# deprekate/PHANOTATE

Hardware: AMD Instinct MI355X
Metric: Mbp/s annotated (whole node) on 50 kb synthetic phage contigs (higher is better)
Workload: dtype u8 bases / fp64 scores / int64 edge weights / int128 distances; 1 GPU; batch of 1000 synthetic 50000 bp phage contigs on one GPU, resident in HBM (BASELINE config 4); contigs_total=1000, contigs_rank0=1000, contig_length=50000

## Files before the change

include/phx.h:

```cpp
#ifndef PHX_H
#define PHX_H

#include <stddef.h>
#include <stdint.h>

#ifdef __cplusplus
extern "C" {
#endif

#define PHX_VERSION 410
#define PHX_MAX_CODONS 16

#define PHX_OK 0
#define PHX_E_ARG (-1)
#define PHX_E_NODEVICE (-10)
#define PHX_E_HIP (-11)
#define PHX_E_NOMEM (-12)
#define PHX_E_STATE (-13)
#define PHX_E_PARAM (-14)
#define PHX_E_IO (-15)

#define PHX_S_OK 0
#define PHX_S_BADLETTER (-2)
#define PHX_S_TOOSHORT (-3)
#define PHX_S_BADTRNA (-4)
#define PHX_S_PARALLEL (-6)
#define PHX_S_OVERFLOW (-7)
#define PHX_S_LONGORF (-8)
#define PHX_S_NEGCYCLE (-9)
#define PHX_S_NOPATH 1

typedef struct phx_ctx phx_ctx;

typedef struct phx_params {
    int32_t minlen;
    int32_t n_start;
    char start[PHX_MAX_CODONS][4];
    double start_w[PHX_MAX_CODONS];
    int32_t n_stop;
    char stop[PHX_MAX_CODONS][4];
    char start_w_text[PHX_MAX_CODONS][32];
} phx_params;

typedef struct phx_gene {
    int32_t left;
    int32_t right;
    int32_t strand;
    int32_t frame;
    double score;
} phx_gene;

typedef struct phx_result {
    int32_t status;
    int32_t n_genes;
    phx_gene *genes;
} phx_result;

typedef struct phx_orf {
    int32_t start;
    int32_t stop;
    int32_t frame;
    int32_t length;
    int32_t rbs;
    int32_t startidx;
    int32_t group;
    int32_t hist[9];
    double pstop;
    double weight_rbs;
    double S;
    double weight;
} phx_orf;

typedef struct phx_node {
    int32_t pos;
    int8_t type;
    int8_t frame;
    int16_t pad;
    int32_t other;
    int32_t refidx;
    double o;
} phx_node;

typedef struct phx_edge {
    int32_t src, dst;
    double w;
    int32_t inexact;
    int32_t pad;
    double d1, d2, err;
} phx_edge;

typedef struct phx_globals {
    int64_t L;
    double pstop;
    double background_rbs[28];
    double training_rbs[28];
    double pos_max[4], pos_min[4];
    int32_t n_orf, n_group, n_node, n_edge, n_bridge;
    int32_t n_limbs;
    int32_t sssp_sweeps;
    int32_t sssp_iters;
    int32_t status;
    int32_t sssp_kernel;
    int32_t sssp_handed_back;
    int32_t tie;
    int32_t certified;
    uint32_t rbs_background_count[28], rbs_training_count[28];
    uint32_t gc_max_count[4], gc_min_count[4];
    int64_t gc_count;
} phx_globals;

int phx_version(void);
int phx_device_count(void);
const char *phx_strerror(int code);
const char *phx_last_error(const phx_ctx *ctx);

void phx_default_params(phx_params *p);
int phx_params_from_flags(const char *start_codons, const char *stop_codons, int32_t minlen, phx_params *p);

int phx_create(const phx_params *params, int device, void *stream, phx_ctx **out);
#define PHX_CREATE_USE_STREAM 1u
#define PHX_CREATE_NO_GRAPH 2u
#define PHX_CREATE_SIZE_EVERY_RUN 4u
#define PHX_CREATE_SOLVER_GLOBAL 8u
#define PHX_CREATE_SOLVER_NO_WAVE 16u
#define PHX_CREATE_NO_CERTIFY 32u
#define PHX_CREATE_CERT_TIGHT 64u
#define PHX_CREATE_POISON 256u
#define PHX_CREATE_ONE_STREAM 512u
#define PHX_CREATE_CERT_WIDE 128u
#define PHX_CREATE_NO_DUO 4096u
#define PHX_CREATE_NO_SEG 8192u
#define PHX_CREATE_NO_FUSE 2048u
#define PHX_CREATE_NO_EXACT 1024u
int phx_create_ex(const phx_params *params, int device, void *stream, uint32_t flags, phx_ctx **out);
void phx_destroy(phx_ctx *ctx);

int phx_annotate(phx_ctx *ctx, int32_t n, const char *const *seq, const int64_t *len, phx_result *out );
void phx_free_results(phx_result *res, int32_t n);

int phx_upload(phx_ctx *ctx, int32_t n, const char *const *seq, const int64_t *len);
int phx_attach(phx_ctx *ctx, int32_t n, const void *d_ascii, const int64_t *offsets);
int phx_set_trnas(phx_ctx *ctx, const int64_t *offsets , const int32_t *start, const int32_t *stop);
int phx_run(phx_ctx *ctx);
int phx_run_async(phx_ctx *ctx);
int phx_wait(phx_ctx *ctx);
int phx_download(phx_ctx *ctx, phx_result *out);
int phx_download_flat(phx_ctx *ctx, phx_gene *genes, int64_t cap, int64_t *offsets , int32_t *status , int64_t *total);

typedef struct phx_pool phx_pool;
int phx_pool_create(const phx_params *params, int32_t n_dev, const int32_t *devices, uint32_t flags, phx_pool **out);
void phx_pool_destroy(phx_pool *pool);
const char *phx_pool_last_error(const phx_pool *pool);
int phx_pool_annotate(phx_pool *pool, int32_t n, const char *const *seq, const int64_t *len, int64_t batch_bases,
                      const int64_t *trna_offsets, const int32_t *trna_start, const int32_t *trna_stop, phx_result *out );

int phx_certified(phx_ctx *ctx, int8_t *cert );
int phx_set_exact(phx_ctx *ctx, int on);

int phx_tap_globals(phx_ctx *ctx, int32_t contig, phx_globals *out);
int phx_tap_positions(phx_ctx *ctx, int32_t contig, uint8_t *cls, uint8_t *gcc, uint8_t *binF, uint8_t *binR);
int phx_tap_orfs(phx_ctx *ctx, int32_t contig, phx_orf *out );
int phx_tap_nodes(phx_ctx *ctx, int32_t contig, phx_node *out );
int phx_tap_edges(phx_ctx *ctx, int32_t contig, phx_edge *out );
int phx_tap_path(phx_ctx *ctx, int32_t contig, int32_t *path, int32_t cap, int32_t *n_path, uint64_t *dist_limbs, int32_t cap_limbs);
int phx_tap_dist(phx_ctx *ctx, int32_t contig, uint64_t *dist_limbs, int64_t cap_words);

typedef struct phx_orf_margin {
    int32_t left, right, strand, frame;
    double score;
    double margin;
    int32_t called;
    int32_t through;
} phx_orf_margin;
int phx_margins_flat(phx_ctx *ctx, phx_orf_margin *rec, int64_t cap, int64_t *offsets , int32_t *status , int64_t *total);
int phx_tap_dist_target(phx_ctx *ctx, int32_t contig, uint64_t *dist_limbs, int64_t cap_words);
int phx_margins_ms(phx_ctx *ctx, float *ms );

typedef struct phx_gene_drop {
    int32_t left, right, strand, frame;
    double score;
    double drop;
    int32_t called;
    int32_t bypass;
} phx_gene_drop;
int phx_drop_margins_flat(phx_ctx *ctx, phx_gene_drop *rec, int64_t cap, int64_t *offsets , int32_t *status , int64_t *total);
int phx_drop_ms(phx_ctx *ctx, float *ms );
int phx_drop_stats(phx_ctx *ctx, int64_t *out );

typedef struct phx_gene_repl {
    int32_t left, right, strand, frame;
    double drop;
    int32_t called, bypass;
    int32_t span_left, span_right;
    int32_t n_removed, n_added;
    int64_t gene_off;
} phx_gene_repl;
int phx_replacements_flat(phx_ctx *ctx, phx_gene_repl *rec, int64_t cap, phx_gene *genes, int64_t gene_cap, int64_t *offsets ,
                          int32_t *status , int64_t *total, int64_t *gene_total);
int phx_tap_replacement(phx_ctx *ctx, int32_t contig, int32_t k, int32_t *path, int32_t cap, int32_t *n_path);
int phx_replacements_ms(phx_ctx *ctx, float *ms );
int phx_replacement_stats(phx_ctx *ctx, int64_t *out );

int phx_reannotate_flat(phx_ctx *ctx, const uint8_t *forbid, const int64_t *orf_offsets , uint32_t flags, phx_gene *genes, int64_t cap,
                        int64_t *offsets , int32_t *status , double *delta , int64_t *total);
int phx_orf_offsets(phx_ctx *ctx, int64_t *orf_offsets );
int phx_tap_repath(phx_ctx *ctx, int32_t contig, int32_t *path, int32_t cap, int32_t *n_path, uint64_t *dist_limbs, int32_t cap_limbs);
int phx_reannotate_ms(phx_ctx *ctx, float *ms );

int phx_dump_text(phx_ctx *ctx, int32_t contig, char **text, int64_t *text_len);

int phx_solve(phx_ctx *ctx, int32_t V, int32_t E, const int32_t *src, const int32_t *dst, const uint64_t *w_limbs,
              int32_t n_limbs, int32_t source, int32_t target, int32_t *path_out, int32_t cap, int32_t *n_path,
              uint64_t *dist_limbs);

#define PHX_N_STAGES 14
int phx_set_profiling(phx_ctx *ctx, int on);
int phx_set_profiling_stages(phx_ctx *ctx, uint32_t stage_mask);
int phx_get_stage_ms(phx_ctx *ctx, float *ms , int32_t *launches , int reset);
const char *phx_stage_name(int k);
int64_t phx_plan_timeouts(phx_ctx *ctx);
int64_t phx_front_runs(phx_ctx *ctx);
int64_t phx_seg_runs(phx_ctx *ctx);
int64_t phx_seg_fallbacks(phx_ctx *ctx);
int phx_seg_stats(phx_ctx *ctx, int32_t i, int32_t *out, int32_t cap_records);
int phx_batch_sizes(phx_ctx *ctx, int64_t *L, int64_t *n_orf, int64_t *n_node, int64_t *n_edge);

int phx_synth_contig(uint64_t seed, int64_t L, char *out);
int phx_dec_eval(const char *op, const char *a, const char *b, int prec, char *out, int cap);
int phx_dd_eval(const char *op, double ah, double al, double bh, double bl, double *rh, double *rl);
int phx_dd_shortest(double x, uint64_t *digits, int32_t *exp10);

typedef struct phx_fasta phx_fasta;
int phx_fasta_read(const char *path, phx_fasta **out);
int32_t phx_fasta_count(const phx_fasta *f);
int phx_fasta_record(const phx_fasta *f, int32_t i, const char **name, const char **seq, int64_t *len);
int phx_fasta_arrays(const phx_fasta *f, const char **names, const char **seqs, int64_t *lens);
void phx_fasta_free(phx_fasta *f);
int phx_format_tabular(int32_t n, const char *const *names, const phx_gene *genes, const int64_t *offsets, const int32_t *status, char **text, int64_t *text_len);
int phx_format_margins(int32_t n, const char *const *names, const phx_orf_margin *rec, const int64_t *offsets, const int32_t *status, char **text, int64_t *text_len);
int phx_format_drops(int32_t n, const char *const *names, const phx_gene_drop *rec, const int64_t *offsets, const int32_t *status, char **text, int64_t *text_len);
int phx_format_replacements(int32_t n, const char *const *names, const phx_gene_repl *rec, const phx_gene *genes, const int64_t *offsets,
                            const int32_t *status, char **text, int64_t *text_len);
void phx_free_text(char *text);

#ifdef __cplusplus
}
#endif
#endif
```

phanotate_amd/_lib.py:

```python
import ctypes as C
import os

import numpy as np

HERE = os.path.dirname(os.path.abspath(__file__))
SO = os.path.join(HERE, "libphx.so")
MAXC = 16
N_STAGES = 14


class Params(C.Structure):
    _fields_ = [
        ("minlen", C.c_int32),
        ("n_start", C.c_int32),
        ("start", (C.c_char * 4) * MAXC),
        ("start_w", C.c_double * MAXC),
        ("n_stop", C.c_int32),
        ("stop", (C.c_char * 4) * MAXC),
        ("start_w_text", (C.c_char * 32) * MAXC),
    ]


class Gene(C.Structure):
    _fields_ = [("left", C.c_int32), ("right", C.c_int32), ("strand", C.c_int32), ("frame", C.c_int32), ("score", C.c_double)]


class Result(C.Structure):
    _fields_ = [("status", C.c_int32), ("n_genes", C.c_int32), ("genes", C.POINTER(Gene))]


class Globals(C.Structure):
    _fields_ = [
        ("L", C.c_int64), ("pstop", C.c_double),
        ("background_rbs", C.c_double * 28), ("training_rbs", C.c_double * 28),
        ("pos_max", C.c_double * 4), ("pos_min", C.c_double * 4),
        ("n_orf", C.c_int32), ("n_group", C.c_int32), ("n_node", C.c_int32), ("n_edge", C.c_int32), ("n_bridge", C.c_int32),
        ("n_limbs", C.c_int32), ("sssp_sweeps", C.c_int32), ("sssp_iters", C.c_int32), ("status", C.c_int32),
        ("sssp_kernel", C.c_int32), ("sssp_handed_back", C.c_int32), ("tie", C.c_int32), ("certified", C.c_int32),
        ("rbs_background_count", C.c_uint32 * 28), ("rbs_training_count", C.c_uint32 * 28), ("gc_max_count", C.c_uint32 * 4), ("gc_min_count", C.c_uint32 * 4),
        ("gc_count", C.c_int64),
    ]


GENE_DT = np.dtype([("left", "i4"), ("right", "i4"), ("strand", "i4"), ("frame", "i4"), ("score", "f8")], align=True)
ORF_DT = np.dtype([("start", "i4"), ("stop", "i4"), ("frame", "i4"), ("length", "i4"), ("rbs", "i4"), ("startidx", "i4"), ("group", "i4"),
                   ("hist", "i4", (9,)), ("pstop", "f8"), ("weight_rbs", "f8"), ("S", "f8"), ("weight", "f8")], align=True)
NODE_DT = np.dtype([("pos", "i4"), ("type", "i1"), ("frame", "i1"), ("pad", "i2"), ("other", "i4"), ("refidx", "i4"), ("o", "f8")], align=True)
MARGIN_DT = np.dtype([("left", "i4"), ("right", "i4"), ("strand", "i4"), ("frame", "i4"), ("score", "f8"), ("margin", "f8"), ("called", "i4"), ("through", "i4")], align=True)
DROP_DT = np.dtype([("left", "i4"), ("right", "i4"), ("strand", "i4"), ("frame", "i4"), ("score", "f8"), ("drop", "f8"), ("called", "i4"), ("bypass", "i4")], align=True)
REPL_DT = np.dtype([("left", "i4"), ("right", "i4"), ("strand", "i4"), ("frame", "i4"), ("drop", "f8"), ("called", "i4"), ("bypass", "i4"),
                    ("span_left", "i4"), ("span_right", "i4"), ("n_removed", "i4"), ("n_added", "i4"), ("gene_off", "i8")], align=True)
EDGE_DT = np.dtype([("src", "i4"), ("dst", "i4"), ("w", "f8"), ("inexact", "i4"), ("pad", "i4"), ("d1", "f8"), ("d2", "f8"), ("err", "f8")], align=True)

_lib = None


class PhxError(RuntimeError):
    def __init__(self, code, msg):
        super().__init__("libphx error %d: %s" % (code, msg))
        self.code = code


def _preload_hip_runtime():
    import importlib.util
    import sys

    if "torch" in sys.modules:
        return
    try:
        spec = importlib.util.find_spec("torch")
    except (ImportError, ValueError):
        spec = None
    if spec is None or not spec.submodule_search_locations:
        return
    cand = os.path.join(list(spec.submodule_search_locations)[0], "lib", "libamdhip64.so")
    if os.path.exists(cand):
        try:
            C.CDLL(cand, mode=C.RTLD_GLOBAL)
        except OSError:
            pass


def lib():
    global _lib
    if _lib is not None:
        return _lib
    if not os.path.exists(SO):
        raise ImportError("%s is missing: build it with `python -c 'import __graft_entry__ as g; g.build()'` "
                          "or `make -C phanotate_amd/csrc`; phanotate_amd has no CPU fallback" % SO)
    _preload_hip_runtime()
    L = C.CDLL(SO)
    vp, i32, i64 = C.c_void_p, C.c_int32, C.c_int64
    P = C.POINTER
    sig = {
        "phx_version": (C.c_int, []),
        "phx_device_count": (C.c_int, []),
        "phx_strerror": (C.c_char_p, [C.c_int]),
        "phx_last_error": (C.c_char_p, [vp]),
        "phx_default_params": (None, [P(Params)]),
        "phx_params_from_flags": (C.c_int, [C.c_char_p, C.c_char_p, i32, P(Params)]),
        "phx_set_exact": (C.c_int, [vp, C.c_int]),
        "phx_pool_create": (C.c_int, [P(Params), i32, P(i32), C.c_uint32, P(vp)]),
        "phx_pool_destroy": (None, [vp]),
        "phx_pool_last_error": (C.c_char_p, [vp]),
        "phx_pool_annotate": (C.c_int, [vp, i32, P(C.c_char_p), P(i64), i64, vp, vp, vp, P(Result)]),
        "phx_dump_text": (C.c_int, [vp, i32, P(vp), P(i64)]),
        "phx_dec_eval": (C.c_int, [C.c_char_p, C.c_char_p, C.c_char_p, C.c_int, C.c_char_p, C.c_int]),
        "phx_dd_eval": (C.c_int, [C.c_char_p, C.c_double, C.c_double, C.c_double, C.c_double, P(C.c_double), P(C.c_double)]),
        "phx_dd_shortest": (C.c_int, [C.c_double, P(C.c_uint64), P(i32)]),
        "phx_create": (C.c_int, [P(Params), C.c_int, vp, P(vp)]),
        "phx_create_ex": (C.c_int, [P(Params), C.c_int, vp, C.c_uint32, P(vp)]),
        "phx_destroy": (None, [vp]),
        "phx_annotate": (C.c_int, [vp, i32, P(C.c_char_p), P(i64), P(Result)]),
        "phx_free_results": (None, [P(Result), i32]),
        "phx_upload": (C.c_int, [vp, i32, P(C.c_char_p), P(i64)]),
        "phx_attach": (C.c_int, [vp, i32, vp, P(i64)]),
        "phx_set_trnas": (C.c_int, [vp, vp, vp, vp]),
        "phx_run": (C.c_int, [vp]),
        "phx_run_async": (C.c_int, [vp]),
        "phx_wait": (C.c_int, [vp]),
        "phx_download": (C.c_int, [vp, P(Result)]),
        "phx_download_flat": (C.c_int, [vp, vp, i64, vp, vp, P(i64)]),
        "phx_certified": (C.c_int, [vp, vp]),
        "phx_tap_globals": (C.c_int, [vp, i32, P(Globals)]),
        "phx_tap_positions": (C.c_int, [vp, i32, vp, vp, vp, vp]),
        "phx_tap_orfs": (C.c_int, [vp, i32, vp]),
        "phx_tap_nodes": (C.c_int, [vp, i32, vp]),
        "phx_tap_edges": (C.c_int, [vp, i32, vp]),
        "phx_tap_path": (C.c_int, [vp, i32, vp, i32, P(i32), vp, i32]),
        "phx_tap_dist": (C.c_int, [vp, i32, vp, i64]),
        "phx_tap_dist_target": (C.c_int, [vp, i32, vp, i64]),
        "phx_margins_flat": (C.c_int, [vp, vp, i64, vp, vp, P(i64)]),
        "phx_margins_ms": (C.c_int, [vp, P(C.c_float)]),
        "phx_format_margins": (C.c_int, [i32, vp, vp, vp, vp, P(vp), P(i64)]),
        "phx_drop_margins_flat": (C.c_int, [vp, vp, i64, vp, vp, P(i64)]),
        "phx_drop_ms": (C.c_int, [vp, P(C.c_float)]),
        "phx_drop_stats": (C.c_int, [vp, P(i64)]),
        "phx_format_drops": (C.c_int, [i32, vp, vp, vp, vp, P(vp), P(i64)]),
        "phx_replacements_flat": (C.c_int, [vp, vp, i64, vp, i64, vp, vp, P(i64), P(i64)]),
        "phx_tap_replacement": (C.c_int, [vp, i32, i32, vp, i32, P(i32)]),
        "phx_replacements_ms": (C.c_int, [vp, P(C.c_float)]),
        "phx_replacement_stats": (C.c_int, [vp, P(i64)]),
        "phx_format_replacements": (C.c_int, [i32, vp, vp, vp, vp, vp, P(vp), P(i64)]),
        "phx_reannotate_flat": (C.c_int, [vp, vp, vp, C.c_uint32, vp, i64, vp, vp, vp, P(i64)]),
        "phx_orf_offsets": (C.c_int, [vp, vp]),
        "phx_tap_repath": (C.c_int, [vp, i32, vp, i32, P(i32), vp, i32]),
        "phx_reannotate_ms": (C.c_int, [vp, P(C.c_float)]),
        "phx_solve": (C.c_int, [vp, i32, i32, vp, vp, vp, i32, i32, i32, vp, i32, P(i32), vp]),
        "phx_set_profiling": (C.c_int, [vp, C.c_int]),
        "phx_set_profiling_stages": (C.c_int, [vp, C.c_uint32]),
        "phx_get_stage_ms": (C.c_int, [vp, P(C.c_float), P(i32), C.c_int]),
        "phx_stage_name": (C.c_char_p, [C.c_int]),
        "phx_batch_sizes": (C.c_int, [vp, P(i64), P(i64), P(i64), P(i64)]),
        "phx_plan_timeouts": (C.c_int64, [vp]),
        "phx_front_runs": (C.c_int64, [vp]),
        "phx_seg_runs": (C.c_int64, [vp]),
        "phx_seg_fallbacks": (C.c_int64, [vp]),
        "phx_seg_stats": (C.c_int, [vp, C.c_int32, C.c_void_p, C.c_int32]),
        "phx_synth_contig": (C.c_int, [C.c_uint64, i64, C.c_char_p]),
        "phx_fasta_read": (C.c_int, [C.c_char_p, P(vp)]),
        "phx_fasta_count": (i32, [vp]),
        "phx_fasta_record": (C.c_int, [vp, i32, P(vp), P(vp), P(i64)]),
        "phx_fasta_arrays": (C.c_int, [vp, vp, vp, vp]),
        "phx_fasta_free": (None, [vp]),
        "phx_format_tabular": (C.c_int, [i32, vp, vp, vp, vp, P(vp), P(i64)]),
        "phx_free_text": (None, [vp]),
    }
    for name, (res, args) in sig.items():
        f = getattr(L, name)
        f.restype = res
        f.argtypes = args
    assert GENE_DT.itemsize == C.sizeof(Gene)
    assert MARGIN_DT.itemsize == 40
    assert DROP_DT.itemsize == 40
    assert REPL_DT.itemsize == 56
    _lib = L
    return L


EXPORTS = ["phx_version", "phx_device_count", "phx_strerror", "phx_last_error", "phx_default_params", "phx_params_from_flags", "phx_set_exact", "phx_pool_create", "phx_pool_destroy", "phx_pool_last_error", "phx_pool_annotate", "phx_dump_text", "phx_dec_eval", "phx_dd_eval", "phx_dd_shortest", "phx_create", "phx_create_ex", "phx_destroy",
           "phx_annotate", "phx_free_results", "phx_upload", "phx_attach", "phx_set_trnas", "phx_run", "phx_run_async", "phx_wait", "phx_download", "phx_download_flat", "phx_certified", "phx_tap_globals",
           "phx_tap_positions", "phx_tap_orfs", "phx_tap_nodes", "phx_tap_edges", "phx_tap_path", "phx_tap_dist", "phx_solve", "phx_set_profiling", "phx_set_profiling_stages",
           "phx_get_stage_ms", "phx_stage_name", "phx_batch_sizes", "phx_plan_timeouts", "phx_front_runs", "phx_seg_runs", "phx_seg_fallbacks", "phx_seg_stats", "phx_synth_contig", "phx_fasta_read", "phx_fasta_count",
           "phx_fasta_record", "phx_fasta_arrays", "phx_fasta_free", "phx_format_tabular", "phx_free_text",
           "phx_margins_flat", "phx_tap_dist_target", "phx_margins_ms", "phx_format_margins",
           "phx_drop_margins_flat", "phx_drop_ms", "phx_drop_stats", "phx_format_drops",
           "phx_replacements_flat", "phx_tap_replacement", "phx_replacements_ms", "phx_replacement_stats",
           "phx_format_replacements",
           "phx_reannotate_flat", "phx_orf_offsets", "phx_tap_repath", "phx_reannotate_ms"]
```

phanotate_amd/api.py:

```python
import ctypes as C

import numpy as np

from . import _lib
from ._lib import PhxError


def make_params(start_codons="atg:0.85,gtg:0.10,ttg:0.05", stop_codons="tag,tga,taa", minlen=90):
    p = _lib.Params()
    rc = _lib.lib().phx_params_from_flags(start_codons.encode(), stop_codons.encode(), int(minlen), C.byref(p))
    if rc:
        raise ValueError("start / stop codons %r / %r, minlen %r: libphx takes codon:weight pairs and codons of exactly 3 letters out of acgt, "
                         "at most %d of each, minlen >= 6 (%s)" % (start_codons, stop_codons, minlen, _lib.MAXC, _lib.lib().phx_strerror(rc).decode()))
    p.start_codons_text = start_codons
    return p


def synth_contig(seed, L=50000):
    buf = C.create_string_buffer(int(L))
    rc = _lib.lib().phx_synth_contig(int(seed), int(L), buf)
    if rc:
        raise PhxError(rc, "phx_synth_contig")
    return buf.raw


class Pool:

    def __init__(self, params=None, devices=(0,), flags=()):
        self.L = _lib.lib()
        self.params = params or make_params()
        fl = 0
        for f in flags:
            fl |= Annotator.FLAGS[f]
        devs = (C.c_int32 * len(devices))(*[int(d) for d in devices])
        h = C.c_void_p()
        rc = self.L.phx_pool_create(C.byref(self.params), len(devices), devs, fl, C.byref(h))
        if rc:
            raise PhxError(rc, "%s (%s)" % (self.L.phx_strerror(rc).decode(), self.L.phx_last_error(None).decode()))
        self.h = h

    def close(self):
        if getattr(self, "h", None):
            self.L.phx_pool_destroy(self.h)
            self.h = None

    def __enter__(self):
        return self

    def __exit__(self, *exc):
        self.close()

    def __del__(self):
        try:
            self.close()
        except Exception:
            pass

    def annotate(self, seqs, trnas=None, batch_bases=0):
        seqs = [s.encode() if isinstance(s, str) else bytes(s) for s in seqs]
        n = len(seqs)
        arr = (C.c_char_p * max(n, 1))(*seqs)
        lens = (C.c_int64 * max(n, 1))(*[len(s) for s in seqs])
        res = (_lib.Result * max(n, 1))()
        to = ta = tz = None
        if trnas is not None:
            offs = np.zeros(n + 1, np.int64)
            np.cumsum([len(t) for t in trnas], out=offs[1:])
            a = np.ascontiguousarray([h[0] for t in trnas for h in t] or [0], np.int32)
            z = np.ascontiguousarray([h[1] for t in trnas for h in t] or [0], np.int32)
            to, ta, tz = (x.ctypes.data_as(C.c_void_p) for x in (offs, a, z))
        rc = self.L.phx_pool_annotate(self.h, n, arr, lens, int(batch_bases), to, ta, tz, res)
        if rc:
            raise PhxError(rc, "phx_pool_annotate: %s (%s)" % (self.L.phx_strerror(rc).decode(), self.L.phx_pool_last_error(self.h).decode()))
        out = []
        for i in range(n):
            g = np.zeros(res[i].n_genes, _lib.GENE_DT)
            if res[i].n_genes:
                C.memmove(g.ctypes.data, res[i].genes, res[i].n_genes * _lib.GENE_DT.itemsize)
            out.append((int(res[i].status), g))
        self.L.phx_free_results(res, n)
        return out


class Annotator:

    FLAGS = {"no_graph": 2, "size_every_run": 4, "solver_global": 8, "solver_no_wave": 16, "no_certify": 32, "cert_tight": 64, "cert_wide": 128, "poison": 256, "one_stream": 512, "no_exact": 1024, "no_fuse": 2048, "no_duo": 4096, "no_seg": 8192}

    def __init__(self, params=None, device=0, stream=None, flags=()):
        self.L = _lib.lib()
        self.params = params or make_params()
        h = C.c_void_p()
        fl = 0
        for f in flags:
            fl |= self.FLAGS[f]
        if stream is None:
            rc = self.L.phx_create_ex(C.byref(self.params), int(device), None, fl, C.byref(h))
        else:
            rc = self.L.phx_create_ex(C.byref(self.params), int(device), C.c_void_p(int(stream)), 1 | fl, C.byref(h))
        if rc:
            raise PhxError(rc, "%s (%s)" % (self.L.phx_strerror(rc).decode(), self.L.phx_last_error(None).decode()))
        self.h = h
        self.n = 0

    def close(self):
        if getattr(self, "h", None):
            self.L.phx_destroy(self.h)
            self.h = None

    def __del__(self):
        try:
            self.close()
        except Exception:
            pass

    def _chk(self, rc, what):
        if rc:
            raise PhxError(rc, "%s: %s (%s)" % (what, self.L.phx_strerror(rc).decode(), self.L.phx_last_error(self.h).decode()))

    def upload(self, seqs):
        seqs = [s.encode() if isinstance(s, str) else bytes(s) for s in seqs]
        n = len(seqs)
        arr = (C.c_char_p * n)(*seqs)
        lens = (C.c_int64 * n)(*[len(s) for s in seqs])
        self._keep = (seqs, arr, lens)
        self._chk(self.L.phx_upload(self.h, n, arr, lens), "phx_upload")
        self.n = n
        self._orf_offs = None

    def upload_raw(self, ptrs, lens, keep=None):
        ptrs = np.ascontiguousarray(ptrs, np.uint64)
        lens = np.ascontiguousarray(lens, np.int64)
        self._keep = (ptrs, lens, keep)
        self._chk(self.L.phx_upload(self.h, len(lens), C.cast(ptrs.ctypes.data, C.POINTER(C.c_char_p)), C.cast(lens.ctypes.data, C.POINTER(C.c_int64))), "phx_upload")
        self.n = len(lens)
        self._orf_offs = None

    def attach(self, dev_ptr, offsets):
        offs = (C.c_int64 * len(offsets))(*[int(x) for x in offsets])
        self._keep = (offs,)
        self._chk(self.L.phx_attach(self.h, len(offsets) - 1, C.c_void_p(int(dev_ptr)), offs), "phx_attach")
        self.n = len(offsets) - 1
        self._orf_offs = None

    def set_trnas(self, trnas):
        if trnas is None:
            self._chk(self.L.phx_set_trnas(self.h, None, None, None), "phx_set_trnas")
            return
        if len(trnas) != self.n:
            raise ValueError("one hit list per contig of the batch")
        offs = np.zeros(self.n + 1, np.int64)
        np.cumsum([len(t) for t in trnas], out=offs[1:])
        a = np.ascontiguousarray([h[0] for t in trnas for h in t] or [0], np.int32)
        z = np.ascontiguousarray([h[1] for t in trnas for h in t] or [0], np.int32)
        vp = lambda x: x.ctypes.data_as(C.c_void_p)
        self._chk(self.L.phx_set_trnas(self.h, vp(offs), vp(a), vp(z)), "phx_set_trnas")

    def run(self):
        self._chk(self.L.phx_run(self.h), "phx_run")
        self._orf_offs = None

    def run_async(self):
        self._chk(self.L.phx_run_async(self.h), "phx_run_async")
        self._orf_offs = None

    def wait(self):
        self._chk(self.L.phx_wait(self.h), "phx_wait")

    def set_exact(self, on):
        self._chk(self.L.phx_set_exact(self.h, 1 if on else 0), "phx_set_exact")

    def download_flat(self, exact=True):
        if not exact:
            self._chk(self.L.phx_set_exact(self.h, 0), "phx_set_exact")
            try:
                res = self._download_flat()
            finally:
                self._chk(self.L.phx_set_exact(self.h, 1), "phx_set_exact")
            self.resolved = []
            return res
        res = self._download_flat()
        self.resolved = [int(i) for i in np.nonzero(self.certified() == 2)[0]] if self.n else []
        return res

    def _download_flat(self):
        n = self.n
        offs = np.zeros(n + 1, np.int64)
        status = np.zeros(max(n, 1), np.int32)
        total = C.c_int64(0)
        vp = lambda a: a.ctypes.data_as(C.c_void_p)
        guess = max(int(getattr(self, "_genes_seen", 0) * 1.25) + 64, 1)
        genes = np.empty(guess, _lib.GENE_DT)
        rc = self.L.phx_download_flat(self.h, vp(genes), len(genes), vp(offs), vp(status), C.byref(total))
        if rc == -1 and int(total.value) > len(genes):
            genes = np.empty(int(total.value), _lib.GENE_DT)
            rc = self.L.phx_download_flat(self.h, vp(genes), len(genes), vp(offs), vp(status), C.byref(total))
        self._chk(rc, "phx_download_flat")
        self._genes_seen = int(total.value)
        return status[:n], offs, genes[: int(total.value)]

    def certified(self):
        c = np.zeros(max(self.n, 1), np.int8)
        self._chk(self.L.phx_certified(self.h, c.ctypes.data_as(C.c_void_p)), "phx_certified")
        return c[: self.n]

    def download(self):
        status, offs, genes = self.download_flat()
        o = offs.tolist()
        st = status.tolist()
        return [(st[i], genes[o[i]:o[i + 1]]) for i in range(self.n)]

    def annotate(self, seqs, trnas=None):
        self.upload(seqs)
        if trnas is not None:
            self.set_trnas(trnas)
        self.run_async()
        return self.download()

    def annotate_flat(self, seqs):
        self.upload(seqs)
        self.run_async()
        return self.download_flat()

    def annotate_flat_raw(self, ptrs, lens, keep=None):
        self.upload_raw(ptrs, lens, keep)
        self.run_async()
        return self.download_flat()

    def dump_text(self, i):
        text, n = C.c_void_p(), C.c_int64()
        self._chk(self.L.phx_dump_text(self.h, int(i), C.byref(text), C.byref(n)), "phx_dump_text")
        out = C.string_at(text.value, n.value)
        self.L.phx_free_text(text)
        return out

    def globals(self, i):
        g = _lib.Globals()
        self._chk(self.L.phx_tap_globals(self.h, i, C.byref(g)), "phx_tap_globals")
        return g

# ... 101 lines not shown
        n = self.n
        offs = np.zeros(n + 1, np.int64)
        status = np.zeros(max(n, 1), np.int32)
        total, gtotal = C.c_int64(), C.c_int64()
        vp = lambda a: a.ctypes.data_as(C.c_void_p)
        self._chk(self.L.phx_replacements_flat(self.h, None, 0, None, 0, vp(offs), vp(status), C.byref(total), C.byref(gtotal)), "phx_replacements_flat")
        rec = np.empty(max(int(total.value), 1), _lib.REPL_DT)
        genes = np.empty(max(int(gtotal.value), 1), _lib.GENE_DT)
        self._chk(self.L.phx_replacements_flat(self.h, vp(rec), len(rec), vp(genes), len(genes), vp(offs), vp(status), C.byref(total), C.byref(gtotal)),
                  "phx_replacements_flat")
        return status[:n], offs, rec[: int(total.value)], genes[: int(gtotal.value)]

    def replacement_path(self, i, k):
        n = C.c_int32()
        self._chk(self.L.phx_tap_replacement(self.h, i, k, None, 0, C.byref(n)), "phx_tap_replacement")
        p = np.zeros(max(n.value, 1), np.int32)
        self._chk(self.L.phx_tap_replacement(self.h, i, k, p.ctypes.data_as(C.c_void_p), len(p), C.byref(n)), "phx_tap_replacement")
        return p[: n.value].copy()

    def replacements_ms(self):
        ms = (C.c_float * 3)()
        self._chk(self.L.phx_replacements_ms(self.h, ms), "phx_replacements_ms")
        return dict(zip(("argmin", "walk", "download"), [float(x) for x in ms]))

    def replacement_stats(self):
        out = (C.c_int64 * 5)()
        self._chk(self.L.phx_replacement_stats(self.h, out), "phx_replacement_stats")
        return dict(zip(("cross", "chain_nodes", "cross_kept", "cut", "regrown"), [int(x) for x in out]))

    def orf_offsets(self):
        if getattr(self, "_orf_offs", None) is None:
            offs = np.zeros(self.n + 1, np.int64)
            self._chk(self.L.phx_orf_offsets(self.h, offs.ctypes.data_as(C.c_void_p)), "phx_orf_offsets")
            self._orf_offs = offs
        return self._orf_offs

    def orf_index(self, i, left, right, strand):
        cache = getattr(self, "_orf_index", None)
        if cache is None or cache[0] is not self.orf_offsets() or cache[1] != i:
            o = self.orfs(i)
            fwd = o["frame"] > 0
            lo = np.where(fwd, o["start"], o["stop"])
            hi = np.where(fwd, o["stop"], o["start"]) + 2
            table = {}
            for k, key in enumerate(zip(lo.tolist(), hi.tolist(), fwd.tolist())):
                table.setdefault(key, k)
            cache = self._orf_index = (self.orf_offsets(), i, table)
        try:
            return cache[2][(int(left), int(right), int(strand) > 0)]
        except KeyError:
            raise KeyError("contig %d has no ORF %d..%d on strand %+d" % (i, left, right, 1 if int(strand) > 0 else -1)) from None

    def reannotate(self, forbid, solve_all=False):
        n = self.n
        if len(forbid) != n:
            raise ValueError("one index array (or None) per contig of the batch")
        oo = self.orf_offsets()
        mask = np.zeros(max(int(oo[n]), 1), np.uint8)
        for i, f in enumerate(forbid):
            if f is None:
                continue
            idx = np.asarray(f, np.int64).reshape(-1)
            if idx.size and (idx.min() < 0 or idx.max() >= oo[i + 1] - oo[i]):
                raise IndexError("contig %d has %d ORFs" % (i, oo[i + 1] - oo[i]))
            mask[oo[i] + idx] = 1
        offs = np.zeros(n + 1, np.int64)
        status = np.zeros(max(n, 1), np.int32)
        delta = np.zeros(max(n, 1), np.float64)
        total = C.c_int64(0)
        vp = lambda a: a.ctypes.data_as(C.c_void_p)
        fl = 1 if solve_all else 0
        self._chk(self.L.phx_reannotate_flat(self.h, vp(mask), vp(oo), fl, None, 0, vp(offs), vp(status), vp(delta), C.byref(total)), "phx_reannotate_flat")
        genes = np.empty(max(int(total.value), 1), _lib.GENE_DT)
        self._chk(self.L.phx_reannotate_flat(self.h, vp(mask), vp(oo), fl, vp(genes), len(genes), vp(offs), vp(status), vp(delta), C.byref(total)), "phx_reannotate_flat")
        return status[:n], offs, genes[: int(total.value)], delta[:n]

    def reannotated_path(self, i):
        g = self.globals(i)
        p = np.zeros(max(g.n_node, 1), np.int32)
        n = C.c_int32()
        limbs = np.zeros(32, np.uint64)
        self._chk(self.L.phx_tap_repath(self.h, i, p.ctypes.data_as(C.c_void_p), len(p), C.byref(n), limbs.ctypes.data_as(C.c_void_p), 32), "phx_tap_repath")
        nl = max(g.n_limbs, 1)
        v = 0
        for k in range(nl):
            v |= int(limbs[k]) << (64 * k)
        if v >> (64 * nl - 1):
            v -= 1 << (64 * nl)
        return p[: n.value].copy(), v

    def reannotate_ms(self):
        ms = (C.c_float * 3)()
        self._chk(self.L.phx_reannotate_ms(self.h, ms), "phx_reannotate_ms")
        return dict(zip(("mask", "solve", "finish"), [float(x) for x in ms]))

    def drop_stats(self):
        out = (C.c_int64 * 4)()
        self._chk(self.L.phx_drop_stats(self.h, out), "phx_drop_stats")
        return dict(zip(("slots", "cross", "rescanned", "layered"), [int(x) for x in out]))

    def solve(self, V, src, dst, weights, source, target, n_limbs=None):
        E = len(src)
        mx = max([abs(int(w)) for w in weights] + [1])
        bits = mx.bit_length() + max(V, 2).bit_length() + 3
        if n_limbs is None:
            n_limbs = 2 if bits <= 128 else 4 if bits <= 256 else 8 if bits <= 512 else 17
        wl = np.zeros((max(E, 1), n_limbs), np.uint64)
        mask = (1 << 64) - 1
        for e, w in enumerate(weights):
            w = int(w) & ((1 << (64 * n_limbs)) - 1)
            for k in range(n_limbs):
                wl[e, k] = (w >> (64 * k)) & mask
        s = np.ascontiguousarray(src, np.int32)
        d = np.ascontiguousarray(dst, np.int32)
        path = np.zeros(V, np.int32)
        n = C.c_int32()
        dl = np.zeros(n_limbs, np.uint64)
        self._chk(self.L.phx_solve(self.h, V, E, s.ctypes.data_as(C.c_void_p), d.ctypes.data_as(C.c_void_p), wl.ctypes.data_as(C.c_void_p),
                                   n_limbs, source, target, path.ctypes.data_as(C.c_void_p), V, C.byref(n), dl.ctypes.data_as(C.c_void_p)), "phx_solve")
        if n.value == 0:
            return [], None
        v = 0
        for k in range(n_limbs):
            v |= int(dl[k]) << (64 * k)
        if v >> (64 * n_limbs - 1):
            v -= 1 << (64 * n_limbs)
        return path[: n.value].tolist(), v

    def set_profiling(self, on=True):
        self._chk(self.L.phx_set_profiling(self.h, 1 if on else 0), "phx_set_profiling")

    def set_profiling_stages(self, names):
        idx = {self.L.phx_stage_name(k).decode(): k for k in range(_lib.N_STAGES)}
        mask = 0
        for nm in names:
            mask |= 1 << idx[nm]
        self._chk(self.L.phx_set_profiling_stages(self.h, mask), "phx_set_profiling_stages")

    def stage_ms(self, reset=True):
        ms = (C.c_float * _lib.N_STAGES)()
        nl = (C.c_int32 * _lib.N_STAGES)()
        self._chk(self.L.phx_get_stage_ms(self.h, ms, nl, 1 if reset else 0), "phx_get_stage_ms")
        return {self.L.phx_stage_name(k).decode(): (float(ms[k]), int(nl[k])) for k in range(_lib.N_STAGES)}

    def front_runs(self):
        return int(self.L.phx_front_runs(self.h))

    def seg_runs(self):
        return int(self.L.phx_seg_runs(self.h))

    def seg_fallbacks(self):
        return int(self.L.phx_seg_fallbacks(self.h))

    def seg_stats(self, i):
        import numpy as np

        out = np.zeros((64, 8), np.int32)
        n = self.L.phx_seg_stats(self.h, int(i), out.ctypes.data_as(C.c_void_p), 64)
        return out[:n]

    def plan_timeouts(self):
        return int(self.L.phx_plan_timeouts(self.h))

    def batch_sizes(self):
        v = [C.c_int64() for _ in range(4)]
        self._chk(self.L.phx_batch_sizes(self.h, *[C.byref(x) for x in v]), "phx_batch_sizes")
        return dict(L=v[0].value, n_orf=v[1].value, n_node=v[2].value, n_edge=v[3].value)
```

phanotate_amd/csrc/phx_api.cpp:

```cpp
#include <hip/hip_runtime.h>

#include <algorithm>
#include <atomic>
#include <cmath>
#include <condition_variable>
#include <functional>
#include <mutex>
#include <cstdio>
#include <cstdlib>
#include <cstring>
#include <memory>
#include <limits>
#include <map>
#include <string>
#include <thread>
#include <vector>

#include "phx_internal.h"
extern "C" {
#include "phx_dec.h"
}

namespace {

// ... 18 lines not shown
            p = nullptr; cap = 0;
            const size_t want = count + count / 4 + 16;
            if (hipHostMalloc((void **)&p, want * sizeof(DMeta), hipHostMallocDefault) != hipSuccess) { p = nullptr; n = 0; return false; }
            cap = want;
        }
        n = count;
        if (n) memset(p, 0, n * sizeof(DMeta));
        return true;
    }
    void release() { if (p) (void)hipHostFree(p); p = nullptr; n = cap = 0; }
    DMeta *begin() { return p; }
    DMeta *end() { return p + n; }
    const DMeta *begin() const { return p; }
    const DMeta *end() const { return p + n; }
    DMeta &operator[](size_t i) { return p[i]; }
    const DMeta &operator[](size_t i) const { return p[i]; }
    DMeta *data() { return p; }
};

}

struct StagePool {
    std::vector<std::thread> th;
    std::mutex m;
    std::condition_variable cv, cv_done;
    const std::function<void()> *job = nullptr;
    uint64_t gen = 0;
    int active = 0;
    bool stop = false;
    void grow(int n) {
        while ((int)th.size() < n) {
            try { th.emplace_back([this, seen = gen]() mutable { loop(seen); }); } catch (...) { break; }
        }
    }
    void loop(uint64_t seen) {
        std::unique_lock<std::mutex> lk(m);
        for (;;) {
            cv.wait(lk, [&] { return stop || gen != seen; });
            if (stop) return;
            seen = gen;
            const std::function<void()> *j = job;
            lk.unlock();
            (*j)();
            lk.lock();
            if (--active == 0) cv_done.notify_all();
        }
    }
    void start(const std::function<void()> *j) {
        std::lock_guard<std::mutex> lk(m);
        job = j; active = (int)th.size(); gen++;
        cv.notify_all();
    }
    void finish() {
        std::unique_lock<std::mutex> lk(m);
        cv_done.wait(lk, [&] { return active == 0; });
    }
    ~StagePool() {
        { std::lock_guard<std::mutex> lk(m); stop = true; cv.notify_all(); }
        for (std::thread &t : th) t.join();
    }
};

struct phx_ctx {
    int device = 0;
    hipStream_t stream = nullptr;
    bool own_stream = false;
    hipStream_t aux[4] = {nullptr, nullptr, nullptr, nullptr};
    bool in_flight = false;
    int pend_mask = 0;
    int64_t pend_lds[4] = {0, 0, 0, 0};
    hipEvent_t ev_fork = nullptr, ev_fork_plan = nullptr, ev_fork_nodes = nullptr, ev_join_nodes = nullptr, ev_fork_pre = nullptr, ev_join_pre = nullptr, ev_fork_orf = nullptr, ev_join_orf = nullptr, ev_fork_score = nullptr, ev_join_score = nullptr, ev_join[4] = {nullptr, nullptr, nullptr, nullptr};
    phx_params params;
    std::string err;
    DParams *d_params = nullptr;
    int n = 0;
    bool uploaded = false, ran = false;
    int64_t totalL = 0, tot_orf = 0, tot_grp = 0, tot_node = 0, tot_edge = 0;
    int n_limbs = 0;
    MetaBuf meta;
    bool meta_stale = false;
    DRes *res = nullptr;
    size_t res_cap = 0;
    std::vector<uint32_t> ftab;
    uint32_t vtotal = 0;
    bool defcod = false;
    const void *attached = nullptr;
    hipEvent_t ev_upload = nullptr; bool upload_pending = false;
    hipEvent_t ev_layout = nullptr; bool layout_pending = false;
    hipEvent_t ev_piece[2] = {nullptr, nullptr};
    void *h_tiles = nullptr; size_t h_tiles_cap = 0;
    bool eager_now = false;
    bool eager_done = false;
    bool trna_clean = true;
    std::unique_ptr<StagePool> pool;
    DevBuf b_bridge, b_recs, b_meta, b_tiles, b_nbits, b_nbase, b_cbits, b_orf, b_ostat, b_oweight, b_owi, b_oflag, b_onode, b_grp, b_bits, b_cpre, b_bpre, b_item, b_iprev;
    DevBuf b_ewf, b_esrcf;
    bool tapw_valid = false;
    int64_t tot_nbits = 0, tot_bridge = 0;
    int64_t tot_words = 0, tot_items = 0;
    DevBuf b_win, b_wrole;
    DevBuf b_tnode, b_tedge, b_tnid, b_tbits;
    std::vector<DTNode> h_tnode;
    bool has_trna = false;
    DevBuf b_cint, b_csig;
    DevBuf b_eref;
    bool certify = true;
    bool cert_done = false;
    bool exact = true;
    bool exact_done = false;
    std::map<int, std::vector<DGene>> exact_genes;
    std::vector<int> host_only;
    int exact_failed = 0;
    double cert_scale = 1.0;
    bool cert_wide = false;
    bool poison = false;
    bool one_stream = false;
    bool learning = false;
    DevBuf b_tie;
    int64_t tie_seen = 0;
    DevBuf b_ekey;
    DevBuf b_meta0;
    bool meta0_dirty = true;
    int runs_on_layout = 0;
    DevBuf b_node, b_parent, b_inoff, b_no, b_npos, b_ehit, b_mreach, b_olist, b_dist, b_esrc, b_ew, b_ewl, b_path, b_genes, b_gtot, b_tot, b_lpart, b_res, b_sord, b_gtab, b_erank;
    DTotals *h_tot = nullptr;
    bool have_plan = false;
    int last_mask = 0;
    int last_vmax = 0;
    int64_t last_lds[4] = {0, 0, 0, 0};
    int64_t max_len = 0;
    bool graphs_enabled = true, graph_valid = false, tiles_dirty = true;
    hipGraph_t graph = nullptr;
    hipGraphExec_t graph_exec = nullptr;
    int graph_flags = -1;
    void *h_stage = nullptr;
    size_t h_stage_cap = 0;
    DGene *h_genes = nullptr; size_t h_genes_cap = 0;
    bool prof = false;
    uint32_t prof_mask = 0xffffffffu;
    int n_simd = 1024;
    bool force_global_sssp = false;
    bool no_wave = false, always_sync = false;
    bool no_fuse = false;
    bool duo = true;
    int front_spins = 8000;
    bool side_score = true;
    int orf_stream = 1;
    bool orf_rows = true;
    bool eager_cert = true;
    bool pend_cert = false;
    bool pend_front = false;
    bool front_off = false;
    int64_t front_runs = 0;
    bool seg_on = true;
    bool seg_off = false;
    bool seg_never = false;
    bool pend_seg = false;
    int pend_seg_k = 0;
    bool seg_clean = false;
    int seg_max_n = 32;
    int seg_margin_bp = 6000;
    int64_t seg_runs = 0, seg_aborts = 0, seg_fallbacks = 0;
    DevBuf b_swin, b_swrole, b_sdist, b_segw;
    int64_t plan_timeouts = 0;
    bool plan_stream_off = false;
    DevBuf b_mo, b_md, b_mw, b_mdt, b_mrec, b_mstat;
    bool margins_done = false;
    phx_orf_margin *h_mrec = nullptr; size_t h_mrec_cap = 0;
    std::vector<int32_t> mstat;
    std::vector<DGrp> mgrp;
    hipEvent_t mev[5] = {nullptr, nullptr, nullptr, nullptr, nullptr};
    float margins_ms[4] = {0, 0, 0, 0};
    bool rev_done = false;
    float rev_ms[2] = {0, 0};
    DevBuf b_dpi, b_djs, b_djt, b_dfi, b_dla, b_dslot, b_dgtab, b_doff, b_dsx, b_dcx, b_dda, b_ddb, b_drec, b_dstats;
    bool drops_done = false;
    phx_gene_drop *h_drec = nullptr; size_t h_drec_cap = 0;
    std::vector<int64_t> droff;
    hipEvent_t dev_[5] = {nullptr, nullptr, nullptr, nullptr, nullptr};
    float drop_ms[4] = {0, 0, 0, 0};
    int64_t drop_stats[4] = {0, 0, 0, 0};
    bool drop_trees = false;
    DevBuf b_dps, b_dts, b_rwin, b_rxs, b_rcoff, b_rcm, b_rchain, b_rrnd, b_rinfo, b_rdoff, b_rdet, b_rgenes, b_rrec, b_rcnt;
    bool repl_done = false;
    std::vector<phx_gene_repl> h_rrec;
    std::vector<phx_gene> h_rgenes;
    std::vector<int32_t> h_rdet, h_rinfo;
    std::vector<int64_t> h_rdoff;
    std::vector<std::vector<int32_t>> h_rpath;
    int64_t rchain_cap = 0;
    hipEvent_t rev_ev[9] = {nullptr, nullptr, nullptr, nullptr, nullptr, nullptr, nullptr, nullptr, nullptr};
    float repl_ms[3] = {0, 0, 0};
    int64_t repl_stats[5] = {0, 0, 0, 0, 0};
    DevBuf b_qmeta, b_qtot, b_qdist, b_qparent, b_qpath, b_qgenes, b_qgtot, b_qtie, b_qmask, b_qforb, b_qsel, b_qplan, b_qrec;
    bool reann_done = false;
    bool qgrp_done = false;
    std::vector<DGrp> qgrp;
    std::vector<uint8_t> h_qforb;
    uint32_t h_qflags = 0;
    std::vector<int32_t> h_qsel;
    std::vector<DReannRec> h_qrec;
    std::vector<DGene> h_qgenes;
    std::vector<uint8_t> h_qdforb;
    DTotals h_qtot;
    uint32_t h_qgtot = 0;
    hipEvent_t qev[6] = {nullptr, nullptr, nullptr, nullptr, nullptr, nullptr};
    float reann_ms[3] = {0, 0, 0};
    float stage_ms[PHX_N_STAGES] = {0};
    int stage_n[PHX_N_STAGES] = {0};
    std::vector<std::pair<int, std::pair<hipEvent_t, hipEvent_t>>> pending;
    std::vector<hipEvent_t> ev_pool;
};

static int seg_cap(const phx_ctx *c);
namespace {

#define HIPCHK(ctx, call)                                                                                      \
    do {                                                                                                       \
        hipError_t e_ = (call);                                                                                \
        if (e_ != hipSuccess) {                                                                                \
            (ctx)->err = std::string(#call) + ": " + hipGetErrorString(e_);                                    \
            return PHX_E_HIP;                                                                                  \
        }                                                                                                      \
    } while (0)

int ensure(phx_ctx *c, DevBuf &b, size_t bytes) {
    if (bytes + 2048 <= b.cap && b.p) return PHX_OK;
    c->graph_valid = false;
    if (b.p) HIPCHK(c, hipFree(b.p));
    b.p = nullptr; b.cap = 0;
    size_t want = bytes + bytes / 8 + 4096;
    HIPCHK(c, hipMalloc(&b.p, want));
    b.cap = want;
    if (c->poison) HIPCHK(c, hipMemset(b.p, 0xA5, want));
    return PHX_OK;
}
void release(DevBuf &b) {
    if (b.p) (void)hipFree(b.p);
    b.p = nullptr; b.cap = 0;
}

inline int code_of(char c) { return c == 'a' ? 0 : c == 'c' ? 1 : c == 't' ? 2 : c == 'g' ? 3 : -1; }

int check_params(const phx_params *p) {
    if (!p || p->minlen < 6 || p->n_start < 1 || p->n_start > PHX_MAX_CODONS || p->n_stop < 1 || p->n_stop > PHX_MAX_CODONS) return PHX_E_PARAM;
    for (int i = 0; i < p->n_start; i++) {
        for (int j = 0; j < 3; j++) if (code_of(p->start[i][j]) < 0) return PHX_E_PARAM;
        if (p->start[i][3] != 0) return PHX_E_PARAM;
        if (!(p->start_w[i] == p->start_w[i])) return PHX_E_PARAM;
        if (!memchr(p->start_w_text[i], 0, sizeof(p->start_w_text[i]))) return PHX_E_PARAM;
        if (p->start_w_text[i][0]) { dec_t t; if (dec_from_str(&t, p->start_w_text[i])) return PHX_E_PARAM; }
    }
    for (int i = 0; i < p->n_stop; i++) {
        for (int j = 0; j < 3; j++) if (code_of(p->stop[i][j]) < 0) return PHX_E_PARAM;
        if (p->stop[i][3] != 0) return PHX_E_PARAM;
    }
    return PHX_OK;
}

void build_dparams(const phx_params *p, DParams *d) {
    memset(d, 0, sizeof(*d));
    d->minlen = p->minlen;
    d->n_start = p->n_start;
    for (int i = 0; i < p->n_start; i++) d->start_w[i] = p->start_w[i];
    { dec_t q[PHX_MAX_CODONS]; dec_start_weights(p->n_start, p->start_w_text, p->start_w, q); for (int i = 0; i < p->n_start; i++) dec_to_dd(&q[i], &d->sw_hi[i], &d->sw_lo[i]); }
    auto codon_code = [](const char *c) { return code_of(c[0]) | (code_of(c[1]) << 2) | (code_of(c[2]) << 4); };
    auto rc_code = [](int ci) {
        int c0 = ci & 3, c1 = (ci >> 2) & 3, c2 = (ci >> 4) & 3;
        return (c2 ^ 2) | ((c1 ^ 2) << 2) | ((c0 ^ 2) << 4);
    };
    int start_idx[64], stop_is[64];
    for (int i = 0; i < 64; i++) { start_idx[i] = -1; stop_is[i] = 0; }
    for (int i = p->n_start - 1; i >= 0; i--) start_idx[codon_code(p->start[i])] = i;
    for (int i = 0; i < p->n_stop; i++) stop_is[codon_code(p->stop[i])] = 1;
    const int atg = codon_code("atg"), cat = codon_code("cat");
    for (int ci = 0; ci < 64; ci++) {
        const int rc = rc_code(ci);
        int cls = CLS_NONE, idx = 0;
        if (start_idx[ci] >= 0) { cls = CLS_FS; idx = start_idx[ci]; }
        else if (start_idx[rc] >= 0) { cls = CLS_RS; idx = start_idx[rc]; }
        else if (stop_is[ci]) cls = CLS_FT;
        else if (stop_is[rc]) cls = CLS_RT;
        d->cls_tab[ci] = (uint8_t)(cls | (idx << 3) | (start_idx[rc] >= 0 ? 0x80 : 0));
        d->atg_tab[ci] = (uint8_t)((ci == atg ? 1 : 0) | (ci == cat ? 2 : 0) | (idx << 2));
    }
}

hipEvent_t get_event(phx_ctx *c) {
    if (!c->ev_pool.empty()) { hipEvent_t e = c->ev_pool.back(); c->ev_pool.pop_back(); return e; }
    hipEvent_t e = nullptr;
    (void)hipEventCreate(&e);
    return e;
}
struct StageTimer {
    phx_ctx *c; int st; bool on = false; hipEvent_t a = nullptr, b = nullptr; hipStream_t str = nullptr;
    StageTimer(phx_ctx *c_, int st_, hipStream_t on_stream = nullptr) : c(c_), st(st_) {
        on = c->prof && ((c->prof_mask >> st_) & 1u);
        str = on_stream ? on_stream : c->stream;
        if (on) { a = get_event(c); b = get_event(c); (void)hipEventRecord(a, str); }
    }
    ~StageTimer() {
        if (on) { (void)hipEventRecord(b, str); c->pending.push_back({st, {a, b}}); }
    }
};
void collect_timers(phx_ctx *c) {
    for (auto &p : c->pending) {
// ... 126 lines not shown
        m.bits_off = words; m.item_off = items; m.nbits_off = nbw;
        m.bridge_off = nbr; m.bridge_cap = (int32_t)(L / 500 + 2);
        nbr += m.bridge_cap;
        nbw += 9 * (int64_t)m.nw;
        words += PHX_BITMAP_WORDS_PER_NW * (int64_t)m.nw; items += 6 * (int64_t)m.nw;
        off += L;
        off = (off + 15) & ~(int64_t)15;
    }
    c->vtotal = (uint32_t)(recs - 1);
    c->ftab.push_back(c->vtotal);
    {
        int ci = 0;
        for (int64_t blk = 0; blk * 62 < (int64_t)c->vtotal + 62; blk++) {
            const int64_t v = blk * 62 > 0 ? blk * 62 - 1 : 0;
            while (ci + 1 < n && v >= (int64_t)c->ftab[(size_t)ci + 1]) ci++;
            c->ftab.push_back((uint32_t)ci);
        }
    }
    c->tot_words = words; c->tot_items = items; c->tot_nbits = nbw; c->tot_bridge = nbr;
    c->totalL = offsets_or_null ? offsets_or_null[n] : off;
    c->n = n;
    return PHX_OK;
}

int ensure_position_buffers(phx_ctx *c) {
    int rc;
    if ((rc = ensure(c, c->b_recs, ((size_t)c->vtotal + 2) * 36))) return rc;
    if ((rc = ensure(c, c->b_nbits, (size_t)(c->tot_nbits + 8) * 8))) return rc;
    if ((rc = ensure(c, c->b_nbase, (size_t)(c->tot_nbits / 3 + 8) * 4))) return rc;
    if ((rc = ensure(c, c->b_meta, sizeof(DMeta) * (size_t)(c->n + 1)))) return rc;
    if ((rc = ensure(c, c->b_tiles, 4 * (c->ftab.size() + 1)))) return rc;
    if ((rc = ensure(c, c->b_gtot, 64))) return rc;
    if ((rc = ensure(c, c->b_lpart, ((size_t)c->n / 256 + 2) * 32 + 512))) return rc;
    if (sssp_ordered(c) && (rc = ensure(c, c->b_sord, (size_t)c->n * 4))) return rc;
    if ((rc = ensure(c, c->b_gtab, ((size_t)c->n + 1) * GT_N * 10))) return rc;
    if ((rc = ensure(c, c->b_res, ((size_t)c->n + 1) * sizeof(DRes) + sizeof(DTotals)))) return rc;
    if (c->res_cap < (size_t)c->n + 1) {
        if (c->res) (void)hipHostFree(c->res);
        c->res = nullptr; c->res_cap = 0;
        const size_t want = (size_t)c->n + (size_t)c->n / 4 + 16;
        if (hipHostMalloc((void **)&c->res, want * sizeof(DRes) + sizeof(DTotals), hipHostMallocDefault) != hipSuccess) { c->res = nullptr; c->err = "hipHostMalloc failed"; return PHX_E_NOMEM; }
        c->res_cap = want;
    }
    if ((rc = ensure(c, c->b_bits, (size_t)(c->tot_words + 8) * 8))) return rc;
    {
        const size_t W = (size_t)(c->tot_words / PHX_BITMAP_WORDS_PER_NW);
        if ((rc = ensure(c, c->b_cpre, (6 * (W / PHX_PRE_G + (size_t)c->n) + 2) * 32))) return rc;
        if ((rc = ensure(c, c->b_bpre, (2 * W + 2 * (size_t)c->n + 4) * 16))) return rc;
    }
    if ((rc = ensure(c, c->b_item, (size_t)(c->tot_items + 8) * 8))) return rc;
    if ((rc = ensure(c, c->b_iprev, (size_t)(c->tot_items + 8) * 4))) return rc;
    if ((rc = ensure(c, c->b_bridge, (size_t)(c->tot_bridge + 8) * sizeof(DBridge)))) return rc;
    return PHX_OK;
}

}

extern "C" {

int phx_version(void) { return PHX_VERSION; }

int phx_device_count(void) {
    int n = 0;
    if (hipGetDeviceCount(&n) != hipSuccess) return 0;
    return n;
}

const char *phx_strerror(int code) {
    switch (code) {
    case PHX_OK: return "ok";
    case PHX_E_ARG: return "bad argument";
    case PHX_E_NODEVICE: return "no usable HIP device (libphx has no CPU path)";
    case PHX_E_HIP: return "HIP runtime error";
    case PHX_E_NOMEM: return "out of memory";
    case PHX_E_STATE: return "call sequence error";
    case PHX_E_PARAM: return "bad codon table / minlen";
    case PHX_E_IO: return "file could not be opened or read";
    case PHX_S_BADLETTER: return "letter outside the IUPAC nucleotide alphabet";
    case PHX_S_TOOSHORT: return "contig shorter than 6 bases";
    case PHX_S_PARALLEL: return "bridge edge duplicates a connect edge";
    case PHX_S_BADTRNA: return "a tRNA hit lies outside the contig";
    case PHX_S_OVERFLOW: return "integer path sums overflow";
    case PHX_S_LONGORF: return "an open reading frame of more than 65535 codons";
    case PHX_S_NEGCYCLE: return "relaxation did not converge";
    case PHX_S_NOPATH: return "target unreachable";
    default: return "unknown";
    }
}

const char *phx_last_error(const phx_ctx *ctx) { return ctx ? ctx->err.c_str() : g_create_error.c_str(); }

void phx_default_params(phx_params *p) {
    memset(p, 0, sizeof(*p));
    p->minlen = 90;
    p->n_start = 3;
    strcpy(p->start[0], "atg"); strcpy(p->start[1], "gtg"); strcpy(p->start[2], "ttg");
    p->start_w[0] = 0.85 / 0.85; p->start_w[1] = 0.10 / 0.85; p->start_w[2] = 0.05 / 0.85;
    strcpy(p->start_w_text[0], "0.85"); strcpy(p->start_w_text[1], "0.10"); strcpy(p->start_w_text[2], "0.05");
    p->n_stop = 3;
    strcpy(p->stop[0], "tag"); strcpy(p->stop[1], "tga"); strcpy(p->stop[2], "taa");
}

int phx_params_from_flags(const char *start_codons, const char *stop_codons, int32_t minlen, phx_params *p) {
    if (!p) return PHX_E_ARG;
    phx_default_params(p);
    p->minlen = minlen;
    auto lower3 = [](const std::string &t, char *out) {
        if (t.size() != 3) return false;
        for (int j = 0; j < 3; j++) { const char ch = (char)(t[(size_t)j] | 0x20); if (code_of(ch) < 0) return false; out[j] = ch; }
        out[3] = 0;
        return true;
    };
    auto split = [](const char *s) { std::vector<std::string> v; std::string cur; for (; *s; s++) { if (*s == ',') { v.push_back(cur); cur.clear(); } else cur.push_back(*s); } v.push_back(cur); return v; };
    if (start_codons) {
        p->n_start = 0;
        memset(p->start, 0, sizeof(p->start)); memset(p->start_w, 0, sizeof(p->start_w)); memset(p->start_w_text, 0, sizeof(p->start_w_text));
        double wv[PHX_MAX_CODONS];
        for (const std::string &item : split(start_codons)) {
            const size_t colon = item.find(':');
            if (colon == std::string::npos || item.find(':', colon + 1) != std::string::npos) return PHX_E_PARAM;
            char cod[4];
            if (!lower3(item.substr(0, colon), cod)) return PHX_E_PARAM;
            const std::string wt = item.substr(colon + 1);
            if (wt.empty() || wt.size() >= sizeof(p->start_w_text[0])) return PHX_E_PARAM;
            char *end = nullptr;
            const double w = phx_strtod_c(wt.c_str(), &end);
            if (!end || *end || !(w == w)) return PHX_E_PARAM;
            int at = -1;
            for (int i = 0; i < p->n_start; i++) if (!strcmp(p->start[i], cod)) at = i;
            if (at < 0) { if (p->n_start >= PHX_MAX_CODONS) return PHX_E_PARAM; at = p->n_start++; strcpy(p->start[at], cod); }
            strcpy(p->start_w_text[at], wt.c_str());
            wv[at] = w;
        }
        if (p->n_start < 1) return PHX_E_PARAM;
        double mx = wv[0];
        for (int i = 1; i < p->n_start; i++) mx = wv[i] > mx ? wv[i] : mx;
        for (int i = 0; i < p->n_start; i++) p->start_w[i] = wv[i] / mx;
    }
    if (stop_codons) {
        p->n_stop = 0;
        memset(p->stop, 0, sizeof(p->stop));
        for (const std::string &item : split(stop_codons)) {
            if (p->n_stop >= PHX_MAX_CODONS) return PHX_E_PARAM;
            if (!lower3(item, p->stop[p->n_stop])) return PHX_E_PARAM;
            p->n_stop++;
        }
    }
    return check_params(p);
}

int phx_create(const phx_params *params, int device, void *stream, phx_ctx **out) { return phx_create_ex(params, device, stream, stream ? PHX_CREATE_USE_STREAM : 0u, out); }

int phx_create_ex(const phx_params *params, int device, void *stream, uint32_t flags, phx_ctx **out) {
    if (!out || (flags & ~(PHX_CREATE_USE_STREAM | PHX_CREATE_NO_GRAPH | PHX_CREATE_SIZE_EVERY_RUN | PHX_CREATE_SOLVER_GLOBAL | PHX_CREATE_SOLVER_NO_WAVE | PHX_CREATE_NO_CERTIFY | PHX_CREATE_CERT_TIGHT | PHX_CREATE_CERT_WIDE | PHX_CREATE_POISON | PHX_CREATE_ONE_STREAM | PHX_CREATE_NO_EXACT | PHX_CREATE_NO_FUSE | PHX_CREATE_NO_DUO | PHX_CREATE_NO_SEG)) || (stream && !(flags & PHX_CREATE_USE_STREAM))) return PHX_E_ARG;
    *out = nullptr;
    int rc = check_params(params);
    if (rc) return rc;
    int ndev = 0;
    hipError_t e = hipGetDeviceCount(&ndev);
    if (e != hipSuccess || ndev <= 0 || device < 0 || device >= ndev) {
        g_create_error = e != hipSuccess ? hipGetErrorString(e) : "device index out of range";
        return PHX_E_NODEVICE;
    }
    phx_ctx *c = new phx_ctx();
    c->device = device;
    c->params = *params;
    c->force_global_sssp = (flags & PHX_CREATE_SOLVER_GLOBAL) != 0;
    c->no_wave = (flags & PHX_CREATE_SOLVER_NO_WAVE) != 0;
    c->graphs_enabled = (flags & PHX_CREATE_NO_GRAPH) == 0;
    c->always_sync = (flags & PHX_CREATE_SIZE_EVERY_RUN) != 0;
    c->certify = (flags & PHX_CREATE_NO_CERTIFY) == 0;
    c->exact = (flags & PHX_CREATE_NO_EXACT) == 0;
    c->no_fuse = (flags & PHX_CREATE_NO_FUSE) != 0;
    { const char *e = getenv("PHX_FRONT_SPINS"); if (e && *e) c->front_spins = atoi(e); }
    { const char *e = getenv("PHX_NO_EAGER_CERT"); c->eager_cert = !(e && e[0] == '1'); }
    { const char *e = getenv("PHX_NO_ORF_ROWS"); c->orf_rows = !(e && e[0] == '1'); }
    { const char *e = getenv("PHX_ORF_STREAM"); if (e && *e) { const int v = atoi(e); if (v >= -1 && v <= 3) c->orf_stream = v; } }
    { const char *e = getenv("PHX_NO_SIDE_SCORE"); c->side_score = !(e && e[0] == '1'); }
    { const char *e = getenv("PHX_NO_DUO"); c->duo = !(flags & PHX_CREATE_NO_DUO) && !(e && e[0] == '1'); }
    { const char *e = getenv("PHX_NO_SEG"); c->seg_on = !(flags & PHX_CREATE_NO_SEG) && !(e && e[0] == '1'); }
    { const char *e = getenv("PHX_SEG_MAX_N"); if (e && atoi(e) >= 0) c->seg_max_n = atoi(e); }
    { const char *e = getenv("PHX_SEG_MARGIN_BP"); if (e && atoi(e) > 0) c->seg_margin_bp = atoi(e); }
    c->cert_wide = (flags & PHX_CREATE_CERT_WIDE) != 0;
    c->poison = (flags & PHX_CREATE_POISON) != 0;
    c->cert_scale = (flags & PHX_CREATE_CERT_TIGHT) ? 68719476736.0 : 1.0;
    auto fail = [&](int code) { g_create_error = c->err; phx_destroy(c); return code; };
    if (hipSetDevice(device) != hipSuccess) { c->err = "hipSetDevice failed"; return fail(PHX_E_NODEVICE); }
    { int cus = 0; if (hipDeviceGetAttribute(&cus, hipDeviceAttributeMultiprocessorCount, device) == hipSuccess && cus > 0) c->n_simd = 4 * cus; }
    if (flags & PHX_CREATE_USE_STREAM) {
        c->stream = (hipStream_t)stream; c->own_stream = false;
        if (!stream) c->graphs_enabled = false;
    } else {
        if (hipStreamCreateWithFlags(&c->stream, hipStreamNonBlocking) != hipSuccess) { c->err = "hipStreamCreate failed"; return fail(PHX_E_HIP); }
        c->own_stream = true;
    }
    for (int a = 0; a < 4; a++) {
        if (flags & PHX_CREATE_ONE_STREAM) { c->aux[a] = c->stream; c->one_stream = true; }
        else if (hipStreamCreateWithFlags(&c->aux[a], hipStreamNonBlocking) != hipSuccess) { c->err = "hipStreamCreate failed"; return fail(PHX_E_HIP); }
        if (hipEventCreateWithFlags(&c->ev_join[a], hipEventDisableTiming) != hipSuccess) { c->err = "hipEventCreate failed"; return fail(PHX_E_HIP); }
    }
    if (hipEventCreateWithFlags(&c->ev_upload, hipEventDisableTiming) != hipSuccess || hipEventCreateWithFlags(&c->ev_layout, hipEventDisableTiming) != hipSuccess ||
        hipEventCreateWithFlags(&c->ev_piece[0], hipEventDisableTiming) != hipSuccess || hipEventCreateWithFlags(&c->ev_piece[1], hipEventDisableTiming) != hipSuccess) { c->err = "hipEventCreate failed"; return fail(PHX_E_HIP); }
    if (hipEventCreateWithFlags(&c->ev_fork, hipEventDisableTiming) != hipSuccess || hipEventCreateWithFlags(&c->ev_fork_plan, hipEventDisableTiming) != hipSuccess ||
        hipEventCreateWithFlags(&c->ev_fork_nodes, hipEventDisableTiming) != hipSuccess || hipEventCreateWithFlags(&c->ev_join_nodes, hipEventDisableTiming) != hipSuccess ||
        hipEventCreateWithFlags(&c->ev_fork_pre, hipEventDisableTiming) != hipSuccess || hipEventCreateWithFlags(&c->ev_join_pre, hipEventDisableTiming) != hipSuccess ||
        hipEventCreateWithFlags(&c->ev_fork_orf, hipEventDisableTiming) != hipSuccess || hipEventCreateWithFlags(&c->ev_join_orf, hipEventDisableTiming) != hipSuccess ||
        hipEventCreateWithFlags(&c->ev_fork_score, hipEventDisableTiming) != hipSuccess || hipEventCreateWithFlags(&c->ev_join_score, hipEventDisableTiming) != hipSuccess) { c->err = "hipEventCreate failed"; return fail(PHX_E_HIP); }
    DParams dp;
    build_dparams(params, &dp);
    {
        phx_params d;
        phx_default_params(&d);
        DParams dd;
        build_dparams(&d, &dd);
        c->defcod = memcmp(dd.cls_tab, dp.cls_tab, sizeof dp.cls_tab) == 0;
    }
    if (hipMalloc((void **)&c->d_params, sizeof(DParams)) != hipSuccess) { c->err = "hipMalloc failed"; return fail(PHX_E_NOMEM); }
    if (hipMemcpy(c->d_params, &dp, sizeof(dp), hipMemcpyHostToDevice) != hipSuccess) { c->err = "hipMemcpy failed"; return fail(PHX_E_HIP); }
    *out = c;
    return PHX_OK;
}

void phx_destroy(phx_ctx *c) {
    if (!c) return;
    (void)hipSetDevice(c->device);
    c->in_flight = false;
    if (c->stream) (void)hipStreamSynchronize(c->stream);
    DevBuf *all[] = {&c->b_eref, &c->b_cint, &c->b_csig, &c->b_meta0, &c->b_tie, &c->b_ekey, &c->b_tnode, &c->b_tedge, &c->b_tnid, &c->b_tbits, &c->b_win, &c->b_wrole, &c->b_bridge, &c->b_recs, &c->b_meta, &c->b_tiles, &c->b_nbits, &c->b_nbase, &c->b_cbits, &c->b_orf, &c->b_ostat, &c->b_oweight, &c->b_owi, &c->b_oflag, &c->b_ewf, &c->b_esrcf, &c->b_onode, &c->b_grp, &c->b_bits, &c->b_cpre, &c->b_bpre, &c->b_item, &c->b_iprev,
                     &c->b_node, &c->b_parent, &c->b_inoff, &c->b_no, &c->b_npos, &c->b_ehit, &c->b_mreach, &c->b_olist, &c->b_dist, &c->b_esrc, &c->b_ew, &c->b_ewl, &c->b_path, &c->b_genes, &c->b_gtot, &c->b_tot, &c->b_lpart, &c->b_res, &c->b_sord, &c->b_gtab, &c->b_erank, &c->b_swin, &c->b_swrole, &c->b_sdist, &c->b_segw,
                     &c->b_mo, &c->b_md, &c->b_mw, &c->b_mdt, &c->b_mrec, &c->b_mstat,
                     &c->b_dpi, &c->b_djs, &c->b_djt, &c->b_dfi, &c->b_dla, &c->b_dslot, &c->b_dgtab, &c->b_doff, &c->b_dsx, &c->b_dcx, &c->b_dda, &c->b_ddb, &c->b_drec, &c->b_dstats,
                     &c->b_dps, &c->b_dts, &c->b_rwin, &c->b_rxs, &c->b_rcoff, &c->b_rcm, &c->b_rchain, &c->b_rrnd, &c->b_rinfo, &c->b_rdoff, &c->b_rdet, &c->b_rgenes, &c->b_rrec, &c->b_rcnt,
                     &c->b_qmeta, &c->b_qtot, &c->b_qdist, &c->b_qparent, &c->b_qpath, &c->b_qgenes, &c->b_qgtot, &c->b_qtie, &c->b_qmask, &c->b_qforb, &c->b_qsel, &c->b_qplan, &c->b_qrec};
    for (DevBuf *b : all) release(*b);
    for (hipEvent_t e : c->qev) if (e) (void)hipEventDestroy(e);
    if (c->h_mrec) (void)hipHostFree(c->h_mrec);
    if (c->h_drec) (void)hipHostFree(c->h_drec);
    for (hipEvent_t e : c->mev) if (e) (void)hipEventDestroy(e);
    for (hipEvent_t e : c->dev_) if (e) (void)hipEventDestroy(e);
    for (hipEvent_t e : c->rev_ev) if (e) (void)hipEventDestroy(e);
    if (c->graph_exec) (void)hipGraphExecDestroy(c->graph_exec);
    if (c->graph) (void)hipGraphDestroy(c->graph);
    if (c->h_tot) (void)hipHostFree(c->h_tot);
    if (c->d_params) (void)hipFree(c->d_params);
    if (c->h_stage) (void)hipHostFree(c->h_stage);
    if (c->h_genes) (void)hipHostFree(c->h_genes);
    c->meta.release();
    if (c->res) (void)hipHostFree(c->res);
    c->res = nullptr; c->res_cap = 0;
    collect_timers(c);
    for (hipEvent_t e : c->ev_pool) (void)hipEventDestroy(e);
    for (int a = 0; a < 4; a++) { if (c->aux[a] && !c->one_stream) (void)hipStreamDestroy(c->aux[a]); if (c->ev_join[a]) (void)hipEventDestroy(c->ev_join[a]); }
    if (c->ev_upload) (void)hipEventDestroy(c->ev_upload);
    if (c->ev_layout) (void)hipEventDestroy(c->ev_layout);
    for (int k = 0; k < 2; k++) if (c->ev_piece[k]) (void)hipEventDestroy(c->ev_piece[k]);
    if (c->h_tiles) (void)hipHostFree(c->h_tiles);
    if (c->ev_fork) (void)hipEventDestroy(c->ev_fork);
    if (c->ev_fork_plan) (void)hipEventDestroy(c->ev_fork_plan);
    if (c->ev_fork_nodes) (void)hipEventDestroy(c->ev_fork_nodes);
    if (c->ev_join_nodes) (void)hipEventDestroy(c->ev_join_nodes);
    if (c->ev_fork_pre) (void)hipEventDestroy(c->ev_fork_pre);
    if (c->ev_fork_orf) (void)hipEventDestroy(c->ev_fork_orf);
    if (c->ev_fork_score) (void)hipEventDestroy(c->ev_fork_score);
    if (c->ev_join_score) (void)hipEventDestroy(c->ev_join_score);
    if (c->ev_join_orf) (void)hipEventDestroy(c->ev_join_orf);
    if (c->ev_join_pre) (void)hipEventDestroy(c->ev_join_pre);
    if (c->own_stream && c->stream) (void)hipStreamDestroy(c->stream);
    delete c;
}

#ifndef PHX_PLAN_STREAM_MAX
#define PHX_PLAN_STREAM_MAX 800
#endif
#ifndef PHX_UPLOAD_THREADS
#define PHX_UPLOAD_THREADS 16
#endif
#ifndef PHX_UPLOAD_PIECE
#define PHX_UPLOAD_PIECE (4 << 20)
#endif
namespace { int push_layout(phx_ctx *c); }

int phx_upload(phx_ctx *c, int32_t n, const char *const *seq, const int64_t *len) {
    if (!c || n < 0 || (n > 0 && (!seq || !len))) return PHX_E_ARG;
    HIPCHK(c, hipSetDevice(c->device));
    if (c->in_flight) (void)settle(c);
    if (c->upload_pending) { HIPCHK(c, hipEventSynchronize(c->ev_upload)); c->upload_pending = false; }
    c->attached = nullptr;
    int rc = set_batch_layout(c, n, len, nullptr);
    if (rc) return rc;
    const size_t T = ((size_t)c->vtotal + 2) * 36;
    if ((rc = ensure(c, c->b_recs, T))) return rc;
    if (c->h_stage_cap < T) {
        if (c->h_stage) HIPCHK(c, hipHostFree(c->h_stage));
        c->h_stage = nullptr; c->h_stage_cap = 0;
        HIPCHK(c, hipHostMalloc(&c->h_stage, T + T / 8, hipHostMallocDefault));
        c->h_stage_cap = T + T / 8;
    }
    StageTimer t(c, ST_COPY);
    bool eager = c->n > 0 && c->vtotal > 0 && c->aux[1] && !c->one_stream && !c->prof;
    DBatch fb;
    if (eager) {
        if ((rc = ensure_position_buffers(c))) return rc;
        if ((rc = ensure(c, c->b_tot, sizeof(DTotals)))) return rc;
        if ((rc = ensure(c, c->b_meta0, sizeof(DMeta) * (size_t)(c->n + 1)))) return rc;
        if ((rc = push_layout(c))) return rc;
        hipStream_t s0 = c->stream;
        fill_batch(c, &fb);
        phxk_reset(&fb, c->b_meta0.p, (unsigned long long)(c->tot_nbits + 8), 0ull, s0);
    }
    int n_sent = 0;
    struct Piece { int i0, i1; int64_t r0, r1; int items; };
    struct Item { const char *in; int64_t n; uint32_t *out; int64_t nrec; int piece; };
    std::vector<Piece> pieces;
    std::vector<Item> items;
    uint32_t *stage = (uint32_t *)c->h_stage;
    {
        const int64_t piece = PHX_UPLOAD_PIECE / 96, chunk = 96 * 1024;
        int64_t sent = 0; int first = 0;
        for (int i = 0; i < n; i++) {
            const int64_t r0 = c->meta[(size_t)i].rec_off, nrec = 2 * (int64_t)c->meta[(size_t)i].nw + 1;
            const int64_t end = i + 1 < n ? r0 + nrec : (int64_t)c->vtotal + 2;
            for (int64_t o = 0; o < len[i] || o == 0; o += chunk) {
                const bool last = o + chunk >= len[i];
                items.push_back(Item{seq[i] + o, std::min(chunk, len[i] - o), stage + (size_t)(r0 + o / 96) * 9, last ? nrec - o / 96 : chunk / 96, (int)pieces.size()});
            }
            if (end - sent >= piece || i + 1 == n) {
                int cnt = 0;
                for (size_t k = items.size(); k > 0 && items[k - 1].piece == (int)pieces.size(); k--) cnt++;
                pieces.push_back(Piece{first, i + 1, sent, end, cnt}); sent = end; first = i + 1;
            }
        }
        for (int k = 0; k < 9; k++) { stage[k] = k % 3 == 2 ? ~0u : 0u; stage[((size_t)c->vtotal + 1) * 9 + (size_t)k] = stage[k]; }
// ... 131 lines not shown
    c->uploaded = true;
    return PHX_OK;
}

static double host_contig_pstop(uint32_t gc, int L);

static int seg_cap(const phx_ctx *c) {
    if (!c->seg_on || c->seg_off || c->seg_never || !c->duo || c->force_global_sssp || c->no_wave || c->n < 1 || c->n > c->seg_max_n || sssp_ordered(c)) return 0;
    if (c->max_len < (int64_t)c->seg_margin_bp + 4000) return 0;
    const int k = std::min(phxk_seg_kmax(), c->n_simd / c->n);
    return k >= 2 ? k : 0;
}
static bool seg_wanted(const phx_ctx *c) { return seg_cap(c) > 0; }
static int ensure_seg(phx_ctx *c) {
    if (!seg_wanted(c)) return PHX_OK;
    DCaps k;
    current_caps(c, &k);
    if (k.node <= 0 || k.win <= 0 || k.node > (1ll << 22)) return PHX_OK;
    const size_t KM = (size_t)seg_cap(c);
    int rc;
    if ((rc = ensure(c, c->b_swin, KM * (size_t)(k.win + 8) * sizeof(DWin)))) return rc;
    if ((rc = ensure(c, c->b_swrole, KM * (size_t)(k.win + 8) * sizeof(uint2) * WIN_ROLES))) return rc;
    if ((rc = ensure(c, c->b_sdist, KM * (size_t)(k.node + 8) * 16))) return rc;
    if ((rc = ensure(c, c->b_segw, KM * (size_t)(c->n + 1) * 32))) return rc;
    return PHX_OK;
}
static bool seg_ready(const phx_ctx *c, const DCaps &k) {
    if (!seg_wanted(c) || k.node <= 0 || k.node > (1ll << 22)) return false;
    const size_t KM = (size_t)seg_cap(c);
    return c->b_swin.p && c->b_swin.cap >= KM * (size_t)(k.win + 8) * sizeof(DWin) && c->b_swrole.p && c->b_swrole.cap >= KM * (size_t)(k.win + 8) * sizeof(uint2) * WIN_ROLES &&
           c->b_sdist.p && c->b_sdist.cap >= KM * (size_t)(k.node + 8) * 16 && c->b_segw.p && c->b_segw.cap >= KM * (size_t)(c->n + 1) * 32;
}

namespace {

const int kRetry = 1000;

int enqueue_run(phx_ctx *c, bool learn, int &mask, int64_t lds[4]) {
    int rc;
    struct Learning { phx_ctx *c; Learning(phx_ctx *c_, bool on) : c(c_) { c->learning = on; } ~Learning() { c->learning = false; } } learning_scope(c, learn);
    const int n = c->n;
    hipStream_t s = c->stream;
    DBatch b;
    const bool head_done = c->eager_now;
    fill_batch(c, &b);
    {
        StageTimer t(c, ST_MEMSET);
        const unsigned long long tw = c->has_trna ? (unsigned long long)(c->tot_nbits / 3 * 4 + 8) : 0ull;
        if (!head_done) phxk_reset(&b, c->b_meta0.p, (unsigned long long)(c->tot_nbits + 8), tw, s);
        else if (c->has_trna) HIPCHK(c, hipMemsetAsync(c->b_tbits.p, 0, (size_t)tw * 8, s));
    }
    fill_batch(c, &b);
    if (!head_done) {
        StageTimer t(c, ST_FEATURES);
        if (c->attached) phxk_pack_planes(&b, c->attached, s);
        phxk_features(&b, 0u, c->vtotal, s);
    }
    const uint32_t front_stages = (1u << ST_ORF_COUNT) | (1u << ST_ORF_EMIT) | (1u << ST_ORF_STATS) | (1u << ST_SCORE) | (1u << ST_NODES) | (1u << ST_EDGE_COUNT) | (1u << ST_EDGE_FILL);
    const bool fuse = !learn && !(c->prof && (c->prof_mask & front_stages)) && !c->no_fuse && !c->front_off && phxk_front_blocks_y(&b) > 0;
    DTotals *ht = c->h_tot;
    c->pend_front = fuse;
    if (fuse) {
        b.defer_overlap = c->max_len < (1 << 21) ? 1 : 0;
        phxk_front(&b, s);
        HIPCHK(c, hipGetLastError());
        mask = c->last_mask;
        for (int k = 0; k < 4; k++) lds[k] = c->last_lds[k];
    } else {
    HIPCHK(c, hipEventRecord(c->ev_fork_pre, s));
    HIPCHK(c, hipStreamWaitEvent(c->aux[0], c->ev_fork_pre, 0));
    phxk_bit_prefix(&b, c->aux[0]);
    HIPCHK(c, hipEventRecord(c->ev_join_pre, c->aux[0]));
    { StageTimer t(c, ST_ORF_COUNT); phxk_orf_count(&b, s); phxk_layout1(&b, s); }
    HIPCHK(c, hipGetLastError());
    if (learn) {
        { StageTimer t(c, ST_COPY); HIPCHK(c, hipMemcpyAsync(ht, c->b_tot.p, sizeof(DTotals), hipMemcpyDeviceToHost, s)); }
        HIPCHK(c, hipStreamSynchronize(s));
        const size_t NV = (size_t)ht->node + 8, G = (size_t)ht->grp + 1;
        if ((rc = ensure(c, c->b_cbits, (size_t)(ht->cb + 8) * 8))) return rc;
        if ((rc = ensure(c, c->b_orf, sizeof(DOrf) * (size_t)(ht->orf + 1)))) return rc;
        if ((rc = ensure(c, c->b_ostat, sizeof(DOrfStat) * (size_t)(ht->orf + 1)))) return rc;
        if ((rc = ensure(c, c->b_oweight, 8 * (size_t)(ht->orf + 1)))) return rc;
        if ((rc = ensure(c, c->b_owi, 8 * (size_t)(ht->orf + 1)))) return rc;
        if ((rc = ensure(c, c->b_oflag, (size_t)(ht->orf + 16)))) return rc;
        if ((rc = ensure(c, c->b_onode, 4 * (size_t)(ht->orf + 1)))) return rc;
        if ((rc = ensure(c, c->b_grp, sizeof(DGrp) * G))) return rc;
        if ((rc = ensure(c, c->b_genes, 2 * sizeof(DGene) * (G + c->h_tnode.size() + 8)))) return rc;
        if ((rc = ensure(c, c->b_node, NV * sizeof(DNode)))) return rc;
        for (DevBuf *q : {&c->b_parent, &c->b_path, &c->b_olist})
            if ((rc = ensure(c, *q, NV * 4))) return rc;
        if ((rc = ensure(c, c->b_inoff, (NV + (size_t)n + 1) * 4))) return rc;
        if ((rc = ensure(c, c->b_no, NV * 8))) return rc;
        if ((rc = ensure(c, c->b_npos, NV * 4))) return rc;
        if ((rc = ensure(c, c->b_ehit, NV * 8))) return rc;
        if ((rc = ensure(c, c->b_erank, NV * 16))) return rc;
        if ((rc = ensure(c, c->b_mreach, NV * 16))) return rc;
        if ((rc = ensure(c, c->b_dist, NV * 8 * (size_t)std::max(c->n_limbs, 2)))) return rc;
        if (c->certify) {
            if ((rc = ensure(c, c->b_cint, NV * 20))) return rc;
            if ((rc = ensure(c, c->b_csig, NV * 16 * (size_t)std::max(c->n_limbs, 2)))) return rc;
        }
        const size_t NW = NV / 16 + 8 * (size_t)n + 16;
        if ((rc = ensure(c, c->b_win, NW * sizeof(DWin)))) return rc;
        if ((rc = ensure(c, c->b_wrole, NW * sizeof(uint2) * WIN_ROLES))) return rc;
        if ((rc = ensure_seg(c))) return rc;
    }
    fill_batch(c, &b);
    { StageTimer t(c, ST_ORF_EMIT); phxk_orf_emit(&b, s); }
    HIPCHK(c, hipEventRecord(c->ev_fork_nodes, s));
    HIPCHK(c, hipStreamWaitEvent(c->aux[1], c->ev_fork_nodes, 0));
    phxk_nodes(&b, c->aux[1]);
    HIPCHK(c, hipEventRecord(c->ev_join_nodes, c->aux[1]));
    { StageTimer t(c, ST_ORF_STATS); HIPCHK(c, hipStreamWaitEvent(s, c->ev_join_pre, 0)); phxk_orf_stats(&b, s); }
    const bool big_batch = c->n >= 600;
    const bool side_score = c->side_score && big_batch && !c->one_stream && c->aux[0] && !learn;
    if (side_score) {
        HIPCHK(c, hipEventRecord(c->ev_fork_score, s));
        HIPCHK(c, hipStreamWaitEvent(c->aux[0], c->ev_fork_score, 0));
        { StageTimer t(c, ST_SCORE, c->aux[0]); phxk_score(&b, c->aux[0]); }
        HIPCHK(c, hipEventRecord(c->ev_join_score, c->aux[0]));
    } else { StageTimer t(c, ST_SCORE); phxk_score(&b, s); }
    { StageTimer t(c, ST_NODES); HIPCHK(c, hipStreamWaitEvent(s, c->ev_join_nodes, 0)); phxk_node_attr(&b, s); }
    { StageTimer t(c, ST_EDGE_COUNT); phxk_edges_count(&b, s); if (side_score) HIPCHK(c, hipStreamWaitEvent(s, c->ev_join_score, 0)); phxk_layout2(&b, s); }
    HIPCHK(c, hipGetLastError());
    mask = c->last_mask;
    for (int k = 0; k < 4; k++) lds[k] = c->last_lds[k];
    if (learn) {
        { StageTimer t(c, ST_COPY); HIPCHK(c, hipMemcpyAsync(ht, c->b_tot.p, sizeof(DTotals), hipMemcpyDeviceToHost, s)); }
        HIPCHK(c, hipStreamSynchronize(s));
        c->n_limbs = std::max(c->n_limbs, std::max(ht->nlmax, 2));
        if ((rc = ensure(c, c->b_esrc, (size_t)(ht->edge + 1) * 4))) return rc;
        if ((rc = ensure(c, c->b_ew, (size_t)(ht->edge + 1) * 8))) return rc;
        if ((rc = ensure(c, c->b_dist, ((size_t)ht->node + 8) * 8 * (size_t)c->n_limbs))) return rc;
        if (c->certify && (rc = ensure(c, c->b_csig, ((size_t)ht->node + 8) * 16 * (size_t)c->n_limbs))) return rc;
        if ((rc = ensure_seg(c))) return rc;
        mask = ht->class_mask;
        if (mask & 4) mask |= 8;
        for (int k = 0; k < 4; k++) lds[k] = ht->lds_need[k];
    }
    }
    fill_batch(c, &b);
    int stream_k = -1;
    if (c->n <= std::min(PHX_PLAN_STREAM_MAX, c->n_simd * 3 / 4) && !c->plan_stream_off && !b.sord && !c->one_stream && c->aux[3]) {
        if ((mask >> 2) & 1) stream_k = 0;
        else for (int k = 1; k <= 2; k++) if (((mask >> (4 * k + 2)) & 1) && !(mask & 0xffff & ~(15 << (4 * k)))) stream_k = k;
    }
    b.seg = (((mask >> 2) & 1) && seg_ready(c, b.caps)) ? seg_cap(c) : 0;
    c->pend_seg = b.seg != 0; c->pend_seg_k = b.seg;
    if (b.seg && stream_k == 0) stream_k = -1;
    b.seg_nofb = (b.seg && c->seg_clean && !learn) ? 1 : 0;
    b.seg_stream = (b.seg && !head_done && !learn && c->n <= 4 && !c->plan_stream_off && !c->one_stream && c->aux[3]) ? 1 : 0;
    const bool stream_plan = stream_k >= 0;
    b.duo = (c->duo && c->n <= c->n_simd) ? 1 : 0;
    b.plan_stream = stream_k < 0 ? 0 : (2 << stream_k);
    b.defer_overlap = c->max_len < (1 << 21) ? 1 : 0;
    auto launch_plan = [&]() -> int {
        HIPCHK(c, hipEventRecord(c->ev_fork_plan, s));
        HIPCHK(c, hipStreamWaitEvent(c->aux[3], c->ev_fork_plan, 0));
        {
            StageTimer t(c, ST_WAVE_PLAN, c->aux[3]);
            phxk_wave_plan(&b, ((mask >> 6) & 1) | (((mask >> 10) & 1) << 1), c->aux[3]);
            if (b.sord) phxk_sssp_order(&b, c->aux[3]);
        }
        HIPCHK(c, hipEventRecord(c->ev_join[3], c->aux[3]));
        return PHX_OK;
    };
    if ((rc = launch_plan())) return rc;
    b.orf_rows = (!fuse && c->orf_rows && c->n >= 600 && !c->one_stream && c->aux[2]) ? 1 : 0;
    const bool orf_side = b.orf_rows && c->orf_stream >= 0;
    if (orf_side) {
        hipStream_t so = c->aux[c->orf_stream];
        HIPCHK(c, hipEventRecord(c->ev_fork_orf, s));
        HIPCHK(c, hipStreamWaitEvent(so, c->ev_fork_orf, 0));
        phxk_edges_orf(&b, so);
        HIPCHK(c, hipEventRecord(c->ev_join_orf, so));
    }
    if (!fuse) { StageTimer t(c, ST_EDGE_FILL); if (b.orf_rows && !orf_side) phxk_edges_orf(&b, s); phxk_edges_fill(&b, s); if (orf_side) HIPCHK(c, hipStreamWaitEvent(s, c->ev_join_orf, 0)); }
    {
        StageTimer t(c, ST_SSSP);
        if (stream_plan) phxk_sssp(&b, 2 << stream_k, 2, (size_t)lds[stream_k], s);
        if (b.seg_stream) phxk_sssp(&b, 2, 2, (size_t)lds[0], s);
        HIPCHK(c, hipStreamWaitEvent(s, c->ev_join[3], 0));
        const int nl_of[4] = {2, 4, 8, 17};
        int nlaunch = 0, nclass = 0;
        bool used[3] = {false, false, false};
        for (int k = 0; k < 4; k++) nclass += ((mask >> (4 * k)) & 15) ? 1 : 0;
        bool early = false;
        auto early_k = [&](int k) { return ((mask >> (4 * k + 2)) & 1) && ((mask >> (4 * k + 1)) & 1) && (((mask >> (16 + k)) | (mask >> (20 + k))) & 1); };
        for (int k = 0; k < 4; k++) early = early || early_k(k);
        early = early && c->aux[2];
        const bool roomy_side = ((mask >> 3) & 1) && c->aux[2] && !c->one_stream;
        if ((nclass > 1 || early || roomy_side) && c->aux[0]) HIPCHK(c, hipEventRecord(c->ev_fork, s));
        if (early || roomy_side) {
            HIPCHK(c, hipStreamWaitEvent(c->aux[2], c->ev_fork, 0));
            used[2] = true;
            if (roomy_side) phxk_sssp(&b, 2, 3, 0, c->aux[2]);
            if (early)
                for (int k = 3; k >= 0; k--)
                    if (early_k(k)) phxk_sssp(&b, nl_of[k], 1, (size_t)lds[k], c->aux[2]);
            HIPCHK(c, hipEventRecord(c->ev_join[2], c->aux[2]));
        }
        for (int k = 3; k >= 0; k--) {
            if (!((mask >> (4 * k)) & 15)) continue;
            hipStream_t st = s;
            if (nlaunch > 0 && c->aux[0]) {
                const int a = (nlaunch - 1) % 2;
                if (!used[a]) { HIPCHK(c, hipStreamWaitEvent(c->aux[a], c->ev_fork, 0)); used[a] = true; }
                st = c->aux[a];
            }
            for (int mode = 3; mode >= 0; mode--)
                if (((mask >> (4 * k + mode)) & 1) && !(mode == 3 && roomy_side) && !(stream_plan && k == stream_k && mode == 2)) {
                    if ((early && mode == 1 && early_k(k)) || (roomy_side && k == 0 && mode <= 1)) HIPCHK(c, hipStreamWaitEvent(st, c->ev_join[2], 0));
                    if (!(b.seg_stream && k == 0 && mode == 2)) phxk_sssp(&b, nl_of[k], mode, (size_t)lds[k], st);
                    if (b.seg && k == 0 && mode == 2) {
                        phxk_seg_merge(&b, c->last_vmax, st);
                        if (!b.seg_nofb) phxk_seg_fallback(&b, st);
                    }
                }
            nlaunch++;
        }
        for (int a = 0; a < 2; a++)
            if (used[a]) { HIPCHK(c, hipEventRecord(c->ev_join[a], c->aux[a])); HIPCHK(c, hipStreamWaitEvent(s, c->ev_join[a], 0)); }
        if (early || roomy_side) HIPCHK(c, hipStreamWaitEvent(s, c->ev_join[2], 0));
    }
    {
        StageTimer t(c, ST_INORDER);
        int nlm = 0;
        for (int k = 0; k < 4; k++) nlm |= ((mask >> (4 * k)) & 15) ? 1 << k : 0;
        phxk_inorder(&b, nlm, s);
        if (b.gpack) phxk_gene_pack(&b, s);
    }
    HIPCHK(c, hipGetLastError());
    {
        StageTimer t(c, ST_COPY);
        phxk_results(&b, s);
        HIPCHK(c, hipMemcpyAsync(c->res, c->b_res.p, sizeof(DRes) * (size_t)n + sizeof(DTotals), hipMemcpyDeviceToHost, s));
    }
    return PHX_OK;
}

void drop_graph(phx_ctx *c) {
    if (c->graph_exec) (void)hipGraphExecDestroy(c->graph_exec);
    if (c->graph) (void)hipGraphDestroy(c->graph);
    c->graph_exec = nullptr; c->graph = nullptr; c->graph_valid = false;
}

int push_layout(phx_ctx *c) {
    hipStream_t s = c->stream;
    bool pushed = false;
    if (c->meta0_dirty) {
        for (DMeta &m : c->meta) {
            DMeta k = m;
            memset(&m, 0, sizeof(m));
            m.off = k.off; m.L = k.L; m.nw = k.nw; m.rec_off = k.rec_off; m.bits_off = k.bits_off; m.item_off = k.item_off; m.nbits_off = k.nbits_off;
            m.bridge_off = k.bridge_off; m.bridge_cap = k.bridge_cap;
            m.n_tnode = k.n_tnode; m.n_tedge = k.n_tedge; m.tn_off = k.tn_off; m.te_off = k.te_off;
            if ((k.status == PHX_S_PARALLEL || k.status == PHX_S_BADTRNA) && k.n_tedge < 0) { m.status = k.status; m.n_tedge = 0; }
        }
        HIPCHK(c, hipMemcpyAsync(c->b_meta0.p, c->meta.data(), sizeof(DMeta) * (size_t)c->n, hipMemcpyHostToDevice, s));
        c->meta0_dirty = false; pushed = true;
    }
    if (c->tiles_dirty) {
        const size_t tb = 4 * c->ftab.size();
        if (c->h_tiles_cap < tb) {
            if (c->h_tiles) HIPCHK(c, hipHostFree(c->h_tiles));
            c->h_tiles = nullptr; c->h_tiles_cap = 0;
            HIPCHK(c, hipHostMalloc(&c->h_tiles, tb + tb / 4 + 4096, hipHostMallocDefault));
            c->h_tiles_cap = tb + tb / 4 + 4096;
        }
        if (tb) { memcpy(c->h_tiles, c->ftab.data(), tb); HIPCHK(c, hipMemcpyAsync(c->b_tiles.p, c->h_tiles, tb, hipMemcpyHostToDevice, s)); }
        c->tiles_dirty = false; pushed = true;
    }
    if (pushed) { HIPCHK(c, hipEventRecord(c->ev_layout, s)); c->layout_pending = true; }
    return PHX_OK;
}

int launch_once(phx_ctx *c, bool learn) {
    int rc;
    c->tapw_valid = false; c->cert_done = false; c->exact_done = false; c->exact_genes.clear(); c->exact_failed = 0; c->host_only.clear();
    c->margins_done = false; c->rev_done = false; c->drops_done = false; c->drop_trees = false; c->repl_done = false; c->reann_done = false; c->qgrp_done = false;
    hipStream_t s = c->stream;
    c->eager_now = c->eager_done && !c->meta0_dirty && !c->tiles_dirty;
    c->eager_done = false;
    if (learn) c->graph_valid = false;
    if ((rc = ensure_position_buffers(c))) return rc;
    if ((rc = ensure(c, c->b_tot, sizeof(DTotals)))) return rc;
    if (!c->h_tot) HIPCHK(c, hipHostMalloc((void **)&c->h_tot, sizeof(DTotals), hipHostMallocDefault));
    if ((rc = ensure(c, c->b_meta0, sizeof(DMeta) * (size_t)(c->n + 1)))) return rc;
    if ((rc = ensure(c, c->b_tie, (size_t)std::max<int64_t>(1 << 20, c->tie_seen + c->tie_seen / 4)))) return rc;
    if ((rc = push_layout(c))) return rc;
    if (!learn && (rc = ensure_seg(c))) return rc;
    int mask = 0;
    int64_t lds[4] = {0, 0, 0, 0};
    DCaps caps_now;
    current_caps(c, &caps_now);
    const bool use_graph = !learn && !c->prof && !c->eager_now && c->graphs_enabled && (c->runs_on_layout >= 2 || c->graph_valid);
    bool launched = false;
    if (use_graph) {
        if (c->graph_valid && c->graph_exec && c->graph_flags == caps_now.flags) {
            mask = c->last_mask;
            for (int k = 0; k < 4; k++) lds[k] = c->last_lds[k];
            if (hipGraphLaunch(c->graph_exec, s) == hipSuccess) launched = true;
            else { (void)hipGetLastError(); drop_graph(c); c->graphs_enabled = false; }
        } else {
            drop_graph(c);
            if (hipStreamBeginCapture(s, hipStreamCaptureModeThreadLocal) == hipSuccess) {
                rc = enqueue_run(c, false, mask, lds);
                hipGraph_t g = nullptr;
                const hipError_t ee = hipStreamEndCapture(s, &g);
                if (rc == PHX_OK && ee == hipSuccess && g && hipGraphInstantiate(&c->graph_exec, g, nullptr, nullptr, 0) == hipSuccess &&
                    hipGraphLaunch(c->graph_exec, s) == hipSuccess) {
                    c->graph = g; c->graph_valid = true; c->graph_flags = caps_now.flags;
                    launched = true;
                } else {
                    (void)hipGetLastError();
                    if (g) (void)hipGraphDestroy(g);
                    drop_graph(c);
                    c->graphs_enabled = false;
                }
            } else { (void)hipGetLastError(); c->graphs_enabled = false; }
        }
    }
    if (!launched && (rc = enqueue_run(c, learn, mask, lds))) return rc;
    c->pend_mask = mask;
    for (int k = 0; k < 4; k++) c->pend_lds[k] = lds[k];
    return PHX_OK;
}

int finish_once(phx_ctx *c) {
    hipStream_t s = c->stream;
    const int mask = c->pend_mask;
    const int64_t *lds = c->pend_lds;
    HIPCHK(c, hipStreamSynchronize(s));
    collect_timers(c);
    c->meta_stale = true;
    memcpy(c->h_tot, (const void *)(c->res + (size_t)c->n), sizeof(DTotals));
    const DTotals *ht = c->h_tot;
    c->tie_seen = std::max(c->tie_seen, ht->tie_need);
#ifdef FRONT_PROFILE
    if (getenv("PHX_DEBUG_FRONT")) {
        int64_t st[40];
        (void)hipMemcpy(st, (int64_t *)c->b_lpart.p + 16, sizeof st, hipMemcpyDeviceToHost);
        fprintf(stderr, "k_front stamps (us, 100 MHz clock):");
        for (int k = 1; k < 26; k++) fprintf(stderr, " %.1f", (double)(st[k] - st[k - 1]) * 0.01);
        fprintf(stderr, "  total %.1f\n", (double)(st[25] - st[0]) * 0.01);
    }
#endif
    if (ht->front_abort) {
        c->front_off = true; c->graph_valid = false;
        return kRetry;
    }
    if (ht->seg_abort) {
        c->seg_off = true; c->seg_clean = false; c->seg_aborts++; c->graph_valid = false;
        if (getenv("PHX_DEBUG_SEG")) fprintf(stderr, "segments: run given up (reasons %d), %d contigs\n", ht->seg_abort, c->n);
        if (c->seg_aborts > 4 && 4 * c->seg_aborts > c->seg_runs + c->seg_aborts) c->seg_never = true;
        return kRetry;
    }
    if (c->pend_seg && ht->seg_fallbacks) { c->seg_off = true; c->graph_valid = false; }
    if (c->pend_seg && !ht->seg_fallbacks && !c->seg_clean) { c->seg_clean = true; c->graph_valid = false; }
    if (c->pend_seg) { c->seg_runs++; c->seg_fallbacks += ht->seg_fallbacks; if (ht->seg_fallbacks && getenv("PHX_DEBUG_SEG")) fprintf(stderr, "segments: %d of %d contigs solved by one sweep instead\n", ht->seg_fallbacks, c->n); }
    if (ht->plan_timeouts > 0) { c->plan_timeouts += ht->plan_timeouts; c->plan_stream_off = true; c->graph_valid = false; }
    if (ht->overflow) { c->graph_valid = false; return kRetry; }
    bool covered = ((ht->class_mask & ~mask) & 0xffff) == 0;
    for (int k = 0; k < 4; k++) covered = covered && ht->lds_need[k] <= lds[k];
    if (ht->class_mask != c->last_mask || ht->lds_need[0] != c->last_lds[0] || ht->lds_need[1] != c->last_lds[1] || ht->lds_need[2] != c->last_lds[2] || ht->lds_need[3] != c->last_lds[3])
        c->graph_valid = false;
    c->last_mask = ht->class_mask;
    c->last_vmax = ht->vmax;
    for (int k = 0; k < 4; k++) c->last_lds[k] = ht->lds_need[k];
    if (!covered) return kRetry;
    c->tot_orf = ht->orf; c->tot_grp = ht->grp; c->tot_node = ht->node; c->tot_edge = ht->edge;
    c->have_plan = true;
    c->runs_on_layout++;
    if (c->pend_front) c->front_runs++;
    return PHX_OK;
}

int run_once(phx_ctx *c, bool learn) {
    const int rc = launch_once(c, learn);
    return rc ? rc : finish_once(c);
}

int settle(phx_ctx *c) {
    if (!c->in_flight) return PHX_OK;
    c->in_flight = false;
    const bool with_cert = c->pend_cert;
    c->pend_cert = false;
    int rc = finish_once(c);
    if (rc == PHX_OK && with_cert) { c->cert_done = true; c->meta_stale = true; }
    for (int attempt = 0; rc == kRetry && attempt < 3; attempt++) rc = run_once(c, true);
    if (rc == kRetry) { c->err = "batch layout did not settle"; return PHX_E_STATE; }
    if (rc) return rc;
    c->ran = true;
    return PHX_OK;
}

}

#ifdef PHX_DEV_REPORT
static void dev_report(phx_ctx *c) {
    const int n = c->n;
    (void)fetch_meta(c);
    if (getenv("PHX_DEBUG_CENSUS")) { uint32_t t[4] = {0,0,0,0}; (void)hipMemcpy(t, c->b_gtot.p, 16, hipMemcpyDeviceToHost); fprintf(stderr, "census: max concurrent sssp workgroups %u (end %u)\n", t[2], t[1]); }
    if (getenv("PHX_DEBUG_WAVE")) {
        int nfb[8] = {0, 0, 0, 0, 0, 0, 0, 0}, nw = 0;
        for (int i = 0; i < n; i++) { if (c->meta[i].sssp_mode == 2 || c->meta[i].sssp_mode == 3) nw++; else if (c->meta[i].n_node > 2 && c->meta[i].sssp_nl == 2) nfb[c->meta[i].sssp_why & 7]++; }
        fprintf(stderr, "wave kernel: %d contigs done, handed back: plan %d spill %d no-convergence %d rollbacks %d other %d\n", nw, nfb[1], nfb[2], nfb[3], nfb[4], nfb[0]);
        std::vector<std::pair<double, int>> tt;
        long nroll = 0;
        for (int i = 0; i < n; i++) if (c->meta[i].sssp_mode == 2 || c->meta[i].sssp_mode == 3) { const DMeta &m = c->meta[i]; tt.push_back({(m.pmax[0] + m.pmax[1] + m.pmax[2] + m.pmax[3] + m.pmin[0] + m.pmin[1]) * 0.01, i}); nroll += m.sweeps - 1; }
        std::sort(tt.begin(), tt.end());
        if (!tt.empty()) {
            const DMeta &m = c->meta[tt.back().second];
            fprintf(stderr, "wave kernel (WV_PROFILE builds): per-contig us p50 %.0f p90 %.0f p99 %.0f max %.0f; rollbacks %ld; slowest contig %d: V=%d phases=%d sweeps=%d | dma-wait %.1f classes+setup %.1f gather %.1f plan+stage %.1f phases %.1f end+rest %.1f\n",
                    tt[tt.size() / 2].first, tt[tt.size() * 9 / 10].first, tt[tt.size() * 99 / 100].first, tt.back().first, nroll, tt.back().second, m.n_node, m.sssp_iters, m.sweeps,
                    m.pmax[0] * 0.01, m.pmax[1] * 0.01, m.pmax[2] * 0.01, m.pmax[3] * 0.01, m.pmin[0] * 0.01, m.pmin[1] * 0.01);
            const DMeta &q = c->meta[tt[tt.size() / 2].second];
            fprintf(stderr, "  slowest contig: 64-bit phases %u (redone in 128 bits: %u), 128-bit phases %u, base moves %u; median contig: %u (%u), %u, %u\n", m.tr[0], m.tr[1], m.tr[2], m.tr[3], q.tr[0], q.tr[1], q.tr[2], q.tr[3]);
            fprintf(stderr, "  median contig (-DWV_PROFILE_AB): helper-lane maxima summed over phases A %u B %u; phases with more than 4 helpers A %u B %u\n", q.tr[4], q.tr[5], q.tr[6], q.tr[7]);
            fprintf(stderr, "  median contig %d: phases %d: relax %.1f followers %.1f spill %.1f apply %.1f loop %.1f us | setup %.1f gather %.1f plan %.1f window-end %.1f path+genes %.1f\n", tt[tt.size() / 2].second, q.sssp_iters,
                    q.bg[0] * 0.01, q.bg[1] * 0.01, q.bg[2] * 0.01, q.bg[3] * 0.01, q.bg[4] * 0.01, q.pmax[1] * 0.01, q.pmax[2] * 0.01, q.pmax[3] * 0.01, q.pmin[1] * 0.01, q.bg[5] * 0.01);
        }
    }
    if (getenv("PHX_DEBUG_WAVE"))
        for (int i = 0; i < n && i < 4; i++) fprintf(stderr, "wave contig %d: V=%d phases=%d sweeps=%d | dma-wait %.1f classes+setup %.1f gather %.1f plan+stage %.1f phases %.1f end+rest %.1f us\n", i, c->meta[i].n_node, c->meta[i].sssp_iters, c->meta[i].sweeps,
                c->meta[i].pmax[0] * 0.01, c->meta[i].pmax[1] * 0.01, c->meta[i].pmax[2] * 0.01, c->meta[i].pmax[3] * 0.01, c->meta[i].pmin[0] * 0.01, c->meta[i].pmin[1] * 0.01);
    if (getenv("PHX_DEBUG_SSSP"))
        for (int i = 0; i < n && i < 6; i++) fprintf(stderr, "sssp contig %d: V=%d iters=%d sweeps=%d setup=%.1fus iter=%.1fus tail=%.1fus\n", i, c->meta[i].n_node, c->meta[i].sssp_iters, c->meta[i].sweeps, c->meta[i].pmax[0] * 0.01, c->meta[i].pmin[0] * 0.01, c->meta[i].sssp_why * 0.01);
}
#endif

static int enqueue_cert(phx_ctx *c);
int phx_run_async(phx_ctx *c) {
    if (!c) return PHX_E_ARG;
    if (!c->uploaded) return PHX_E_STATE;
    if (!c->have_plan || c->always_sync || c->n == 0) return phx_run(c);
    HIPCHK(c, hipSetDevice(c->device));
    int rc = settle(c);
    if (rc) return rc;
    c->ran = false;
    c->tot_orf = c->tot_grp = c->tot_node = c->tot_edge = 0;
    if ((rc = launch_once(c, false))) return rc;
    c->in_flight = true;
    if (c->certify && c->exact && c->eager_cert) {
        DCaps k;
        current_caps(c, &k);
        if (ensure(c, c->b_eref, ((size_t)k.edge + 16) * sizeof(DERef)) == PHX_OK && enqueue_cert(c) == PHX_OK) c->pend_cert = true;
    }
    return PHX_OK;
}

int phx_wait(phx_ctx *c) {
    if (!c) return PHX_E_ARG;
    HIPCHK(c, hipSetDevice(c->device));
    if (c->in_flight) return settle(c);
    return c->ran ? PHX_OK : PHX_E_STATE;
}

int phx_run(phx_ctx *c) {
    if (!c) return PHX_E_ARG;
    if (!c->uploaded) return PHX_E_STATE;
    HIPCHK(c, hipSetDevice(c->device));
    { const int rs = settle(c); if (rs) return rs; }
    c->ran = false;
    c->tot_orf = c->tot_grp = c->tot_node = c->tot_edge = 0;
    if (c->n == 0) { c->ran = true; return PHX_OK; }
    int rc = run_once(c, !c->have_plan || c->always_sync);
    for (int attempt = 0; rc == kRetry && attempt < 3; attempt++) rc = run_once(c, true);
    if (rc == kRetry) { c->err = "batch layout did not settle"; return PHX_E_STATE; }
    if (rc) return rc;
#ifdef PHX_DEV_REPORT
    dev_report(c);
#endif
    c->ran = true;
    return PHX_OK;
}

static int ensure_gene_stage(phx_ctx *c, size_t n) {
    if (n <= c->h_genes_cap) return PHX_OK;
    if (c->h_genes) HIPCHK(c, hipHostFree(c->h_genes));
    c->h_genes = nullptr; c->h_genes_cap = 0;
    const size_t cap = n + n / 4 + 1024;
    HIPCHK(c, hipHostMalloc((void **)&c->h_genes, cap * sizeof(DGene), hipHostMallocDefault));
    c->h_genes_cap = cap;
    return PHX_OK;
}

static int ensure_exact(phx_ctx *c);

int phx_download(phx_ctx *c, phx_result *out) {
    if (!c || (!out && c->n > 0)) return PHX_E_ARG;
// ... 1403 lines not shown
    return nd;
}

int phx_dump_text(phx_ctx *c, int32_t contig, char **text, int64_t *text_len) {
    if (!c || !text) return PHX_E_ARG;
    *text = nullptr;
    if (text_len) *text_len = 0;
    if (c->in_flight) { const int rs = phx_wait(c); if (rs) return rs; }
    if (!c->ran) return PHX_E_STATE;
    if (contig < 0 || contig >= c->n) return PHX_E_ARG;
    ExactIn in;
    { const int rc = exact_fetch(c, contig, in); if (rc) return rc; }
    std::string out;
    if (in.gl.status >= 0 && !exact_dump(in, c->params, out)) { c->err = "dump: an operation outside what phx_dec.c restates"; return PHX_E_STATE; }
    char *buf = (char *)malloc(out.size() + 1);
    if (!buf) return PHX_E_NOMEM;
    memcpy(buf, out.data(), out.size()); buf[out.size()] = 0;
    *text = buf;
    if (text_len) *text_len = (int64_t)out.size();
    return PHX_OK;
}

int phx_solve(phx_ctx *c, int32_t V, int32_t E, const int32_t *src, const int32_t *dst, const uint64_t *w_limbs, int32_t n_limbs,
              int32_t source, int32_t target, int32_t *path_out, int32_t cap, int32_t *n_path, uint64_t *dist_limbs) {
    if (!c || V < 2 || E < 0 || (E > 0 && (!src || !dst || !w_limbs)) || !n_path) return PHX_E_ARG;
    if (V >= (1 << 29)) return PHX_E_ARG;
    if (!(n_limbs == 2 || n_limbs == 4 || n_limbs == 8 || n_limbs == 17)) return PHX_E_ARG;
    if (source < 0 || source >= V || target < 0 || target >= V || source == target) return PHX_E_ARG;
    HIPCHK(c, hipSetDevice(c->device));
    if (c->in_flight) (void)settle(c);
    *n_path = 0;
    std::vector<int32_t> to_dev((size_t)V), to_user((size_t)V);
    {
        int k = 0;
        for (int v = 0; v < V; v++) if (v != source && v != target) { to_dev[(size_t)v] = k; to_user[(size_t)k] = v; k++; }
        to_dev[(size_t)source] = V - 2; to_user[(size_t)V - 2] = source;
        to_dev[(size_t)target] = V - 1; to_user[(size_t)V - 1] = target;
    }
    std::vector<uint32_t> in_off((size_t)V + 1, 0), esrc((size_t)E);
    std::vector<uint64_t> ewl((size_t)E * (size_t)n_limbs);
    for (int e = 0; e < E; e++) {
        if (src[e] < 0 || src[e] >= V || dst[e] < 0 || dst[e] >= V) return PHX_E_ARG;
        in_off[(size_t)to_dev[(size_t)dst[e]] + 1]++;
    }
    for (int v = 0; v < V; v++) in_off[(size_t)v + 1] += in_off[(size_t)v];
    {
        std::vector<uint32_t> fill(in_off.begin(), in_off.end() - 1);
        for (int e = 0; e < E; e++) {
            uint32_t k = fill[(size_t)to_dev[(size_t)dst[e]]]++;
            esrc[k] = (uint32_t)to_dev[(size_t)src[e]];
            memcpy(&ewl[(size_t)k * (size_t)n_limbs], &w_limbs[(size_t)e * (size_t)n_limbs], (size_t)n_limbs * 8);
        }
    }
    std::vector<uint32_t> ekey((size_t)E);
    {
        std::vector<uint32_t> fill(in_off.begin(), in_off.end() - 1);
        for (int e = 0; e < E; e++) ekey[fill[(size_t)to_dev[(size_t)dst[e]]]++] = (uint32_t)e;
    }
    DMeta m;
    memset(&m, 0, sizeof(m));
    m.n_node = V; m.n_edge = E; m.L = 1; m.sssp_nl = n_limbs; m.sssp_mode = 0;
    int rc;
    DevBuf &b_meta = c->b_meta;
    if ((rc = ensure(c, b_meta, sizeof(DMeta) * 2))) return rc;
    if ((rc = ensure(c, c->b_inoff, ((size_t)V + 2) * 4))) return rc;
    if ((rc = ensure(c, c->b_esrc, ((size_t)E + 1) * 4))) return rc;
    if ((rc = ensure(c, c->b_ekey, ((size_t)E + 1) * 4))) return rc;
    if ((rc = ensure(c, c->b_ew, ((size_t)E + 1) * 8))) return rc;
    if ((rc = ensure(c, c->b_ewl, ((size_t)E + 1) * 8 * (size_t)n_limbs))) return rc;
    if ((rc = ensure(c, c->b_dist, ((size_t)V + 1) * 8 * (size_t)n_limbs))) return rc;
    if ((rc = ensure(c, c->b_parent, ((size_t)V + 1) * 4))) return rc;
    if ((rc = ensure(c, c->b_path, ((size_t)V + 1) * 4))) return rc;
    if ((rc = ensure(c, c->b_tie, (size_t)V * 40 + (size_t)E * 12 + 64))) return rc;
    if ((rc = ensure(c, c->b_tot, sizeof(DTotals)))) return rc;
    c->uploaded = false; c->ran = false;
    hipStream_t s = c->stream;
    HIPCHK(c, hipMemsetAsync(c->b_tot.p, 0, sizeof(DTotals), s));
    HIPCHK(c, hipMemcpyAsync(b_meta.p, &m, sizeof(m), hipMemcpyHostToDevice, s));
    HIPCHK(c, hipMemcpyAsync(c->b_inoff.p, in_off.data(), ((size_t)V + 1) * 4, hipMemcpyHostToDevice, s));
    if (E) {
        HIPCHK(c, hipMemcpyAsync(c->b_esrc.p, esrc.data(), (size_t)E * 4, hipMemcpyHostToDevice, s));
        HIPCHK(c, hipMemcpyAsync(c->b_ekey.p, ekey.data(), (size_t)E * 4, hipMemcpyHostToDevice, s));
        HIPCHK(c, hipMemcpyAsync(c->b_ewl.p, ewl.data(), (size_t)E * 8 * (size_t)n_limbs, hipMemcpyHostToDevice, s));
    }
    DBatch b;
    memset(&b, 0, sizeof(b));
    b.n_contig = 1;
    b.meta = (DMeta *)b_meta.p;
    b.tot = (DTotals *)c->b_tot.p;
    b.in_off = (uint32_t *)c->b_inoff.p; b.esrc = (uint32_t *)c->b_esrc.p; b.ew = (long long *)c->b_ew.p;
    b.ewl = (const uint64_t *)c->b_ewl.p;
    b.ekey = (const uint32_t *)c->b_ekey.p;
    b.dist = (uint64_t *)c->b_dist.p; b.parent = (int32_t *)c->b_parent.p;
    b.path = (int32_t *)c->b_path.p;
    b.tie = (uint8_t *)c->b_tie.p; b.tie_cap = cap_of(c->b_tie, 1, 0);
    b.dist_stride = n_limbs;
    hipLaunchSsspOnly(&b, n_limbs, s);
    HIPCHK(c, hipGetLastError());
    std::vector<int32_t> path((size_t)V);
    std::vector<uint64_t> dt((size_t)n_limbs);
    HIPCHK(c, hipMemcpyAsync(&m, b_meta.p, sizeof(m), hipMemcpyDeviceToHost, s));
    HIPCHK(c, hipMemcpyAsync(path.data(), c->b_path.p, (size_t)V * 4, hipMemcpyDeviceToHost, s));
    HIPCHK(c, hipMemcpyAsync(dt.data(), (uint64_t *)c->b_dist.p + (size_t)(V - 1) * (size_t)n_limbs, (size_t)n_limbs * 8, hipMemcpyDeviceToHost, s));
    HIPCHK(c, hipStreamSynchronize(s));
    if (m.status < 0) return m.status;
    if (m.n_path < 2) return PHX_OK;
    if (m.n_path > cap && path_out) return PHX_E_ARG;
    *n_path = m.n_path;
    if (path_out) for (int k = 0; k < m.n_path; k++) path_out[k] = to_user[(size_t)path[(size_t)k]];
    if (dist_limbs) memcpy(dist_limbs, dt.data(), (size_t)n_limbs * 8);
    return PHX_OK;
}

int phx_set_profiling(phx_ctx *c, int on) {
    if (!c) return PHX_E_ARG;
    c->prof = on != 0;
    c->prof_mask = 0xffffffffu;
    return PHX_OK;
}
int phx_set_profiling_stages(phx_ctx *c, uint32_t stage_mask) {
    if (!c) return PHX_E_ARG;
    c->prof = stage_mask != 0;
    c->prof_mask = stage_mask;
    return PHX_OK;
}
int phx_get_stage_ms(phx_ctx *c, float *ms, int32_t *launches, int reset) {
    if (!c) return PHX_E_ARG;
    for (int i = 0; i < PHX_N_STAGES; i++) { if (ms) ms[i] = c->stage_ms[i]; if (launches) launches[i] = c->stage_n[i]; }
    if (reset) for (int i = 0; i < PHX_N_STAGES; i++) { c->stage_ms[i] = 0; c->stage_n[i] = 0; }
    return PHX_OK;
}
const char *phx_stage_name(int k) { return k >= 0 && k < PHX_N_STAGES ? kStageName[k] : ""; }
int64_t phx_seg_runs(phx_ctx *c) {
    if (!c) return 0;
    if (c->in_flight && phx_wait(c)) return 0;
    return c->seg_runs;
}
int64_t phx_seg_fallbacks(phx_ctx *c) {
    if (!c) return 0;
    if (c->in_flight && phx_wait(c)) return 0;
    return c->seg_fallbacks;
}
int phx_seg_stats(phx_ctx *c, int32_t i, int32_t *out, int32_t cap_records) {
    if (!c || !out) return 0;
    if (c->in_flight && phx_wait(c)) return 0;
    if (i < 0 || i >= c->n || !c->ran || !c->pend_seg || !c->b_segw.p) return 0;
    if (hipSetDevice(c->device) != hipSuccess || hipStreamSynchronize(c->stream) != hipSuccess) return 0;
    const int K = c->pend_seg_k;
    const int n = std::min(K, (int)cap_records);
    if (n <= 0) return 0;
    if (hipMemcpy(out, (const int32_t *)c->b_segw.p + (size_t)i * (size_t)K * 8, (size_t)n * 32, hipMemcpyDeviceToHost) != hipSuccess) return 0;
    return n;
}
int64_t phx_front_runs(phx_ctx *c) {
    if (!c) return PHX_E_ARG;
    if (c->in_flight) { const int rs = phx_wait(c); if (rs) return rs; }
    return c->front_off ? -c->front_runs - 1 : c->front_runs;
}

int64_t phx_plan_timeouts(phx_ctx *c) {
    if (!c) return PHX_E_ARG;
    if (c->in_flight) { const int rs = phx_wait(c); if (rs) return rs; }
    return c->plan_timeouts;
}

int phx_batch_sizes(phx_ctx *c, int64_t *L, int64_t *n_orf, int64_t *n_node, int64_t *n_edge) {
    if (!c) return PHX_E_ARG;
    if (c->in_flight) { const int rs = phx_wait(c); if (rs) return rs; }
    if (L) *L = c->totalL;
    if (n_orf) *n_orf = c->tot_orf;
    if (n_node) *n_node = c->tot_node;
    if (n_edge) *n_edge = c->tot_edge;
    return PHX_OK;
}

}
```

phanotate_amd/csrc/phx_inorder.inc:

```
#define IO_T_FULL 256
#define IO_T_BIG 1024
#ifndef IO_SKIP_T
#define IO_SKIP_T IO_T_BIG
#endif
#define IO_WALK 4096
#define IO_PATH 2048

__device__ __forceinline__ uint64_t node_refkey(const DNode *nd, const DOrf *orf, const DGrp *grp, const DTNode *tn, int v, int V) {
    if (v >= V - 2) return ~0ull - (uint64_t)(V - 1 - v);
    const uint32_t link = nd[v].link;
    if (LINK_KIND(link) == LINK_TRNA) return (0xC0000000ull << 32) | (uint32_t)tn[LINK_IDX(link)].rank;
    uint32_t g, sub;
    if (LINK_KIND(link) == LINK_STOP) { g = LINK_IDX(link); sub = grp[g].frame > 0 ? 1u : 0u; }
    else {
        const uint32_t k = LINK_IDX(link);
        g = (uint32_t)orf[k].grp;
        const uint32_t mth = k - (uint32_t)grp[g].orf_begin;
        sub = grp[g].frame > 0 ? (mth == 0 ? 0u : 1u + mth) : 1u + mth;
    }
    return (((uint64_t)(uint32_t)grp[g].evkey + 1ull) << 32) | sub;
}

template <int IO_T>
struct IoShared {
    int flag, nA, ne, prog, hi, changed, np, fail;
    long long off;
    uint32_t g0;
    uint32_t scan[IO_T / 64 + 1];
    uint32_t e0[IO_T + 1];
    uint32_t ef[IO_T];
    uint32_t pe[IO_T];
    int32_t v[IO_T];
    int32_t wv, wn, wcb, wstate;
    static constexpr int WALK = IO_T >= IO_T_BIG ? 2 * IO_WALK : (IO_T >= IO_T_FULL ? IO_WALK : IO_WALK / 4), PATH = IO_T >= IO_T_FULL ? IO_PATH : IO_PATH / 4;
    int32_t pc[WALK];
    int32_t rpath[PATH];
    static constexpr int SKIP = IO_T >= IO_SKIP_T ? WALK : 1, NCP = IO_T >= IO_SKIP_T ? WALK / 8 + 2 : 1;
    int32_t pj[SKIP];
    int32_t cp[NCP];
};

template <int NL, int IO_T>
__device__ void walk_path(const DBatch &b, DMeta *meta, IoShared<IO_T> *sh) {
    const int tid = threadIdx.x;
    constexpr int WALK = IoShared<IO_T>::WALK, PATH = IoShared<IO_T>::PATH;
    const int V = meta->n_node, SRC = V - 2, TGT = V - 1;
    const uint32_t *esrc = b.esrc + meta->edge_off;
    const int32_t *gpe = b.parent + meta->node_off;
    int32_t *path = b.path + meta->node_off;
    if (tid == 0) { sh->wv = TGT; sh->wn = 0; sh->wcb = V > WALK ? V - WALK : 0; sh->wstate = 1; sh->rpath[0] = TGT; }
    __syncthreads();
    while (sh->wstate == 1) {
        const int cb = sh->wcb;
        for (int i0 = 0; i0 < WALK && cb + i0 < V; i0 += 8 * IO_T) {
            int32_t x[8];
#pragma unroll
            for (int g = 0; g < 8; g++) { const int i = i0 + g * IO_T + tid; x[g] = (i < WALK && cb + i < V) ? gpe[cb + i] : -1; }
#pragma unroll
            for (int g = 0; g < 8; g++) x[g] = x[g] >= 0 ? (int32_t)ESRC_NODE(esrc[x[g]]) : -1;
#pragma unroll
            for (int g = 0; g < 8; g++) { const int i = i0 + g * IO_T + tid; if (i < WALK) sh->pc[i] = x[g]; }
        }
        __syncthreads();
        if constexpr (IO_T >= IO_SKIP_T) {
            if (cb == 0 && V <= WALK) {
                for (int v = tid; v < V; v += IO_T) { const int pv = sh->pc[v]; sh->pj[v] = (v == SRC || pv < 0) ? v : pv; }
                __syncthreads();
                for (int r = 0; r < 3; r++) {
                    int32_t nx[(WALK + IO_T - 1) / IO_T];
                    int k = 0;
                    for (int v = tid; v < V; v += IO_T) nx[k++] = sh->pj[sh->pj[v]];
                    __syncthreads();
                    k = 0;
                    for (int v = tid; v < V; v += IO_T) sh->pj[v] = nx[k++];
                    __syncthreads();
                }
                if (tid == 0) {
                    int v = TGT, k = 0;
                    sh->cp[0] = v;
                    while (v != SRC && k < V / 8 + 1) { v = sh->pj[v]; sh->cp[++k] = v; }
                    sh->np = k;
                    sh->fail = 0;
                }
                __syncthreads();
                const int nst = sh->np;
                if (8 * (nst + 1) < PATH) {
                    bool dead = false;
                    for (int k = tid; k < nst; k += IO_T) {
                        int v = sh->cp[k];
                        for (int h = 1; h <= 8; h++) {
                            if (v == SRC) break;
                            const int pv = sh->pc[v];
                            if (pv < 0) { dead = true; break; }
                            v = pv;
                            sh->rpath[8 * k + h] = v;
                        }
                    }
                    if (dead) sh->fail = 1;
                    __syncthreads();
                    if (tid == 0) {
                        int st = 2, n = 0;
                        if (sh->fail || sh->cp[nst] != SRC) st = 3;
                        else if (nst > 0) {
                            n = 8 * (nst - 1);
                            for (int v = sh->cp[nst - 1]; v != SRC; v = sh->pc[v]) n++;
                        }
                        sh->fail = 0;
                        sh->wv = SRC; sh->wn = n; sh->wstate = st;
                    }
                    __syncthreads();
                    continue;
                }
            }
        }
        if (tid == 0) {
            int v = sh->wv, n = sh->wn, st = 0;
            while (true) {
                if (v == SRC) { st = 2; break; }
                if (v < cb) { sh->wcb = v + 256 > WALK ? v + 256 - WALK : 0; st = 1; break; }
                if (++n >= V) { st = 3; break; }
                v = sh->pc[v - cb];
                if (v < 0) { st = 3; break; }
                if (n < PATH) sh->rpath[n] = v; else path[V - 1 - n] = v;
            }
            sh->wv = v; sh->wn = n; sh->wstate = st;
        }
        __syncthreads();
    }
    const int n = sh->wn;
    if (sh->wstate == 3) { if (tid == 0) meta->n_path = -1; return; }
    if (n >= PATH) {
        __threadfence_block();
        const int shift = V - 1 - n;
        if (shift > 0)
            for (int k0 = 0; k0 <= n - PATH; k0 += IO_T) {
                const int k = k0 + tid;
                int x = 0;
                if (k <= n - PATH) x = path[shift + k];
                __syncthreads();
                if (k <= n - PATH) path[k] = x;
                __syncthreads();
            }
    }
    for (int k = tid; k <= n && k < PATH; k += IO_T) path[n - k] = sh->rpath[k];
    const int np = n / 2;
    if (tid == 0) { const uint32_t g0 = !b.genes ? 0u : (b.gpack ? (uint32_t)(meta->grp_off + meta->tn_off) : atomicAdd(b.gene_total, (uint32_t)np)); sh->g0 = g0; meta->n_path = n + 1; meta->n_genes = b.genes ? np : 0; meta->gene_off = g0; }
    __syncthreads();
    __threadfence_block();
    if (b.genes && np > 0) emit_genes(b, meta, path, np, (size_t)sh->g0, tid, IO_T);
    __syncthreads();
}

template <int NL, int IO_T, bool MASKED = false>
__device__ void inorder_contig(const DBatch &b, DMeta *meta, IoShared<IO_T> *sh, const uint32_t *mask = nullptr) {
    const int tid = threadIdx.x;
    const uint64_t mbase = MASKED ? (uint64_t)meta->edge_off : 0ull;
    auto refused = [&](uint32_t e) -> bool { const uint64_t x = mbase + e; return ((mask[x >> 5] >> (x & 31)) & 1u) != 0; };
    const int V = meta->n_node;
    const bool walked = meta->n_path >= 2;
    const int n = walked ? meta->n_path : 2;
    const uint32_t *in_off = b.in_off + meta->node_off + blockIdx.x;
    const uint32_t *esrc = b.esrc + meta->edge_off;
    const long long *ew = b.ew + meta->edge_off;
    const uint64_t *ewl = b.ewl ? b.ewl + (size_t)meta->edge_off * NL : nullptr;
    const uint32_t *ekey_arr = b.ekey ? b.ekey + meta->edge_off : nullptr;
    const uint64_t *dist = b.dist + (size_t)meta->node_off * b.dist_stride;
    const DNode *nd = b.node ? b.node + meta->node_off : nullptr;
    const DOrf *orf = b.orf ? b.orf + meta->orf_off : nullptr;
    const DGrp *grp = b.grp ? b.grp + meta->grp_off : nullptr;
    const DTNode *tn = b.tnode ? b.tnode + meta->tn_off : nullptr;
    int32_t *path = b.path + meta->node_off;
    const long long *gt = gtab_of(b, meta);
    auto tight = [&](uint32_t e, const WInt<NL> &dv) -> bool {
        if constexpr (MASKED) { if (refused(e)) return false; }
        const uint32_t sw = esrc[e];
        const WInt<NL> du = wi_load<NL>(dist + (size_t)ESRC_NODE(sw) * NL);
        const WInt<NL> w = ewl ? wi_load<NL>(ewl + (size_t)e * NL) : ew_decode<NL>(edge_wenc(sw, ew, e, gt));
        return !wi_unreached<NL>(du) && wi_eq<NL>(wi_add<NL>(du, w), dv);
    };
    const uint32_t *pedge = (const uint32_t *)(b.parent + meta->node_off);
    bool mine = !walked;
    for (int c0 = 1; c0 < n && walked; c0 += IO_T) {
        const int i = c0 + tid;
        uint32_t deg = 0;
        if (i < n) {
            const int v = path[i];
            const uint32_t f = in_off[v];
            deg = in_off[v + 1] - f;
            sh->v[tid] = v; sh->ef[tid] = f; sh->pe[tid] = pedge[v];
        }
        uint32_t total;
        const uint32_t ex = block_excl_scan<IO_T>(deg, sh->scan, &total);
        sh->e0[tid] = ex;
        if (tid == 0) sh->e0[IO_T] = total;
        __syncthreads();
        for (uint32_t f0 = (uint32_t)tid; f0 < total; f0 += 4 * IO_T) {
            uint32_t e[4]; int j[4]; bool on[4];
#pragma unroll
            for (int q = 0; q < 4; q++) {
                const uint32_t f = f0 + (uint32_t)q * IO_T;
                on[q] = f < total;
                int lo = 0, hi = IO_T;
                while (hi - lo > 1) { const int mid = (lo + hi) >> 1; if (sh->e0[mid] <= f) lo = mid; else hi = mid; }
                if (!on[q]) lo = 0;
                j[q] = lo;
                e[q] = sh->ef[lo] + (f - sh->e0[lo]);
                on[q] = on[q] && e[q] != sh->pe[lo];
                if constexpr (MASKED) { if (on[q] && refused(e[q])) on[q] = false; }
            }
            uint32_t u[4]; WInt<NL> w[4];
#pragma unroll
            for (int q = 0; q < 4; q++) {
                const uint32_t ee = on[q] ? e[q] : 0u;
                const uint32_t sw = esrc[ee];
                u[q] = ESRC_NODE(sw);
                w[q] = ewl ? wi_load<NL>(ewl + (size_t)ee * NL) : ew_decode<NL>(edge_wenc(sw, ew, ee, gt));
            }
#pragma unroll
            for (int q = 0; q < 4; q++) {
                const WInt<NL> du = wi_load<NL>(dist + (size_t)u[q] * NL), dv = wi_load<NL>(dist + (size_t)sh->v[j[q]] * NL);
                mine |= on[q] && !wi_unreached<NL>(du) && wi_eq<NL>(wi_add<NL>(du, w[q]), dv);
            }
        }
        __syncthreads();
    }
    if (mine) sh->flag = 1;
    __syncthreads();
    if (!sh->flag) return;

    const size_t sz4 = ((size_t)V * 4 + 7) & ~(size_t)7, E = (size_t)meta->n_edge;
    if (tid == 0) {
        const unsigned long long bytes = ((size_t)V * 8 + 7 * sz4 + E * 12 + 15) & ~(size_t)15;
        const unsigned long long off = atomicAdd((unsigned long long *)&b.tot->tie_need, bytes);
        sh->off = off + bytes <= (unsigned long long)b.tie_cap ? (long long)off : -1;
        if (sh->off < 0) atomicOr(&b.tot->overflow, 4);
        meta->tie = 1;
    }
    __syncthreads();
    if (sh->off < 0) return;
    uint8_t *scr = b.tie + sh->off;
    uint64_t *Tk = (uint64_t *)scr;
    int32_t *amap = (int32_t *)(scr + (size_t)V * 8);
    int32_t *anode = (int32_t *)((uint8_t *)amap + sz4);
    uint32_t *estart = (uint32_t *)((uint8_t *)anode + sz4), *ecnt = (uint32_t *)((uint8_t *)estart + sz4);
    uint32_t *Tr = (uint32_t *)((uint8_t *)ecnt + sz4);
    int32_t *par = (int32_t *)((uint8_t *)Tr + sz4);
    uint32_t *done = (uint32_t *)((uint8_t *)par + sz4);
    uint64_t *ek = (uint64_t *)((uint8_t *)done + sz4);
    int32_t *eu = (int32_t *)(ek + E);

    for (int v = tid; v < V; v += IO_T) amap[v] = -1;
    __syncthreads();
    for (int i = tid; i < n; i += IO_T) { const int v = walked ? path[i] : (i == 0 ? V - 2 : V - 1); anode[i] = v; amap[v] = i; }
    if (tid == 0) { sh->nA = n; sh->ne = 0; }
    __syncthreads();
    for (int lo = 0, hi = n; lo < hi;) {
        for (int a = lo + tid; a < hi; a += IO_T) {
            const int x = anode[a];
            const WInt<NL> dv = wi_load<NL>(dist + (size_t)x * NL);
            const uint32_t e0 = in_off[x], e1 = in_off[x + 1];
            int c = 0;
            for (uint32_t e = e0; e < e1; e++) c += tight(e, dv) ? 1 : 0;
            int k = atomicAdd(&sh->ne, c);
            estart[a] = (uint32_t)k; ecnt[a] = (uint32_t)c;
            for (uint32_t e = e0; e < e1; e++)
                if (tight(e, dv)) {
                    const int u = (int)ESRC_NODE(esrc[e]);
                    eu[k] = u;
                    ek[k] = ekey_arr ? (uint64_t)ekey_arr[e] + 1ull : node_refkey(nd, orf, grp, tn, u, V);
                    k++;
                    if (atomicCAS(&amap[u], -1, -2) == -1) { const int idx = atomicAdd(&sh->nA, 1); anode[idx] = u; amap[u] = idx; }
                }
        }
        __syncthreads();
        lo = hi; hi = sh->nA;
        __syncthreads();
    }
    const int nA = sh->nA, ne = sh->ne;
    for (int k = tid; k < ne; k += IO_T) eu[k] = amap[eu[k]];
    for (int a = tid; a < nA; a += IO_T) { done[a] = a == 0 ? 1u : 0u; Tr[a] = 0; Tk[a] = 0; par[a] = -1; }
    if (tid == 0) { sh->fail = 0; sh->changed = 0; }
    __syncthreads();

    const int tgt = n - 1;
    for (uint32_t iter = 1;; iter++) {
        if (tid == 0) sh->prog = 0;
        __syncthreads();
        for (int a = tid; a < nA; a += IO_T) {
            if (done[a] || !ecnt[a]) continue;
            bool all = true;
            uint32_t br = ~0u; uint64_t bk = ~0ull; int bu = -1;
            for (uint32_t k = estart[a], k1 = k + ecnt[a]; k < k1; k++) {
                const int u = eu[k];
                const uint32_t d = done[u];
                if (d == 0 || d > iter) { all = false; break; }
                const uint32_t r = Tr[u] + (ek[k] < Tk[u] ? 1u : 0u);
                if (r < br || (r == br && ek[k] < bk)) { br = r; bk = ek[k]; bu = u; }
            }
            if (all) { Tr[a] = br; Tk[a] = bk; par[a] = bu; done[a] = iter + 1; sh->prog = 1; }
        }
        __syncthreads();
        const bool fin = done[tgt] != 0, prog = sh->prog != 0;
        __syncthreads();
        if (fin) break;
        if (!prog) {
            if (tid == 0) {
                uint32_t br = ~0u; uint64_t bk = ~0ull; int bu = -1, ba = -1;
                for (int a = 0; a < nA; a++) {
                    if (done[a]) continue;
                    for (uint32_t k = estart[a], k1 = k + ecnt[a]; k < k1; k++) {
                        const int u = eu[k];
                        if (!done[u]) continue;
                        const uint32_t r = Tr[u] + (ek[k] < Tk[u] ? 1u : 0u);
                        if (r < br || (r == br && ek[k] < bk)) { br = r; bk = ek[k]; bu = u; ba = a; }
                    }
                }
                if (ba < 0) sh->fail = 1;
                else { Tr[ba] = br; Tk[ba] = bk; par[ba] = bu; done[ba] = iter + 1; }
            }
            __syncthreads();
            if (sh->fail) break;
        }
        if (iter > 2u * (uint32_t)nA + 8u) { if (tid == 0) sh->fail = 1; __syncthreads(); break; }
    }
    if (sh->fail) { if (tid == 0) { meta->tie = -1; if (!walked) { meta->status = PHX_S_NEGCYCLE; meta->n_path = 0; } } return; }

    if (tid == 0) {
        int m = 0;
        bool same = true;
        for (int a = tgt; a != 0 && m <= nA; a = par[a]) m++;
        if (m > nA) { sh->fail = 1; meta->tie = -1; if (!walked) { meta->status = PHX_S_NEGCYCLE; meta->n_path = 0; } }
        else {
            same = walked && m == n - 1;
            if (same) { int j = n - 1; for (int a = tgt; a != 0; a = par[a], j--) if (a != j) { same = false; break; } }
            if (!same) {
                int k = m;
                for (int a = tgt;; a = par[a]) { path[k--] = anode[a]; if (a == 0) break; }
                meta->n_path = m + 1;
                const int np = m / 2;
                uint32_t g0 = (uint32_t)meta->gene_off;
                if (b.genes && np > meta->n_genes && !b.gpack) g0 = atomicAdd(b.gene_total, (uint32_t)np);
                meta->gene_off = g0; meta->n_genes = b.genes ? np : 0;
                sh->np = np; sh->g0 = g0; sh->changed = 1;
                meta->tie = 2;
            }
        }
    }
    __syncthreads();
    if (sh->changed && b.genes) {
        __threadfence_block();
        emit_genes(b, meta, path, sh->np, (size_t)sh->g0, tid, IO_T);
    }
}

template <int NL, int IO_T>
__global__ __launch_bounds__(IO_T) void k_inorder(DBatch b) {
    __shared__ IoShared<IO_T> sh;
    if (b.tot->overflow & 3) return;
    DMeta *meta = &b.meta[blockIdx.x];
    if (meta->sssp_nl != NL) return;
    if (threadIdx.x == 0) { sh.flag = 0; meta->tie = 0; }
    __syncthreads();
    if (meta->status < 0 || (meta->n_node <= 2 && !b.ewl)) return;
    if (meta->n_path == -2) walk_path<NL, IO_T>(b, meta, &sh);
    __syncthreads();
    if (meta->n_path < 2 && meta->n_path != -1) return;
    inorder_contig<NL, IO_T>(b, meta, &sh);
}
```

phanotate_amd/csrc/phx_internal.h:

```cpp
#pragma once
#include <hip/hip_runtime.h>
#include <stdint.h>

#include "../../include/phx.h"

#define PHX_TILE 1536
#define PHX_CTG_THREADS 256
#define PHX_N_CODON_BITMAPS 12
#define PHX_PLANE_GCF 4
#define PHX_PLANE_GCR 7
#define PHX_PLANE_ATG 10
#define PHX_PRE_G 2
#define PHX_BITMAP_WORDS_PER_NW (PHX_N_CODON_BITMAPS * 3)

#define CLS_NONE 0
#define CLS_FS 1
#define CLS_RS 2
#define CLS_FT 3
#define CLS_RT 4

#define ESRC_F_GAP 0x20000000u
#define ESRC_GAP_NODES (1 << 19)
#define ESRC_IS_GAP(x) (((x) >> 29) & 1u)
#define ESRC_GAP_CODE(x) (((x) >> 19) & 1023u)
#define ESRC_GAP_WORD(src, code) ((uint32_t)(src) | ESRC_F_GAP | ((uint32_t)(code) << 19))
static inline __host__ __device__ uint32_t esrc_node(uint32_t x) { return x & ((x & ESRC_F_GAP) ? 0x7ffffu : 0x1fffffffu); }
#define ESRC_NODE(x) esrc_node(x)
#define GT_SAME 500
#define GT_DIFF 303
#define GT_N 808
#define ESRC_INEXACT(x) ((x) >> 31)
#define ESRC_OFFPATH(x) (((x) >> 30) & 1u)
#define ESRC_F_INEXACT 0x80000000u
#define ESRC_F_OFFPATH 0x40000000u

#define LINK_NONE 0u
#define LINK_START (1u << 30)
#define LINK_STOP (2u << 30)
#define LINK_TRNA (3u << 30)
#define LINK_IDX(x) ((x)&0x3fffffffu)
#define LINK_KIND(x) ((x)&0xc0000000u)

#define NINFO(type, frame) ((int32_t)(((uint32_t)(type)&3u) | (((uint32_t)(uint8_t)(int8_t)(frame)) << 8)))
#define NTYPE(i) ((i)&3)
#define NFRAME(i) ((int)(int8_t)(((uint32_t)(i) >> 8) & 0xff))

struct DParams {
    int32_t minlen;
    int32_t n_start;
    double start_w[PHX_MAX_CODONS];
    uint8_t cls_tab[72];
    uint8_t atg_tab[72];
    double sw_hi[PHX_MAX_CODONS], sw_lo[PHX_MAX_CODONS];
};

struct DOrf {
    int32_t start, stop;
    int8_t frame;
    uint8_t pad[2];
    uint8_t flags;
    int32_t grp;
};
struct DOrfStat {
    uint16_t hist[9];
    uint8_t rbs;
    int8_t startidx;
    uint8_t flags;
    uint8_t pad[3];
    double pstop;
};

struct DGrp {
    int32_t stop;
    int32_t orf_begin;
    int32_t n;
    int32_t node;
    int32_t frame;
    int32_t evkey;
    int32_t pick;
    int32_t pad0;
};
static_assert(sizeof(DGrp) == 32, "group record");

struct DBridge {
    int32_t last, base;
};

struct DTNode {
    int32_t pos;
    int32_t info;
    int32_t other;
    int32_t rank;
};
struct DTEdge {
    int32_t src, dst;
};

struct DMeta {
    int64_t off;
    int32_t L;
    int32_t status;
    uint32_t gc;
    uint32_t bg[28];
    uint32_t tr[28];
    uint32_t pmax[4];
    uint32_t pmin[4];
    int32_t n_orf, n_grp;
    int64_t orf_off, grp_off;
    int32_t n_node;
    int32_t n_edge;
    int64_t node_off, edge_off;
    int32_t n_bridge;
    int32_t maxexp;
    int64_t bridge_off;
    int32_t bridge_cap;
    int32_t n_win;
    int32_t n_genes;
    int32_t n_path;
    int64_t gene_off;
    int32_t sweeps;
    int32_t nw;
    int64_t bits_off;
    int64_t item_off;
    int64_t cb_off;
    int32_t ncw;
    int32_t sssp_fb;
    int64_t nbits_off;
    int32_t n_orf_main, n_grp_main;
    int32_t sssp_nl;
    int32_t sssp_iters;
    int32_t sssp_why;
    int32_t sssp_mode;
    int32_t n_open;
    int32_t dense;
    double wsum;
    int64_t win_off;
    int32_t n_tnode, n_tedge;
    int64_t tn_off, te_off;
    int32_t tie;
    int32_t cert;
    int32_t plan_prog;
    int32_t seg_fail;
    int64_t rec_off;
};

struct DRes {
    int32_t status, n_genes;
    int64_t gene_off;
    int32_t cert, tie;
};

struct DERef {
    double d1, d2, err;
};

struct DGene {
    int32_t left, right, strand, frame;
    double score;
};

struct DNode {
    int32_t pos;
    int32_t info;
    uint32_t link;
    int32_t other;
};

struct DWin {
    int32_t v0, va, v1;
    uint32_t e0;
    uint32_t ne;
    uint32_t pa, pb;
    uint32_t sp;
};
#define WIN_ROLES 128

struct DTotals {
    int64_t orf, grp, node, cb, edge;
    int32_t nlmax;
    int32_t class_mask;
    int32_t vmax;
    int32_t overflow;
    int64_t lds_need[4];
    int64_t tie_need;
    int32_t plan_timeouts;
    int32_t front_abort;
    uint32_t gsync;
    int32_t seg_abort;
    int32_t seg_fallbacks;
    int32_t pad_t2;
};
struct DCaps {
    int64_t orf, grp, node, cb, edge;
    int64_t win;
    int32_t limbs;
    int32_t flags;
};

struct DBatch {
    int32_t n_contig;
    int64_t mean_len;
    DMeta *meta;
    DTotals *tot;
    DRes *res;
    int32_t *sord;
    int64_t *lpart;
    DCaps caps;
    const DParams *params;
    uint32_t *recs;
    const uint32_t *voff;
    const uint32_t *wfirst;
    uint32_t vtotal;
    int32_t defcod;
    uint64_t *nbits;
    uint32_t *nbase;
    uint64_t *cbits;
    uint64_t *bits;
    int32_t *iprev;
    uint2 *item;
    const DTNode *tnode;
    const DTEdge *tedge;
    int32_t *tnid;
    uint32_t *cpre, *bpre;
    uint64_t *tbits;
    DBridge *bridge;
    DOrf *orf;
    DOrfStat *ostat;
    double *oweight;
    long long *owi;
    uint8_t *oflag;
    int32_t *onode;
    DGrp *grp;
    DNode *node;
    int32_t *parent;
    uint32_t *in_off;
    double *no;
    int32_t *npos;
    DWin *win;
    uint2 *wrole;
    int32_t *olist;
    int4 *erank;
    uint64_t *ehit;
    uint32_t *mreach;
    uint64_t *dist;
    int32_t dist_stride;
    uint32_t *esrc;
    long long *ew;
    int32_t orf_rows;
    int32_t gap_code;
    long long *gtab;
    uint16_t *gtabf;
    uint32_t *esrcf;
    double *ewf;
    const uint64_t *ewl;
    const uint32_t *ekey;
    uint8_t *tie;
    int64_t tie_cap;
    int32_t *cint;
    uint64_t *csig;
    DERef *eref;
    double cert_scale;
    int32_t defer_overlap;
    int32_t *path;
    DGene *genes;
    uint32_t *gene_total;
    int32_t duo;
    int32_t plan_stream;
    int32_t seg;
    int32_t seg_margin_bp;
    int32_t seg_stream;
    int32_t segw_ints;
    int32_t seg_nofb;
    DWin *swin;
    uint2 *swrole;
    uint64_t *sdist;
    int64_t sdist_nodes;
    int32_t *segw;
    int32_t front_spins;
    int32_t gpack;
    DGene *genes_c;
};

struct DMarg {
    uint32_t *out_off;
    uint32_t *out_dst;
    long long *out_w;
    uint64_t *dist_t;
    phx_orf_margin *rec;
    int32_t *mstat;
};

#define DP_TAB_LDS 4096
struct DDrop {
    int32_t *pidx;
    int32_t *js, *jt;
    int32_t *first, *last;
    uint64_t *slot;
    uint64_t *gtab;
    const int64_t *toff;
    const int64_t *roff;
    uint64_t *sx, *cx;
    uint64_t *da, *db;
    phx_gene_drop *rec;
    unsigned long long *stats;
    int32_t layered;
    int32_t *ps, *ts;
};
struct DRepl {
    uint64_t *win;
    int32_t *xs;
    int64_t *coff;
    int32_t *cm;
    int32_t *chain;
    int64_t ccap;
    int32_t *rnd;
    int32_t *info;
    const int64_t *doff, *goff;
    int32_t *det;
    phx_gene *genes;
    phx_gene_repl *rec;
    unsigned long long *cnt;
};

struct DReannRec {
    int32_t status, n_genes;
    int64_t gene_off;
    double delta;
    int32_t n_path, tie;
};
struct DReann {
    const uint8_t *forb;
    uint32_t *mask;
    const int32_t *sel;
    uint8_t *gplan;
    const uint64_t *dist0;
    DReannRec *rec;
};

#ifdef __cplusplus
extern "C" {
#endif
void phx_pack_planes(const char *in, int64_t n, uint32_t *out, int64_t nrec);
void phxk_features(const DBatch *b, uint32_t v_begin, uint32_t v_end, void *stream);
void phxk_features_tap(const DBatch *b, int contig, uint32_t v_begin, uint32_t v_end, uint32_t *tapbuf, void *stream);
void phxk_pack_planes(const DBatch *b, const void *letters, void *stream);
void phxk_orf_count(const DBatch *b, void *stream);
void phxk_orf_emit(const DBatch *b, void *stream);
void phxk_bit_prefix(const DBatch *b, void *stream);
void phxk_orf_stats(const DBatch *b, void *stream);
void phxk_score(const DBatch *b, void *stream);
void phxk_nodes(const DBatch *b, void *stream);
void phxk_node_attr(const DBatch *b, void *stream);
void phxk_edges_count(const DBatch *b, void *stream);
void phxk_layout1(const DBatch *b, void *stream);
void phxk_layout2(const DBatch *b, void *stream);
void phxk_edges_fill(const DBatch *b, void *stream);
void phxk_edges_orf(const DBatch *b, void *stream);
void phxk_edges_expand(const DBatch *b, int n_limbs, int mode, void *stream);
void phxk_edges_tap(const DBatch *b, void *stream);
void phxk_sssp_order(const DBatch *b, void *stream);
size_t phxk_sssp_lds_bytes(int V, int n_limbs);
void phxk_wave_plan(const DBatch *b, int wide_too, void *stream);
int phxk_sssp_wave_ok(int n_limbs);
void phxk_sssp(const DBatch *b, int n_limbs, int mode, size_t lds_bytes, void *stream);
void phxk_inorder(const DBatch *b, int nl_mask, void *stream);
void phxk_refine(const DBatch *b, void *stream);
void phxk_certify(const DBatch *b, int nl_mask, int vmax, void *stream);
void phxk_gene_pack(const DBatch *b, void *stream);
void phxk_reset(const DBatch *b, const void *meta0, unsigned long long nbits_words, unsigned long long tbits_words, void *stream);
int phxk_front_blocks_y(const DBatch *b);
void phxk_front(const DBatch *b, void *stream);
void phxk_seg_merge(const DBatch *b, int vmax, void *stream);
int phxk_seg_kmax(void);
void phxk_seg_fallback(const DBatch *b, void *stream);
void phxk_results(const DBatch *b, void *stream);
void phxk_margins_transpose(const DBatch *b, const DMarg *g, void *stream);
void phxk_sssp_rev(const DBatch *b, const DMarg *g, int nl_mask, void *stream);
void phxk_margins(const DBatch *b, const DMarg *g, int nl_mask, void *stream);
void phxk_drop_trees(const DBatch *b, const DMarg *g, const DDrop *q, int nl_mask, void *stream);
void phxk_drop_cand(const DBatch *b, const DMarg *g, const DDrop *q, int nl_mask, void *stream);
void phxk_drop_fix(const DBatch *b, const DMarg *g, const DDrop *q, int nl_mask, void *stream);
void phxk_repl_pick(const DBatch *b, const DMarg *g, const DDrop *q, const DRepl *r, int nl_mask, void *stream);
void phxk_repl_cross(const DBatch *b, const DMarg *g, const DDrop *q, const DRepl *r, int nl_mask, void *stream);
void phxk_repl_walk(const DBatch *b, const DMarg *g, const DDrop *q, const DRepl *r, int fill, void *stream);
void phxk_reann_mask(const DBatch *b, const DReann *q, void *stream);
void phxk_reann_solve(const DBatch *b, const DReann *q, int nl_mask, void *stream);
void phxk_reann_finish(const DBatch *b, const DReann *q, int nl_mask, void *stream);
#ifdef __cplusplus
}
#endif
```

phanotate_amd/csrc/phx_kernels.hip:

```cpp
#include <hip/hip_runtime.h>
#include <type_traits>

#include "phx_internal.h"

#define NT PHX_CTG_THREADS

__device__ __forceinline__ uint32_t wave_incl_scan(uint32_t v) {
    const int lane = threadIdx.x & 63;
#pragma unroll
    for (int d = 1; d < 64; d <<= 1) {
        uint32_t t = __shfl_up(v, d);
        if (lane >= d) v += t;
    }
    return v;
}
__device__ __forceinline__ uint32_t wave_incl_max(uint32_t v) {
    const int lane = threadIdx.x & 63;
#pragma unroll
    for (int d = 1; d < 64; d <<= 1) {
        uint32_t t = __shfl_up(v, d);
        if (lane >= d) v = v > t ? v : t;
    }
    return v;
}
template <int N>
__device__ __forceinline__ uint32_t block_excl_scan(uint32_t v, uint32_t *lds, uint32_t *total) {
    const int lane = threadIdx.x & 63, w = threadIdx.x >> 6;
    uint32_t inc = wave_incl_scan(v);
    if (lane == 63) lds[w] = inc;
    __syncthreads();
    if (threadIdx.x == 0) {
        uint32_t s = 0;
        for (int i = 0; i < N / 64; i++) { uint32_t t = lds[i]; lds[i] = s; s += t; }
        lds[N / 64] = s;
    }
    __syncthreads();
    uint32_t r = inc - v + lds[w];
    *total = lds[N / 64];
    __syncthreads();
    return r;
}
template <int N>
__device__ __forceinline__ uint32_t block_excl_max(uint32_t v, uint32_t *lds, uint32_t *total) {
    const int lane = threadIdx.x & 63, w = threadIdx.x >> 6;
    uint32_t inc = wave_incl_max(v);
    if (lane == 63) lds[w] = inc;
    __syncthreads();
    if (threadIdx.x == 0) {
        uint32_t s = 0;
        for (int i = 0; i < N / 64; i++) { uint32_t t = lds[i]; lds[i] = s; s = s > t ? s : t; }
        lds[N / 64] = s;
    }
    __syncthreads();
    uint32_t prev = __shfl_up(inc, 1);
    if (lane == 0) prev = 0;
    uint32_t r = prev > lds[w] ? prev : lds[w];
    *total = lds[N / 64];
    __syncthreads();
    return r;
}

template <int N>
__device__ __forceinline__ uint32_t dpp_row_shr(uint32_t x) { return (uint32_t)__builtin_amdgcn_update_dpp((int)x, (int)x, 0x110 + N, 0xf, 0xf, false); }
template <int N>
__device__ __forceinline__ uint64_t dpp_row_shr64(uint64_t x) { return ((uint64_t)dpp_row_shr<N>((uint32_t)(x >> 32)) << 32) | dpp_row_shr<N>((uint32_t)x); }
__device__ __forceinline__ uint64_t row16_sum_u64(uint64_t x, int sub) {
    uint64_t y;
    y = dpp_row_shr64<1>(x); if (sub >= 1) x += y;
    y = dpp_row_shr64<2>(x); if (sub >= 2) x += y;
    y = dpp_row_shr64<4>(x); if (sub >= 4) x += y;
    y = dpp_row_shr64<8>(x); if (sub >= 8) x += y;
    return x;
}

#define EW_WIDE(x) (((((unsigned long long)(x)) >> 63) ^ (((unsigned long long)(x)) >> 62)) & 1ull)
__device__ __forceinline__ long long ew_encode(double w) {
    const double t = trunc(w * 1000.0);
    if (fabs(t) < 2251799813685248.0) return __double_as_longlong(t + 6755399441055744.0) - 0x4338000000000000ll;
    if (fabs(t) < 4611686018427387904.0) return (long long)t;
    const long long bits = __double_as_longlong(t);
    return bits < 0 ? (bits & ~(1ll << 62)) : bits;
}
__device__ __forceinline__ bool ew_narrow51(long long w) { return (unsigned long long)(w + (1ll << 51)) < (1ull << 52); }
__device__ __forceinline__ bool cert_eps_is_zero_fast(double w, double c) {
#ifdef EW_NOCHECK
    return true;
#endif
    const double p = w * 1000.0, a = fabs(p);
    const double f = a - fabs(trunc(p));
    const bool far = (f < 1.0 - f ? f : 1.0 - f) > a * (60.0 * c);
    return w == -20.0 || (a < 4503599627370496.0 && far);
}
#define CERT_C(b) ((b).cert_scale * 1.4210854715202004e-14)
struct EWt { unsigned long long bits; uint32_t fl; int code; };
template <bool TAPW>
__device__ __forceinline__ EWt make_ew(double w, double c) {
    EWt r;
    r.code = -1;
    if (TAPW) { r.bits = (unsigned long long)__double_as_longlong(w); r.fl = 0u; }
    else {
        r.bits = (unsigned long long)ew_encode(w);
        r.fl = (cert_eps_is_zero_fast(w, c) ? 0u : ESRC_F_INEXACT) | (ew_narrow51((long long)r.bits) ? 0u : ESRC_F_OFFPATH);
    }
    return r;
}

__device__ __forceinline__ long long edge_wenc(uint32_t sw, const long long *ew, uint32_t e, const long long *gt) { return ESRC_IS_GAP(sw) ? gt[ESRC_GAP_CODE(sw)] : ew[e]; }
__device__ __forceinline__ const long long *gtab_of(const DBatch &b, const DMeta *meta) { return b.gtab ? b.gtab + (size_t)(meta - b.meta) * GT_N : nullptr; }

__device__ __forceinline__ double contig_pstop(uint32_t gc, int L) {
    double fa = (double)((uint32_t)L - gc), fg = (double)gc;
    double d = (double)((int64_t)L * 2);
    double Pa = fa / d, Pt = fa / d, Pg = fg / d;
    return Pt * Pa * Pa + Pt * Pg * Pa + Pt * Pa * Pg;
}
__device__ __forceinline__ int max_idx(int a, int b, int c) { return a > b ? (a > c ? 1 : 3) : (b > c ? 2 : 3); }
__device__ __forceinline__ int min_idx(int a, int b, int c) { return a > b ? (b > c ? 3 : 2) : (a > c ? 3 : 1); }

#include "phx_features.inc"
#include "phx_orf.inc"
#include "phx_graph.inc"
#include "phx_sssp.inc"
#include "phx_layout.inc"
#include "phx_front.inc"
#include "phx_sssp_seg.inc"
#include "phx_sssp_wave.inc"
#include "phx_sssp_duo.inc"
#include "phx_inorder.inc"
#include "phx_refine.inc"
#include "phx_certify.inc"
#include "phx_margins.inc"
#include "phx_drop.inc"
#include "phx_replace.inc"
#include "phx_resolve.inc"

template <int NL>
static void launch_certify(const DBatch *b, int vcap, hipStream_t s) {
    const size_t lds = (size_t)vcap * 12 + 16;
    if (lds > 48 * 1024) (void)hipFuncSetAttribute((const void *)k_certify<NL>, hipFuncAttributeMaxDynamicSharedMemorySize, (int)lds);
    hipLaunchKernelGGL(k_certify<NL>, dim3(b->n_contig), dim3(CERT_T), lds, s, *b, vcap);
    hipLaunchKernelGGL(k_certify_wide<NL>, dim3(b->n_contig), dim3(CERT_T), 0, s, *b);
}
extern "C" {
void phxk_features(const DBatch *b, uint32_t v_begin, uint32_t v_end, void *stream) {
    if (v_end <= v_begin) return;
    const unsigned g = (v_end - 1) / FEAT_SPAN - v_begin / FEAT_SPAN + 1;
    if (b->defcod) hipLaunchKernelGGL((k_features<false, true>), dim3(g), dim3(64), 0, (hipStream_t)stream, *b, v_begin, v_end, (uint32_t *)nullptr, -1);
    else hipLaunchKernelGGL((k_features<false, false>), dim3(g), dim3(64), 0, (hipStream_t)stream, *b, v_begin, v_end, (uint32_t *)nullptr, -1);
}
void phxk_features_tap(const DBatch *b, int contig, uint32_t v_begin, uint32_t v_end, uint32_t *tapbuf, void *stream) {
    if (v_end <= v_begin) return;
    const unsigned g = (v_end - 1) / FEAT_SPAN - v_begin / FEAT_SPAN + 1;
    hipLaunchKernelGGL((k_features<true, false>), dim3(g), dim3(64), 0, (hipStream_t)stream, *b, v_begin, v_end, tapbuf, contig);
}
void phxk_pack_planes(const DBatch *b, const void *letters, void *stream) {
    if (b->n_contig > 0) hipLaunchKernelGGL(k_pack_planes, dim3(b->n_contig, 8), dim3(64), 0, (hipStream_t)stream, *b, (const uint8_t *)letters);
}
#ifndef YS_EMIT
#define YS_EMIT 6
#endif
#ifndef YS_STATS
#define YS_STATS 8
#endif
static unsigned ysplit(const DBatch *b, unsigned full) {
    const unsigned y = (unsigned)((b->mean_len + 8191) / 8192);
    const unsigned cap = (unsigned)b->n_contig * 4u * full <= 256u ? 4u * full : full;
    return y < 1u ? 1u : (y > cap ? cap : y);
}
void phxk_orf_count(const DBatch *b, void *stream) {
    if (b->mean_len < 16384) hipLaunchKernelGGL((k_orf<false, 256>), dim3(b->n_contig), dim3(256), 0, (hipStream_t)stream, *b);
    else hipLaunchKernelGGL((k_orf<false, ORF_COUNT_T>), dim3(b->n_contig), dim3(ORF_COUNT_T), 0, (hipStream_t)stream, *b);
}
void phxk_orf_emit(const DBatch *b, void *stream) { hipLaunchKernelGGL(k_orf<true>, dim3(b->n_contig, ysplit(b, YS_EMIT)), dim3(NT), 0, (hipStream_t)stream, *b); }
void phxk_bit_prefix(const DBatch *b, void *stream) {
    hipLaunchKernelGGL(k_bit_prefix, dim3(b->n_contig, 7), dim3(64), 0, (hipStream_t)stream, *b);
    hipLaunchKernelGGL(k_gap_table, dim3(b->n_contig), dim3(NT), 0, (hipStream_t)stream, *b);
}
void phxk_orf_stats(const DBatch *b, void *stream) { hipLaunchKernelGGL(k_orf_stats, dim3(b->n_contig, ysplit(b, YS_STATS)), dim3(NT), 0, (hipStream_t)stream, *b); }
void phxk_score(const DBatch *b, void *stream) {
    if (b->n_contig <= 16 && b->mean_len >= 32768) { hipLaunchKernelGGL(k_score_big, dim3(b->n_contig), dim3(1024), 0, (hipStream_t)stream, *b); return; }
    hipLaunchKernelGGL(k_score, dim3(b->n_contig), dim3(b->mean_len >= 8192 ? NT : 64), 0, (hipStream_t)stream, *b);
}
void phxk_nodes(const DBatch *b, void *stream) {
#ifndef NODES_STAGED
    if (!(b->n_contig <= 16 && b->mean_len >= 32768)) {
        hipLaunchKernelGGL(k_nodes_fused, dim3(b->n_contig), dim3(NT), 0, (hipStream_t)stream, *b);
        return;
    }
#endif
    hipLaunchKernelGGL(k_node_cov, dim3(b->n_contig, ysplit(b, 4)), dim3(NT), 0, (hipStream_t)stream, *b);
    hipLaunchKernelGGL(k_node_rank, dim3(b->n_contig), dim3(NT), 0, (hipStream_t)stream, *b);
    hipLaunchKernelGGL(k_node_build, dim3(b->n_contig, ysplit(b, 4)), dim3(NT), 0, (hipStream_t)stream, *b);
    hipLaunchKernelGGL(k_node_order, dim3(b->n_contig), dim3(NT), 0, (hipStream_t)stream, *b);
}
void phxk_node_attr(const DBatch *b, void *stream) { hipLaunchKernelGGL(k_node_attr, dim3(b->n_contig, ysplit(b, 4)), dim3(NT), 0, (hipStream_t)stream, *b); }
void phxk_edges_count(const DBatch *b, void *stream) {
    hipLaunchKernelGGL(k_edges<false>, dim3(b->n_contig, ysplit(b, 4)), dim3(NT), 0, (hipStream_t)stream, *b);
    if (b->n_contig <= 16 && b->mean_len >= 32768) hipLaunchKernelGGL(k_edges_scan_big, dim3(b->n_contig), dim3(1024), 0, (hipStream_t)stream, *b);
    else hipLaunchKernelGGL(k_edges_scan, dim3(b->n_contig), dim3(ES_T), 0, (hipStream_t)stream, *b);
}
void phxk_edges_fill(const DBatch *b, void *stream) {
    if (b->gap_code) hipLaunchKernelGGL((k_edges<true, false, true>), dim3(b->n_contig, ysplit(b, 4)), dim3(NT), 0, (hipStream_t)stream, *b);
    else hipLaunchKernelGGL(k_edges<true>, dim3(b->n_contig, ysplit(b, 4)), dim3(NT), 0, (hipStream_t)stream, *b);
}
void phxk_edges_orf(const DBatch *b, void *stream) { hipLaunchKernelGGL(k_edges_orf, dim3(b->n_contig, ysplit(b, 4)), dim3(NT), 0, (hipStream_t)stream, *b); }
void phxk_edges_expand(const DBatch *b, int nl, int mode, void *stream) { hipLaunchKernelGGL(k_edges_expand, dim3(b->n_contig, ysplit(b, 4)), dim3(NT), 0, (hipStream_t)stream, *b, nl, mode); }
void phxk_edges_tap(const DBatch *b, void *stream) { hipLaunchKernelGGL((k_edges<true, true>), dim3(b->n_contig, ysplit(b, 4)), dim3(NT), 0, (hipStream_t)stream, *b); }
void phxk_sssp_only(const DBatch *b, int nl, void *stream) {
    phxk_sssp(b, nl, 0, 0, stream);
    phxk_inorder(b, nl == 2 ? 1 : nl == 4 ? 2 : nl == 8 ? 4 : 8, stream);
}

void phxk_inorder(const DBatch *b, int nl_mask, void *stream) {
    dim3 g(b->n_contig);
    hipStream_t s = (hipStream_t)stream;
    const bool small = b->mean_len < 8192;
    const bool big = (b->n_contig <= 64 && b->mean_len >= 65536) || (b->n_contig <= 8 && b->mean_len >= 16384);
    if (big && (nl_mask & 1)) { hipLaunchKernelGGL((k_inorder<2, IO_T_BIG>), g, dim3(IO_T_BIG), 0, s, *b); nl_mask &= ~1; }
    if (small) {
        if (nl_mask & 1) hipLaunchKernelGGL((k_inorder<2, 64>), g, dim3(64), 0, s, *b);
        if (nl_mask & 2) hipLaunchKernelGGL((k_inorder<4, 64>), g, dim3(64), 0, s, *b);
        if (nl_mask & 4) hipLaunchKernelGGL((k_inorder<8, 64>), g, dim3(64), 0, s, *b);
        if (nl_mask & 8) hipLaunchKernelGGL((k_inorder<17, 64>), g, dim3(64), 0, s, *b);
    } else {
        if (nl_mask & 1) hipLaunchKernelGGL((k_inorder<2, IO_T_FULL>), g, dim3(IO_T_FULL), 0, s, *b);
        if (nl_mask & 2) hipLaunchKernelGGL((k_inorder<4, IO_T_FULL>), g, dim3(IO_T_FULL), 0, s, *b);
        if (nl_mask & 4) hipLaunchKernelGGL((k_inorder<8, IO_T_FULL>), g, dim3(IO_T_FULL), 0, s, *b);
        if (nl_mask & 8) hipLaunchKernelGGL((k_inorder<17, IO_T_FULL>), g, dim3(IO_T_FULL), 0, s, *b);
    }
}

void phxk_certify(const DBatch *b, int nl_mask, int vmax, void *stream) {
    hipStream_t s = (hipStream_t)stream;
    int vcap = ((vmax > 1024 ? vmax : 1024) + 255) & ~255;
    if (vcap > 12288) vcap = 12288;
    if (vmax < 0) vcap = 0;
    if (nl_mask & 1) launch_certify<2>(b, vcap, s);
    if (nl_mask & 2) launch_certify<4>(b, vcap, s);
    if (nl_mask & 4) launch_certify<8>(b, vcap, s);
    if (nl_mask & 8) launch_certify<17>(b, vcap, s);
}

void phxk_refine(const DBatch *b, void *stream) {
    const unsigned y = b->n_contig <= 16 ? ysplit(b, 4) : 1u;
    hipLaunchKernelGGL(k_refine, dim3(b->n_contig, y), dim3(RF_T), 0, (hipStream_t)stream, *b);
}

void phxk_gene_pack(const DBatch *b, void *stream) {
    const unsigned g = (unsigned)((b->n_contig + LMB_T - 1) / LMB_T);
    hipLaunchKernelGGL(k_gene_pack_a, dim3(g), dim3(LMB_T), 0, (hipStream_t)stream, *b);
    hipLaunchKernelGGL(k_gene_pack_b, dim3(g, 8), dim3(LMB_T), 0, (hipStream_t)stream, *b);
}
void phxk_reset(const DBatch *b, const void *meta0, unsigned long long nbits_words, unsigned long long tbits_words, void *stream) {
    unsigned long long work = nbits_words / 2 + tbits_words / 2 + (unsigned long long)b->n_contig * (sizeof(DMeta) / 8);
    unsigned g = (unsigned)((work + 255) / 256);
    g = g < 1u ? 1u : (g > 4096u ? 4096u : g);
    hipLaunchKernelGGL(k_reset, dim3(g), dim3(256), 0, (hipStream_t)stream, *b, (const DMeta *)meta0, nbits_words, tbits_words);
}
int phxk_front_blocks_y(const DBatch *b) {
    if (b->n_contig < 1 || b->n_contig > FRONT_MAX_CONTIGS || b->mean_len * b->n_contig > (40 << 10)) return 0;
    unsigned y = ysplit(b, 8);
    while (y > 1 && (unsigned)b->n_contig * y > FRONT_MAX_BLOCKS) y--;
    return (unsigned)b->n_contig * y <= FRONT_MAX_BLOCKS ? (int)y : 0;
}
void phxk_front(const DBatch *b, void *stream) {
    const int y = phxk_front_blocks_y(b);
    if (y > 0) hipLaunchKernelGGL(k_front, dim3(b->n_contig, y), dim3(NT), 0, (hipStream_t)stream, *b);
}
void phxk_seg_merge(const DBatch *b, int vmax, void *stream) {
    const int n = b->n_contig > 0 ? b->n_contig : 1;
    int y = vmax > 0 ? (vmax + SEGJ_T / SEGJ_LPN - 1) / (SEGJ_T / SEGJ_LPN) : 64;
    const int cap = 4096 / n;
    y = y > cap ? cap : y;
    y = y < 4 ? 4 : y;
    hipLaunchKernelGGL(k_seg_join, dim3(b->n_contig, y), dim3(SEGJ_T), 0, (hipStream_t)stream, *b);
    hipLaunchKernelGGL(k_seg_close, dim3(b->n_contig), dim3(SEGM_T), 0, (hipStream_t)stream, *b);
}
int phxk_seg_kmax(void) { return SEG_KMAX; }
void phxk_seg_fallback(const DBatch *b, void *stream) {
    hipLaunchKernelGGL((k_wave_plan<2, 0>), dim3(b->n_contig), dim3(64), 0, (hipStream_t)stream, *b);
    hipLaunchKernelGGL((k_sssp_duo<0, false>), dim3(b->n_contig), dim3(128), 0, (hipStream_t)stream, *b);
// ... 170 lines not shown
```

phanotate_amd/csrc/phx_sssp_duo.inc:

```

template <int CFG> struct DuoDims;
template <> struct DuoDims<0> { static constexpr int RING = 512, OV = 192, MODE = 2; };
#define DUO_SLOTS 20
#ifndef DUO_GT_LDS
#define DUO_GT_LDS 0
#endif
template <int CFG>
constexpr size_t duo_lds_bytes() {
    typedef DuoDims<CFG> D;
    return (DUO_GT_LDS ? (size_t)GT_N * 4 : 0) + (size_t)(D::RING + 2) * 16 + (size_t)(D::RING + 2) * 8 + (size_t)DUO_SLOTS * 64 * 8 + (size_t)(DUO_SLOTS / 2) * 64 * 4 + 2 * 64 * 4 +
           (size_t)WIN_ROLES * 8 + (size_t)D::OV * 20 + 64 + 64;
}
static_assert(DUO_GT_LDS || 4 * duo_lds_bytes<0>() + 40 * 1024 + 64 <= 160 * 1024, "k_sssp_duo, tight configuration: a 40 KB workgroup fits beside four contigs per CU");

#define DUO_P_READY 0
#define DUO_C_ACK 1
#define DUO_C_CMD 2
#define DUO_C_LOADED 3
#define DUO_C_DONE 4
#define DUO_C_EXIT 5
#define DUO_GO 6
#define DUO_NWIN 7
#define DUO_H_V0 0
#define DUO_H_VA 1
// ... 714 lines not shown
            const bool any = __ballot(chg) != 0;
            if (__ballot(widen)) wide = true;
            return any;
        };
        uint64_t again_mask = 0;
        auto phase64 = [&](Role &R, auto capc, const CW *cw, const uint32_t *cs) -> bool {
            constexpr int cap = decltype(capc)::value;
            uint64_t mm = 0x7000000000000000ull;
            const long long d0 = *(const long long *)(rel + R.slot / NL);
            uint64_t x[cap];
#pragma unroll
            for (int t = 0; t < cap; t++) x[t] = *(const uint64_t *)(rel + cs[t] / NL);
#pragma unroll
            for (int t = 0; t < cap; t++) x[t] += (uint64_t)cw[t];
#pragma unroll
            for (int w = 1; w < cap; w <<= 1)
#pragma unroll
                for (int t = 0; t + w < cap; t += 2 * w) x[t] = min64(x[t], x[t + w]);
            mm = min64(mm, x[0]);
            int e = R.ebase + (int)(mm & 15u);
            long long m = (long long)mm >> 4;
            if (R.maxfollow > 0 && R.maxfollow <= 4) {
                for (int q = 0; q < R.maxfollow; q++) {
                    const long long c = (long long)(((uint64_t)(uint32_t)wv_next_self((int)((uint64_t)m >> 32)) << 32) | (uint32_t)wv_next_self((int)m));
                    const int ce = wv_next_self(e);
                    const bool l = R.nextf && c < m;
                    m = l ? c : m;
                    e = l ? ce : e;
                }
            } else if (R.maxfollow > 0) {
                for (int st = 1; st <= R.maxfollow; st <<= 1) {
                    const int src = (lane + st) & 63;
                    const int och = __shfl(R.node >= 0 ? R.ch : 0, src);
                    const long long c = (long long)(((uint64_t)(uint32_t)__shfl((int)((uint64_t)m >> 32), src) << 32) | (uint32_t)__shfl((int)m, src));
                    const int ce = __shfl(e, src);
                    const bool l = lane + st < 64 && och >= st && c < m;
                    m = l ? c : m;
                    e = l ? ce : e;
                }
            }
            if (has_spill) {
                for (int i = R.sp0; i < R.sp1; i++) {
                    const long long c0 = (long long)((*(const uint64_t *)(ov_w + (size_t)i * NL * 8) << 4) + *(const uint64_t *)(rel + ov_s[i] / NL)) >> 4;
                    const bool l = c0 < m;
                    m = l ? c0 : m;
                    e = l ? R.spe + (i - R.sp0) : e;
                }
            }
            const bool again = R.head && m >= WV_BIAS + WV_NARROW && m < WV_BIAS + WV_VAL_BIG - (1ll << 52);
            const bool store = R.head && m < WV_BIAS + WV_NARROW && m < (d0 >> 4);
            const long long v = m - WV_BIAS;
            const bool fits = v > -WV_NARROW;
            R.pe = R.head ? e : R.pe;
            if (store) {
                N::store(ring + R.slot, N::add(base, N::from_i64(v)));
                *(long long *)(rel + R.slot / NL) = fits ? (long long)((uint64_t)m << 4) : WV_REL_WIDE;
            }
            const uint64_t cm = __ballot(store);
            again_mask = __ballot(again);
            wv_sync();
            if (cm && __ballot(store && !fits)) wide = true;
            return cm != 0;
        };
        {
            int inner = 0;
#ifdef DUO_PROFILE_AB
            long long tmark_ab = wall_clock64();
#endif
            for (int ph = 0;; ph ^= 1) {
                bool chg = false;
                const bool n64 = narrow_w && !wide;
                if (n64) chg = ph ? phase64(B, std::integral_constant<int, CB>(), cwB, csB) : phase64(A, std::integral_constant<int, CA>(), cwA, csA);
                const bool exact = !n64 || again_mask != 0;
                if (exact) chg |= ph ? phase(B, std::integral_constant<int, CB>(), cwB, csB) : phase(A, std::integral_constant<int, CA>(), cwA, csA);
                phases++;
#ifdef DUO_PROFILE_AB
                { const long long t_ = wall_clock64(); tab[ph ? 1 : 0] += t_ - tmark_ab; tmark_ab = t_; nab[ph ? 1 : 0]++; if (exact) nab[2]++; }
#endif
                if (!chg && (ph == 1 || inner > 0)) break;
                if (++inner > 4 * WV_WIN + 16) { fail = true; fail_code = 3; break; }
            }
            if (fail) break;
        }
        DUO_TICK(2)
        if (lane == 0) duo_poke(&mb[DUO_C_DONE], (uint32_t)seq);

        pend_dv = v0 + lane < va ? v0 + lane : -1;
        pend_d = N::load(ring + (size_t)((v0 + lane) & (WV_RING - 1)) * NL * 8);
        auto parents = [&](Role &R, int &pv, int &pe) {
            pv = (R.head && v0 + R.node < va) ? v0 + R.node : -1;
            pe = (pv >= 0 && pv != SRC && R.pe >= 0 && !N::unreached(N::load(ring + (R.head ? R.slot : ZERO)))) ? (int)(e0 + (uint32_t)R.pe) : -1;
        };
        parents(A, pend_av, pend_ae);
        parents(B, pend_bv, pend_be);

        const bool trig = A.head && A.watch && N::lt(N::load(ring + A.slot), a_old);
        const uint64_t tm = __ballot(trig);
        if (tm) {
            if (++rollbacks > 4 * (V / WV_ADV + 4)) { fail = true; fail_code = 4; break; }
            uint32_t mr = trig ? b.mreach[4 * (size_t)meta->node_off + (size_t)(v0 + A.node)] : ~0u;
            for (int st = 32; st >= 1; st >>= 1) { const uint32_t o = (uint32_t)__shfl_xor((int)mr, st); mr = o < mr ? o : mr; }
            int rr = (int)mr < v0 ? (int)mr : v0;
            if (meta->dense & 2) {
                const DNode *nd = b.node + meta->node_off;
                const int tl = __ffsll((long long)tm) - 1;
                const int xpos = nd[v0 + __shfl(A.node, tl)].pos;
                rr = v0;
                while (rr > 0) {
                    const int q = rr - 1 - lane;
                    const bool aff = q >= 0 && nd[q].pos > xpos - 500;
                    const uint64_t am = __ballot(aff);
                    if (am == ~0ull) { rr -= 64; continue; }
                    rr -= am ? (__ffsll((long long)~am) - 1) : 0;
                    break;
                }
            }
            if (rr < seg_ns) rr = seg_ns;
            pend_rr = rr;
            continue;
        }
        if (last) break;
    }
    if (lane == 0) duo_poke(&mb[DUO_C_EXIT], 1u);
    if (abandoned) return;
    flush_results();
    if constexpr (SEG) {
        if (lane == 0) {
            seg_rec[1] = fail ? (fail_code ? fail_code : 7) : 0; atomicAdd(&meta->sssp_iters, phases);
            seg_rec[4] = (int32_t)(wall_clock64() - seg_t0); seg_rec[5] = phases; seg_rec[6] = seq; seg_rec[7] = rollbacks;
            if (fail && fail_code == 5) atomicAdd(&b.tot->plan_timeouts, 1);
        }
        return;
    }
    if (fail) {
        if (lane == 0) {
            if (fail_code == 5) { if (atomicCAS(&meta->sssp_mode, D::MODE, meta->sssp_fb) == D::MODE) { meta->sssp_why = 5; atomicAdd(&b.tot->plan_timeouts, 1); } }
            else if (STREAM) { if (atomicCAS(&meta->sssp_mode, D::MODE, meta->sssp_fb) == D::MODE) meta->sssp_why = fail_code; }
            else { meta->sssp_mode = meta->sssp_fb; meta->sssp_why = fail_code; }
        }
        return;
    }
    if (lane == 0) {
        meta->sweeps = 1 + rollbacks;
#ifdef DUO_PROFILE
        DUO_TICK(3)
        for (int q_ = 0; q_ < 4; q_++) meta->pmax[q_] = (uint32_t)tp[q_];
        meta->bg[6] = (uint32_t)(wall_clock64() - t_begin); meta->bg[7] = (uint32_t)seq;
#ifdef DUO_PROFILE_AB
        meta->bg[0] = (uint32_t)tab[0]; meta->bg[1] = (uint32_t)tab[1]; meta->bg[2] = (uint32_t)nab[0]; meta->bg[3] = (uint32_t)nab[1]; meta->bg[4] = (uint32_t)nab[2];
#endif
#endif
        meta->sssp_iters = phases;
        meta->n_genes = 0; meta->gene_off = 0;
        if (N::unreached(N::load(ring + (size_t)((V - 1) & (WV_RING - 1)) * NL * 8))) { meta->status = PHX_S_NOPATH; meta->n_path = 0; }
        else meta->n_path = -2;
    }
}
```

Baseline: 32700 Mbp/s.

## Fuse path walk and in-order tie check into duo SSSP kernel tail

When the single-wavefront duo SSSP finishes, it now walks the parent chain, emits genes and runs the tie check in place, reusing the ring LDS as scratch. Contigs that pass the check are marked so the separate k_inorder kernel skips them. This is meant to remove a kernel launch and the extra global-memory round trip for most contigs. In exchange the duo kernel holds its wavefront longer, and a one-wave walk with larger walk buffers may be slower per contig than the 256-thread block.

```diff
diff --git a/include/phx.h b/include/phx.h
--- a/include/phx.h
+++ b/include/phx.h
@@ -130,6 +130,7 @@
 #define PHX_CREATE_CERT_WIDE 128u
 #define PHX_CREATE_NO_DUO 4096u
 #define PHX_CREATE_NO_SEG 8192u
+#define PHX_CREATE_NO_DUO_TAIL 16384u
 #define PHX_CREATE_NO_FUSE 2048u
 #define PHX_CREATE_NO_EXACT 1024u
 int phx_create_ex(const phx_params *params, int device, void *stream, uint32_t flags, phx_ctx **out);
@@ -222,6 +223,7 @@
 int64_t phx_front_runs(phx_ctx *ctx);
 int64_t phx_seg_runs(phx_ctx *ctx);
 int64_t phx_seg_fallbacks(phx_ctx *ctx);
+int64_t phx_tail_contigs(phx_ctx *ctx);
 int phx_seg_stats(phx_ctx *ctx, int32_t i, int32_t *out, int32_t cap_records);
 int phx_batch_sizes(phx_ctx *ctx, int64_t *L, int64_t *n_orf, int64_t *n_node, int64_t *n_edge);
 
diff --git a/phanotate_amd/_lib.py b/phanotate_amd/_lib.py
--- a/phanotate_amd/_lib.py
+++ b/phanotate_amd/_lib.py
@@ -156,6 +156,7 @@
         "phx_front_runs": (C.c_int64, [vp]),
         "phx_seg_runs": (C.c_int64, [vp]),
         "phx_seg_fallbacks": (C.c_int64, [vp]),
+        "phx_tail_contigs": (C.c_int64, [vp]),
         "phx_seg_stats": (C.c_int, [vp, C.c_int32, C.c_void_p, C.c_int32]),
         "phx_synth_contig": (C.c_int, [C.c_uint64, i64, C.c_char_p]),
         "phx_fasta_read": (C.c_int, [C.c_char_p, P(vp)]),
@@ -181,7 +182,7 @@
 EXPORTS = ["phx_version", "phx_device_count", "phx_strerror", "phx_last_error", "phx_default_params", "phx_params_from_flags", "phx_set_exact", "phx_pool_create", "phx_pool_destroy", "phx_pool_last_error", "phx_pool_annotate", "phx_dump_text", "phx_dec_eval", "phx_dd_eval", "phx_dd_shortest", "phx_create", "phx_create_ex", "phx_destroy",
            "phx_annotate", "phx_free_results", "phx_upload", "phx_attach", "phx_set_trnas", "phx_run", "phx_run_async", "phx_wait", "phx_download", "phx_download_flat", "phx_certified", "phx_tap_globals",
            "phx_tap_positions", "phx_tap_orfs", "phx_tap_nodes", "phx_tap_edges", "phx_tap_path", "phx_tap_dist", "phx_solve", "phx_set_profiling", "phx_set_profiling_stages",
-           "phx_get_stage_ms", "phx_stage_name", "phx_batch_sizes", "phx_plan_timeouts", "phx_front_runs", "phx_seg_runs", "phx_seg_fallbacks", "phx_seg_stats", "phx_synth_contig", "phx_fasta_read", "phx_fasta_count",
+           "phx_get_stage_ms", "phx_stage_name", "phx_batch_sizes", "phx_plan_timeouts", "phx_front_runs", "phx_seg_runs", "phx_seg_fallbacks", "phx_tail_contigs", "phx_seg_stats", "phx_synth_contig", "phx_fasta_read", "phx_fasta_count",
            "phx_fasta_record", "phx_fasta_arrays", "phx_fasta_free", "phx_format_tabular", "phx_free_text",
            "phx_margins_flat", "phx_tap_dist_target", "phx_margins_ms", "phx_format_margins",
            "phx_drop_margins_flat", "phx_drop_ms", "phx_drop_stats", "phx_format_drops",
diff --git a/phanotate_amd/api.py b/phanotate_amd/api.py
--- a/phanotate_amd/api.py
+++ b/phanotate_amd/api.py
@@ -84,7 +84,7 @@
 
 class Annotator:
 
-    FLAGS = {"no_graph": 2, "size_every_run": 4, "solver_global": 8, "solver_no_wave": 16, "no_certify": 32, "cert_tight": 64, "cert_wide": 128, "poison": 256, "one_stream": 512, "no_exact": 1024, "no_fuse": 2048, "no_duo": 4096, "no_seg": 8192}
+    FLAGS = {"no_graph": 2, "size_every_run": 4, "solver_global": 8, "solver_no_wave": 16, "no_certify": 32, "cert_tight": 64, "cert_wide": 128, "poison": 256, "one_stream": 512, "no_exact": 1024, "no_fuse": 2048, "no_duo": 4096, "no_seg": 8192, "no_duo_tail": 16384}
 
     def __init__(self, params=None, device=0, stream=None, flags=()):
         self.L = _lib.lib()
@@ -492,6 +492,9 @@
     def seg_fallbacks(self):
         return int(self.L.phx_seg_fallbacks(self.h))
 
+    def tail_contigs(self):
+        return int(self.L.phx_tail_contigs(self.h))
+
     def seg_stats(self, i):
         import numpy as np
 
diff --git a/phanotate_amd/csrc/phx_api.cpp b/phanotate_amd/csrc/phx_api.cpp
--- a/phanotate_amd/csrc/phx_api.cpp
+++ b/phanotate_amd/csrc/phx_api.cpp
@@ -194,6 +194,8 @@
     bool pend_front = false;
     bool front_off = false;
     int64_t front_runs = 0;
+    bool duo_tail = true;
+    int64_t tail_contigs = 0;
     bool seg_on = true;
     bool seg_off = false;
     bool seg_never = false;
@@ -626,7 +628,7 @@
 int phx_create(const phx_params *params, int device, void *stream, phx_ctx **out) { return phx_create_ex(params, device, stream, stream ? PHX_CREATE_USE_STREAM : 0u, out); }
 
 int phx_create_ex(const phx_params *params, int device, void *stream, uint32_t flags, phx_ctx **out) {
-    if (!out || (flags & ~(PHX_CREATE_USE_STREAM | PHX_CREATE_NO_GRAPH | PHX_CREATE_SIZE_EVERY_RUN | PHX_CREATE_SOLVER_GLOBAL | PHX_CREATE_SOLVER_NO_WAVE | PHX_CREATE_NO_CERTIFY | PHX_CREATE_CERT_TIGHT | PHX_CREATE_CERT_WIDE | PHX_CREATE_POISON | PHX_CREATE_ONE_STREAM | PHX_CREATE_NO_EXACT | PHX_CREATE_NO_FUSE | PHX_CREATE_NO_DUO | PHX_CREATE_NO_SEG)) || (stream && !(flags & PHX_CREATE_USE_STREAM))) return PHX_E_ARG;
+    if (!out || (flags & ~(PHX_CREATE_USE_STREAM | PHX_CREATE_NO_GRAPH | PHX_CREATE_SIZE_EVERY_RUN | PHX_CREATE_SOLVER_GLOBAL | PHX_CREATE_SOLVER_NO_WAVE | PHX_CREATE_NO_CERTIFY | PHX_CREATE_CERT_TIGHT | PHX_CREATE_CERT_WIDE | PHX_CREATE_POISON | PHX_CREATE_ONE_STREAM | PHX_CREATE_NO_EXACT | PHX_CREATE_NO_FUSE | PHX_CREATE_NO_DUO | PHX_CREATE_NO_SEG | PHX_CREATE_NO_DUO_TAIL)) || (stream && !(flags & PHX_CREATE_USE_STREAM))) return PHX_E_ARG;
     *out = nullptr;
     int rc = check_params(params);
     if (rc) return rc;
@@ -652,6 +654,7 @@
     { const char *e = getenv("PHX_ORF_STREAM"); if (e && *e) { const int v = atoi(e); if (v >= -1 && v <= 3) c->orf_stream = v; } }
     { const char *e = getenv("PHX_NO_SIDE_SCORE"); c->side_score = !(e && e[0] == '1'); }
     { const char *e = getenv("PHX_NO_DUO"); c->duo = !(flags & PHX_CREATE_NO_DUO) && !(e && e[0] == '1'); }
+    { const char *e = getenv("PHX_NO_DUO_TAIL"); c->duo_tail = !(flags & PHX_CREATE_NO_DUO_TAIL) && !(e && e[0] == '1'); }
     { const char *e = getenv("PHX_NO_SEG"); c->seg_on = !(flags & PHX_CREATE_NO_SEG) && !(e && e[0] == '1'); }
     { const char *e = getenv("PHX_SEG_MAX_N"); if (e && atoi(e) >= 0) c->seg_max_n = atoi(e); }
     { const char *e = getenv("PHX_SEG_MARGIN_BP"); if (e && atoi(e) > 0) c->seg_margin_bp = atoi(e); }
@@ -1089,6 +1092,7 @@
     b.seg_stream = (b.seg && !head_done && !learn && c->n <= 4 && !c->plan_stream_off && !c->one_stream && c->aux[3]) ? 1 : 0;
     const bool stream_plan = stream_k >= 0;
     b.duo = (c->duo && c->n <= c->n_simd) ? 1 : 0;
+    b.duo_tail = c->duo_tail ? 1 : 0;
     b.plan_stream = stream_k < 0 ? 0 : (2 << stream_k);
     b.defer_overlap = c->max_len < (1 << 21) ? 1 : 0;
     auto launch_plan = [&]() -> int {
@@ -1274,6 +1278,7 @@
     memcpy(c->h_tot, (const void *)(c->res + (size_t)c->n), sizeof(DTotals));
     const DTotals *ht = c->h_tot;
     c->tie_seen = std::max(c->tie_seen, ht->tie_need);
+    c->tail_contigs = ht->tail_contigs;
 #ifdef FRONT_PROFILE
     if (getenv("PHX_DEBUG_FRONT")) {
         int64_t st[40];
@@ -2983,6 +2988,11 @@
     if (hipMemcpy(out, (const int32_t *)c->b_segw.p + (size_t)i * (size_t)K * 8, (size_t)n * 32, hipMemcpyDeviceToHost) != hipSuccess) return 0;
     return n;
 }
+int64_t phx_tail_contigs(phx_ctx *c) {
+    if (!c) return 0;
+    if (c->in_flight && phx_wait(c)) return 0;
+    return c->tail_contigs;
+}
 int64_t phx_front_runs(phx_ctx *c) {
     if (!c) return PHX_E_ARG;
     if (c->in_flight) { const int rs = phx_wait(c); if (rs) return rs; }
diff --git a/phanotate_amd/csrc/phx_inorder.inc b/phanotate_amd/csrc/phx_inorder.inc
--- a/phanotate_amd/csrc/phx_inorder.inc
+++ b/phanotate_amd/csrc/phx_inorder.inc
@@ -21,7 +21,27 @@
     return (((uint64_t)(uint32_t)grp[g].evkey + 1ull) << 32) | sub;
 }
 
-template <int IO_T>
+template <bool WAVE>
+__device__ __forceinline__ void io_sync() {
+    if constexpr (WAVE) {
+        __builtin_amdgcn_fence(__ATOMIC_RELEASE, "workgroup");
+        __builtin_amdgcn_wave_barrier();
+        __builtin_amdgcn_fence(__ATOMIC_ACQUIRE, "workgroup");
+    } else __syncthreads();
+}
+template <int IO_T, bool WAVE>
+__device__ __forceinline__ uint32_t io_excl_scan(uint32_t v, uint32_t *lds, uint32_t *total) {
+    if constexpr (WAVE) {
+        static_assert(IO_T == 64, "one wavefront");
+        const uint32_t inc = wave_incl_scan(v);
+        *total = (uint32_t)__builtin_amdgcn_readlane((int)inc, 63);
+        return inc - v;
+    } else return block_excl_scan<IO_T>(v, lds, total);
+}
+
+#define IO_TAIL_WALK 2048
+#define IO_TAIL_PATH 512
+template <int IO_T, bool WAVE = false>
 struct IoShared {
     int flag, nA, ne, prog, hi, changed, np, fail;
     long long off;
@@ -32,7 +52,7 @@
     uint32_t pe[IO_T];
     int32_t v[IO_T];
     int32_t wv, wn, wcb, wstate;
-    static constexpr int WALK = IO_T >= IO_T_BIG ? 2 * IO_WALK : (IO_T >= IO_T_FULL ? IO_WALK : IO_WALK / 4), PATH = IO_T >= IO_T_FULL ? IO_PATH : IO_PATH / 4;
+    static constexpr int WALK = WAVE ? IO_TAIL_WALK : (IO_T >= IO_T_BIG ? 2 * IO_WALK : (IO_T >= IO_T_FULL ? IO_WALK : IO_WALK / 4)), PATH = WAVE ? IO_TAIL_PATH : (IO_T >= IO_T_FULL ? IO_PATH : IO_PATH / 4);
     int32_t pc[WALK];
     int32_t rpath[PATH];
     static constexpr int SKIP = IO_T >= IO_SKIP_T ? WALK : 1, NCP = IO_T >= IO_SKIP_T ? WALK / 8 + 2 : 1;
@@ -40,16 +60,16 @@
     int32_t cp[NCP];
 };
 
-template <int NL, int IO_T>
-__device__ void walk_path(const DBatch &b, DMeta *meta, IoShared<IO_T> *sh) {
+template <int NL, int IO_T, bool WAVE = false>
+__device__ int walk_path(const DBatch &b, DMeta *meta, IoShared<IO_T, WAVE> *sh) {
     const int tid = threadIdx.x;
-    constexpr int WALK = IoShared<IO_T>::WALK, PATH = IoShared<IO_T>::PATH;
+    constexpr int WALK = IoShared<IO_T, WAVE>::WALK, PATH = IoShared<IO_T, WAVE>::PATH;
     const int V = meta->n_node, SRC = V - 2, TGT = V - 1;
     const uint32_t *esrc = b.esrc + meta->edge_off;
     const int32_t *gpe = b.parent + meta->node_off;
     int32_t *path = b.path + meta->node_off;
     if (tid == 0) { sh->wv = TGT; sh->wn = 0; sh->wcb = V > WALK ? V - WALK : 0; sh->wstate = 1; sh->rpath[0] = TGT; }
-    __syncthreads();
+    io_sync<WAVE>();
     while (sh->wstate == 1) {
         const int cb = sh->wcb;
         for (int i0 = 0; i0 < WALK && cb + i0 < V; i0 += 8 * IO_T) {
@@ -61,19 +81,19 @@
 #pragma unroll
             for (int g = 0; g < 8; g++) { const int i = i0 + g * IO_T + tid; if (i < WALK) sh->pc[i] = x[g]; }
         }
-        __syncthreads();
+        io_sync<WAVE>();
         if constexpr (IO_T >= IO_SKIP_T) {
             if (cb == 0 && V <= WALK) {
                 for (int v = tid; v < V; v += IO_T) { const int pv = sh->pc[v]; sh->pj[v] = (v == SRC || pv < 0) ? v : pv; }
-                __syncthreads();
+                io_sync<WAVE>();
                 for (int r = 0; r < 3; r++) {
                     int32_t nx[(WALK + IO_T - 1) / IO_T];
                     int k = 0;
                     for (int v = tid; v < V; v += IO_T) nx[k++] = sh->pj[sh->pj[v]];
-                    __syncthreads();
+                    io_sync<WAVE>();
                     k = 0;
                     for (int v = tid; v < V; v += IO_T) sh->pj[v] = nx[k++];
-                    __syncthreads();
+                    io_sync<WAVE>();
                 }
                 if (tid == 0) {
                     int v = TGT, k = 0;
@@ -82,7 +102,7 @@
                     sh->np = k;
                     sh->fail = 0;
                 }
-                __syncthreads();
+                io_sync<WAVE>();
                 const int nst = sh->np;
                 if (8 * (nst + 1) < PATH) {
                     bool dead = false;
@@ -97,7 +117,7 @@
                         }
                     }
                     if (dead) sh->fail = 1;
-                    __syncthreads();
+                    io_sync<WAVE>();
                     if (tid == 0) {
                         int st = 2, n = 0;
                         if (sh->fail || sh->cp[nst] != SRC) st = 3;
@@ -108,7 +128,7 @@
                         sh->fail = 0;
                         sh->wv = SRC; sh->wn = n; sh->wstate = st;
                     }
-                    __syncthreads();
+                    io_sync<WAVE>();
                     continue;
                 }
             }
@@ -125,10 +145,10 @@
             }
             sh->wv = v; sh->wn = n; sh->wstate = st;
         }
-        __syncthreads();
+        io_sync<WAVE>();
     }
     const int n = sh->wn;
-    if (sh->wstate == 3) { if (tid == 0) meta->n_path = -1; return; }
+    if (sh->wstate == 3) { if (tid == 0) meta->n_path = -1; return -1; }
     if (n >= PATH) {
         __threadfence_block();
         const int shift = V - 1 - n;
@@ -137,29 +157,95 @@
                 const int k = k0 + tid;
                 int x = 0;
                 if (k <= n - PATH) x = path[shift + k];
-                __syncthreads();
+                io_sync<WAVE>();
                 if (k <= n - PATH) path[k] = x;
-                __syncthreads();
+                io_sync<WAVE>();
             }
     }
     for (int k = tid; k <= n && k < PATH; k += IO_T) path[n - k] = sh->rpath[k];
     const int np = n / 2;
     if (tid == 0) { const uint32_t g0 = !b.genes ? 0u : (b.gpack ? (uint32_t)(meta->grp_off + meta->tn_off) : atomicAdd(b.gene_total, (uint32_t)np)); sh->g0 = g0; meta->n_path = n + 1; meta->n_genes = b.genes ? np : 0; meta->gene_off = g0; }
-    __syncthreads();
+    io_sync<WAVE>();
     __threadfence_block();
     if (b.genes && np > 0) emit_genes(b, meta, path, np, (size_t)sh->g0, tid, IO_T);
-    __syncthreads();
+    io_sync<WAVE>();
+    return n + 1;
+}
+
+template <int NL, int IO_T, bool MASKED = false, bool WAVE = false>
+__device__ bool inorder_check(const DBatch &b, const DMeta *meta, IoShared<IO_T, WAVE> *sh, const int n_path, const uint32_t *mask = nullptr) {
+    const int tid = threadIdx.x;
+    const uint64_t mbase = MASKED ? (uint64_t)meta->edge_off : 0ull;
+    auto refused = [&](uint32_t e) -> bool { const uint64_t x = mbase + e; return ((mask[x >> 5] >> (x & 31)) & 1u) != 0; };
+    const bool walked = n_path >= 2;
+    const int n = walked ? n_path : 2;
+    const uint32_t *in_off = b.in_off + meta->node_off + (meta - b.meta);
+    const uint32_t *esrc = b.esrc + meta->edge_off;
+    const long long *ew = b.ew + meta->edge_off;
+    const uint64_t *ewl = b.ewl ? b.ewl + (size_t)meta->edge_off * NL : nullptr;
+    const uint64_t *dist = b.dist + (size_t)meta->node_off * b.dist_stride;
+    const int32_t *path = b.path + meta->node_off;
+    const long long *gt = gtab_of(b, meta);
+    const uint32_t *pedge = (const uint32_t *)(b.parent + meta->node_off);
+    bool mine = !walked;
+    for (int c0 = 1; c0 < n && walked; c0 += IO_T) {
+        const int i = c0 + tid;
+        uint32_t deg = 0;
+        if (i < n) {
+            const int v = path[i];
+            const uint32_t f = in_off[v];
+            deg = in_off[v + 1] - f;
+            sh->v[tid] = v; sh->ef[tid] = f; sh->pe[tid] = pedge[v];
+        }
+        uint32_t total;
+        const uint32_t ex = io_excl_scan<IO_T, WAVE>(deg, sh->scan, &total);
+        sh->e0[tid] = ex;
+        if (tid == 0) sh->e0[IO_T] = total;
+        io_sync<WAVE>();
+        for (uint32_t f0 = (uint32_t)tid; f0 < total; f0 += 4 * IO_T) {
+            uint32_t e[4]; int j[4]; bool on[4];
+#pragma unroll
+            for (int q = 0; q < 4; q++) {
+                const uint32_t f = f0 + (uint32_t)q * IO_T;
+                on[q] = f < total;
+                int lo = 0, hi = IO_T;
+                while (hi - lo > 1) { const int mid = (lo + hi) >> 1; if (sh->e0[mid] <= f) lo = mid; else hi = mid; }
+                if (!on[q]) lo = 0;
+                j[q] = lo;
+                e[q] = sh->ef[lo] + (f - sh->e0[lo]);
+                on[q] = on[q] && e[q] != sh->pe[lo];
+                if constexpr (MASKED) { if (on[q] && refused(e[q])) on[q] = false; }
+            }
+            uint32_t u[4]; WInt<NL> w[4];
+#pragma unroll
+            for (int q = 0; q < 4; q++) {
+                const uint32_t ee = on[q] ? e[q] : 0u;
+                const uint32_t sw = esrc[ee];
+                u[q] = ESRC_NODE(sw);
+                w[q] = ewl ? wi_load<NL>(ewl + (size_t)ee * NL) : ew_decode<NL>(edge_wenc(sw, ew, ee, gt));
+            }
+#pragma unroll
+            for (int q = 0; q < 4; q++) {
+                const WInt<NL> du = wi_load<NL>(dist + (size_t)u[q] * NL), dv = wi_load<NL>(dist + (size_t)sh->v[j[q]] * NL);
+                mine |= on[q] && !wi_unreached<NL>(du) && wi_eq<NL>(wi_add<NL>(du, w[q]), dv);
+            }
+        }
+        io_sync<WAVE>();
+    }
+    if (mine) sh->flag = 1;
+    io_sync<WAVE>();
+    return sh->flag != 0;
 }
 
 template <int NL, int IO_T, bool MASKED = false>
-__device__ void inorder_contig(const DBatch &b, DMeta *meta, IoShared<IO_T> *sh, const uint32_t *mask = nullptr) {
+__device__ void inorder_rest(const DBatch &b, DMeta *meta, IoShared<IO_T> *sh, const uint32_t *mask = nullptr) {
     const int tid = threadIdx.x;
     const uint64_t mbase = MASKED ? (uint64_t)meta->edge_off : 0ull;
     auto refused = [&](uint32_t e) -> bool { const uint64_t x = mbase + e; return ((mask[x >> 5] >> (x & 31)) & 1u) != 0; };
     const int V = meta->n_node;
     const bool walked = meta->n_path >= 2;
     const int n = walked ? meta->n_path : 2;
-    const uint32_t *in_off = b.in_off + meta->node_off + blockIdx.x;
+    const uint32_t *in_off = b.in_off + meta->node_off + (meta - b.meta);
     const uint32_t *esrc = b.esrc + meta->edge_off;
     const long long *ew = b.ew + meta->edge_off;
     const uint64_t *ewl = b.ewl ? b.ewl + (size_t)meta->edge_off * NL : nullptr;
@@ -178,55 +264,6 @@
         const WInt<NL> w = ewl ? wi_load<NL>(ewl + (size_t)e * NL) : ew_decode<NL>(edge_wenc(sw, ew, e, gt));
         return !wi_unreached<NL>(du) && wi_eq<NL>(wi_add<NL>(du, w), dv);
     };
-    const uint32_t *pedge = (const uint32_t *)(b.parent + meta->node_off);
-    bool mine = !walked;
-    for (int c0 = 1; c0 < n && walked; c0 += IO_T) {
-        const int i = c0 + tid;
-        uint32_t deg = 0;
-        if (i < n) {
-            const int v = path[i];
-            const uint32_t f = in_off[v];
-            deg = in_off[v + 1] - f;
-            sh->v[tid] = v; sh->ef[tid] = f; sh->pe[tid] = pedge[v];
-        }
-        uint32_t total;
-        const uint32_t ex = block_excl_scan<IO_T>(deg, sh->scan, &total);
-        sh->e0[tid] = ex;
-        if (tid == 0) sh->e0[IO_T] = total;
-        __syncthreads();
-        for (uint32_t f0 = (uint32_t)tid; f0 < total; f0 += 4 * IO_T) {
-            uint32_t e[4]; int j[4]; bool on[4];
-#pragma unroll
-            for (int q = 0; q < 4; q++) {
-                const uint32_t f = f0 + (uint32_t)q * IO_T;
-                on[q] = f < total;
-                int lo = 0, hi = IO_T;
-                while (hi - lo > 1) { const int mid = (lo + hi) >> 1; if (sh->e0[mid] <= f) lo = mid; else hi = mid; }
-                if (!on[q]) lo = 0;
-                j[q] = lo;
-                e[q] = sh->ef[lo] + (f - sh->e0[lo]);
-                on[q] = on[q] && e[q] != sh->pe[lo];
-                if constexpr (MASKED) { if (on[q] && refused(e[q])) on[q] = false; }
-            }
-            uint32_t u[4]; WInt<NL> w[4];
-#pragma unroll
-            for (int q = 0; q < 4; q++) {
-                const uint32_t ee = on[q] ? e[q] : 0u;
-                const uint32_t sw = esrc[ee];
-                u[q] = ESRC_NODE(sw);
-                w[q] = ewl ? wi_load<NL>(ewl + (size_t)ee * NL) : ew_decode<NL>(edge_wenc(sw, ew, ee, gt));
-            }
-#pragma unroll
-            for (int q = 0; q < 4; q++) {
-                const WInt<NL> du = wi_load<NL>(dist + (size_t)u[q] * NL), dv = wi_load<NL>(dist + (size_t)sh->v[j[q]] * NL);
-                mine |= on[q] && !wi_unreached<NL>(du) && wi_eq<NL>(wi_add<NL>(du, w[q]), dv);
-            }
-        }
-        __syncthreads();
-    }
-    if (mine) sh->flag = 1;
-    __syncthreads();
-    if (!sh->flag) return;
 
     const size_t sz4 = ((size_t)V * 4 + 7) & ~(size_t)7, E = (size_t)meta->n_edge;
     if (tid == 0) {
@@ -353,12 +390,29 @@
     }
 }
 
+template <int NL, int IO_T, bool MASKED = false>
+__device__ void inorder_contig(const DBatch &b, DMeta *meta, IoShared<IO_T> *sh, const uint32_t *mask = nullptr) {
+    if (inorder_check<NL, IO_T, MASKED>(b, meta, sh, meta->n_path, mask)) inorder_rest<NL, IO_T, MASKED>(b, meta, sh, mask);
+}
+
+typedef IoShared<64, true> IoTail;
+template <int NL>
+__device__ __forceinline__ void duo_tail(const DBatch &b, DMeta *meta, IoTail *sh) {
+    if (threadIdx.x == 0) sh->flag = 0;
+    io_sync<true>();
+    const int np = walk_path<NL, 64, true>(b, meta, sh);
+    if (np < 2) return;
+    if (inorder_check<NL, 64, false, true>(b, meta, sh, np)) return;
+    if (threadIdx.x == 0) { meta->tail = 1; atomicAdd(&b.tot->tail_contigs, 1); }
+}
+
 template <int NL, int IO_T>
 __global__ __launch_bounds__(IO_T) void k_inorder(DBatch b) {
     __shared__ IoShared<IO_T> sh;
     if (b.tot->overflow & 3) return;
     DMeta *meta = &b.meta[blockIdx.x];
     if (meta->sssp_nl != NL) return;
+    if (meta->tail) return;
     if (threadIdx.x == 0) { sh.flag = 0; meta->tie = 0; }
     __syncthreads();
     if (meta->status < 0 || (meta->n_node <= 2 && !b.ewl)) return;
diff --git a/phanotate_amd/csrc/phx_internal.h b/phanotate_amd/csrc/phx_internal.h
--- a/phanotate_amd/csrc/phx_internal.h
+++ b/phanotate_amd/csrc/phx_internal.h
@@ -141,6 +141,8 @@
     int32_t cert;
     int32_t plan_prog;
     int32_t seg_fail;
+    int32_t tail;
+    int32_t pad_m;
     int64_t rec_off;
 };
 
@@ -188,7 +190,7 @@
     uint32_t gsync;
     int32_t seg_abort;
     int32_t seg_fallbacks;
-    int32_t pad_t2;
+    int32_t tail_contigs;
 };
 struct DCaps {
     int64_t orf, grp, node, cb, edge;
@@ -265,6 +267,7 @@
     DGene *genes;
     uint32_t *gene_total;
     int32_t duo;
+    int32_t duo_tail;
     int32_t plan_stream;
     int32_t seg;
     int32_t seg_margin_bp;
diff --git a/phanotate_amd/csrc/phx_kernels.hip b/phanotate_amd/csrc/phx_kernels.hip
--- a/phanotate_amd/csrc/phx_kernels.hip
+++ b/phanotate_amd/csrc/phx_kernels.hip
@@ -125,8 +125,8 @@
 #include "phx_front.inc"
 #include "phx_sssp_seg.inc"
 #include "phx_sssp_wave.inc"
+#include "phx_inorder.inc"
 #include "phx_sssp_duo.inc"
-#include "phx_inorder.inc"
 #include "phx_refine.inc"
 #include "phx_certify.inc"
 #include "phx_margins.inc"
diff --git a/phanotate_amd/csrc/phx_sssp_duo.inc b/phanotate_amd/csrc/phx_sssp_duo.inc
--- a/phanotate_amd/csrc/phx_sssp_duo.inc
+++ b/phanotate_amd/csrc/phx_sssp_duo.inc
@@ -890,7 +890,19 @@
 #endif
         meta->sssp_iters = phases;
         meta->n_genes = 0; meta->gene_off = 0;
-        if (N::unreached(N::load(ring + (size_t)((V - 1) & (WV_RING - 1)) * NL * 8))) { meta->status = PHX_S_NOPATH; meta->n_path = 0; }
+    }
+    const bool nopath = __builtin_amdgcn_readfirstlane((int)N::unreached(N::load(ring + (size_t)((V - 1) & (WV_RING - 1)) * NL * 8))) != 0;
+    if (lane == 0) {
+        if (nopath) { meta->status = PHX_S_NOPATH; meta->n_path = 0; }
         else meta->n_path = -2;
     }
+    if (!b.duo_tail || nopath) return;
+    static_assert(sizeof(IoTail) <= (size_t)WV_SLOTS * NL * 8 + (size_t)WV_SLOTS * 8 && alignof(IoTail) <= 16, "the tail's LDS fits ring + rel");
+#ifdef DUO_PROFILE
+    const long long t_tail = wall_clock64();
+#endif
+    duo_tail<NL>(b, meta, (IoTail *)ring);
+#ifdef DUO_PROFILE
+    if (lane == 0) meta->bg[5] = (uint32_t)(wall_clock64() - t_tail);
+#endif
 }
```

New measurement: 31780 Mbp/s. 0.972x the previous value.
